# swiss-territorial-data-lab/proj-roadsurf

Hardware: AMD Instinct MI355X
Metric: tiles_per_sec_512x512x3 (higher is better)
Workload: dtype f16 hi + lo operand planes (22 significand bits, 3 MFMA products per product) / f32 accumulate; 1 GPU; Mask R-CNN R50-FPN inference, batch 16 of 512x512 3-band tiles per GPU (BASELINE configs[1]), 800x800 network input; seeded synthetic weights, saturated: 1000 proposals and 100 detections per tile; batch_per_gpu=16, lanes=2, lane_streams=independent, num_classes=2, weights=random

## Files before the change

proj_roadsurf_amd/csrc/common.h:

```cpp
#pragma once
#include <hip/hip_runtime.h>
#include <stdint.h>
#include <stdio.h>

typedef _Float16 half_t;
typedef _Float16 half4 __attribute__((ext_vector_type(4)));
typedef _Float16 half8 __attribute__((ext_vector_type(8)));
typedef float f32x4 __attribute__((ext_vector_type(4)));

#define RS_OK 0
#define RS_ERR_ARG -1
#define RS_ERR_HIP -2
#define RS_ERR_BLOB -3
#define RS_ERR_UNSUPPORTED -4

void rs_set_error(const char* fmt, ...);

#define RS_HIP(expr)                                                                       \
  do {                                                                                     \
    hipError_t _e = (expr);                                                                \
    if (_e != hipSuccess) {                                                                \
      rs_set_error("%s:%d: %s -> %s", __FILE__, __LINE__, #expr, hipGetErrorString(_e));   \
      return RS_ERR_HIP;                                                                   \
    }                                                                                      \
  } while (0)

#define RS_CHECK(cond, code, ...)  \
  do {                             \
    if (!(cond)) {                 \
      rs_set_error(__VA_ARGS__);   \
      return (code);               \
    }                              \
  } while (0)

static inline int cdiv(long long a, long long b) { return (int)((a + b - 1) / b); }

#if defined(__HIPCC__)
__device__ __forceinline__ float rs_fdiv(float a, float b) {
  const float y0 = __builtin_amdgcn_rcpf(b);
  const float e = __builtin_fmaf(-b, y0, 1.0f);
  const float y = __builtin_fmaf(e, y0, y0);
  const float q0 = a * y;
  const float r0 = __builtin_fmaf(-b, q0, a);
  const float q1 = __builtin_fmaf(r0, y, q0);
  const float r1 = __builtin_fmaf(-b, q1, a);
  const float q = __builtin_fmaf(r1, y, q1);
  const bool special = !(__builtin_fabsf(b) > 0.f && __builtin_fabsf(b) < __builtin_inff() && __builtin_fabsf(a) > 0.f && __builtin_fabsf(a) < __builtin_inff());
  return special ? a * y0 : q;
}

__device__ __forceinline__ unsigned rs_sat_bad(float f) { return !(__builtin_fabsf(f) <= 65504.f); }
__device__ __forceinline__ void rs_sat_flush(unsigned long long* sat, unsigned cnt) {
  if (sat != nullptr && cnt != 0u) atomicAdd(sat, (unsigned long long)cnt);
}
#endif

struct RsDebug {
  int conv_single_stage_nk = 4;
  int conv_persist = 0;
  int conv_tuned = 1;
  int conv_deep = 1;
  int conv_wide_px = 128;
  int wreg_dbg = 0;
  int wreg_waves = 2;
  int conv_wreg = 1;
  int stem_small_tile = 1;
  int deep_dbg = 0;
  int deconv_variant = 22;
  int fuse_mask_predictor = 1;
  int side_stream = 1;
  int narrow_roialign = 0;
  int use_glds = 1;
  int fuse_shortcut = 1;
  int fuse_stem = 1;
  int fuse_bneck = 1;
  int deep_tile_px = 1;
  int deep_tail = 1;
  int fuse_rpn_heads = 1;
  int merge_levels = 1;
  int graph_small = 1;
  int use_graph = 0;
  int train_roi_side = -1;
  int train_side = -1;
  int wgrad_target = 512;
  int wgrad_cb = 0;
  int select_debug = 0;
  int nms_debug = 0;
  int roi_window = 1;
  int roi_bwd_atomic = 0;
  int roi_order = 1;
};
const RsDebug& rs_debug();
void rs_debug_reload();

struct ConvSeg {
  const half_t* in;
  const half_t* w;
  const float* bias;
  void* out;
  float* head_out;
  int Ho, Wo, in_Hp, in_Wp, out_Hp, out_Wp;
  int M;
  int tile0;
  long long in_lo, out_lo;
  const float* wscale;
};
#define RS_MAX_SEGS 5

struct ConvParams {
  const half_t* in;
  const half_t* w;
  const float* bias;
  void* out;
  const half_t* res;
  const half_t* up;
  const int* m_count;
  const int* koff;
  int m_mul;
  int M;
  int Ho, Wo;
  int in_Hp, in_Wp, in_Cs, in_off;
  int stride;
  int KH, KW, Cin;
  int Kpad;
  int Cout;
  int out_Hp, out_Wp, out_Cs, out_pad;
  int up_Hp, up_Wp, up_Cs, up_pad;
  int relu;
  int mode;
  int out_f32;
  const float* dot_w;
  const int* dot_cls;
  const int* dot_slot;
  float* dot_out;
  int dot_k;
  const half_t* in2;
  int in2_Hp, in2_Wp, in2_Cs, in2_off, stride2, Cin2;
  const half_t* down;
  int down_Hp, down_Wp, down_Cs, down_pad;
  const float* res32;
  const half_t* mask;
  int out_stride;
  long long* probe;
  int persist;
  int stages;
  const half_t* head_w;
  const float* head_b;
  float* head_out;
  int nseg;
  int seg_tiles;
  int tail_tiles;
  int split;
  long long in_lo, w_lo, out_lo, res_lo, up_lo, in2_lo;
  const float* wscale;
  long long head_w_lo;
  const float* head_scale;
  ConvSeg seg[RS_MAX_SEGS];
  unsigned long long* sat;
};

int launch_conv(const ConvParams& p, hipStream_t stream, int force_variant , int use_glds);
int conv_choose_variant(ConvParams& p, int force_variant, int use_glds);
extern thread_local int g_last_conv_variant;

struct StemPoolParams {
  const half_t* in;
  const half_t* wf;
  const float* bias;
  half_t* out;
  int N, in_Hp, in_Wp;
  int Hc, Wc;
  int Hq, Wq;
  unsigned long long* sat;
};
int launch_stem_pool(const StemPoolParams& p, hipStream_t stream);
struct StemPoolSplitParams {
  const half_t* in; long long in_lo;
  const half_t* wf;
  const float* wscale;
  const float* bias;
  half_t* out; long long out_lo;
  int N, in_Hp, in_Wp;
  int Hc, Wc;
  int Hq, Wq;
  unsigned long long* sat;
};
int launch_stem_pool_split(const StemPoolSplitParams& p, hipStream_t stream);

struct BneckParams {
  const half_t* t1;
  const half_t* w2;
  const float* b2;
  const half_t* w3p;
  const float* b3;
  const half_t* x;
  const half_t* x0;
  const half_t* wsc;
  half_t* out;
  const half_t* w1p;
  const float* b1;
  half_t* t1n;
  int M, H, W, Hp, Wp;
  int CB;
  unsigned long long* sat;
};
int launch_bneck_tail(const BneckParams& p, hipStream_t stream);

struct BneckSplitParams {
  const half_t* t1; long long t1_lo;
  const half_t* w2; long long w2_lo;
  const float* b2; const float* s2;
  const half_t* w3p; long long w3_lo;
  const float* b3; const float* s3;
  const half_t* x; long long x_lo;
  half_t* out; long long out_lo;
  const half_t* w1p; long long w1_lo;
  const float* b1; const float* s1;
  half_t* t1n; long long t1n_lo;
  const half_t* x0; long long x0_lo;
  int M, H, W, Hp, Wp;
  int CB;
  unsigned long long* sat;
};
int launch_bneck_tail_split(const BneckSplitParams& p, hipStream_t stream);

int launch_mask_overlap(const uint8_t* det, int n_det, const uint8_t* lab, int n_lab, int h, int w, int* inter, int* lab_area, hipStream_t s);

struct WgradParams {
  const half_t* dy;
  const half_t* x;
  float* partial;
  float* grad;
  const half_t* zeros;
  const float* scale;
  int M, Ho, Wo;
  int dy_Hp, dy_Wp, dy_Cs, dy_pad;
  int in_Hp, in_Wp, in_Cs, in_off;
  int stride, KH, KW, Cin, Cout, Kpad;
  const int* m_count;
  int m_mul;
  int splits;
  int accumulate;
  int f32;
};
int wgrad_splits(const WgradParams& p);
int launch_conv_wgrad(const WgradParams& p, hipStream_t stream);

struct PreprocParams {
  const uint8_t* tiles;
  half_t* out;
  const int* hb;
  const int* hk;
  const int* vb;
  const int* vk;
  int N, H, W, C;
  int new_h, new_w;
  int out_Hp, out_Wp;
  int ksh, ksv;
  int need_h, need_v;
  int flip;
  int out_f32;
  long long out_lo;
  float mean[4], stdv[4];
  unsigned long long* sat;
};
int launch_preprocess(const PreprocParams& p, hipStream_t s);
int launch_maxpool(const half_t* in, half_t* out, int N, int Hi, int Wi, int Ho, int Wo, int C, hipStream_t s);
int launch_subsample2(const half_t* in, half_t* out, int N, int Hi, int Wi, int Ho, int Wo, int C, hipStream_t s);
int launch_maxpool_f32(const float* in, float* out, int N, int Hi, int Wi, int Ho, int Wo, int C, hipStream_t s);
int launch_maxpool_split(const half_t* in, long long in_lo, half_t* out, long long out_lo, int N, int Hi, int Wi, int Ho, int Wo, int C, hipStream_t s);
int launch_subsample2_split(const half_t* in, long long in_lo, half_t* out, long long out_lo, int N, int Hi, int Wi, int Ho, int Wo, int C, hipStream_t s);
int launch_subsample2_f32(const float* in, float* out, int N, int Hi, int Wi, int Ho, int Wo, int C, hipStream_t s);
int launch_conv_f32(const ConvParams& p, hipStream_t stream, int force_valu = 0, int tile = 0);
int launch_conv_deep(const ConvParams& p, hipStream_t stream, int tile_px = 256);
int rs_device_cu_count();
bool conv_wreg_ok(const ConvParams& p);
int launch_conv_wreg(const ConvParams& p, hipStream_t stream, int waves = 0);
int launch_conv_deep_multi(const ConvParams& common, const ConvSeg* segs, const int* m_per_image, int nseg, int images, hipStream_t stream);
```

proj_roadsurf_amd/csrc/conv_deep.hip:

```cpp
#include "common.h"

namespace {

constexpr int BN = 256, NT = 512, MI = 4, WCH = 4;
constexpr int ASTAGE = 256 * 128, WSTAGE = BN * 128;
constexpr int W_BASE = 3 * ASTAGE;
constexpr int LDS_BYTES = 3 * ASTAGE + 2 * WSTAGE;

__device__ __forceinline__ void glds16(const half_t* g, char* lds_wave_base) {
  __builtin_amdgcn_global_load_lds((const __attribute__((address_space(1))) void*)g,
                                   (__attribute__((address_space(3))) void*)lds_wave_base, 16, 0, 0);
}

template <int DBG, bool TRAIN, int NJ, bool SPLIT>
__device__ __forceinline__ void conv_deep_tile(const ConvParams& p, char* smem, const half_t* g_in, const half_t* g_w, const float* g_bias, void* g_out,
                                               float* g_head_out, const int Ho, const int Wo, const int in_Hp, const int in_Wp, const int out_Hp, const int out_Wp,
                                               const int M, const int m0, const int n0, const int q, const long long in_lo, const long long out_lo,
                                               const float* g_wscale) {
  constexpr int APS = (NJ + 1) / 2;
  constexpr int WPX = NJ * 16;
  const int tid = threadIdx.x;
  const int lane = tid & 63;
  const int wave = __builtin_amdgcn_readfirstlane(tid >> 6);
  const int wpx = wave / WCH, wch = wave % WCH;
  (void)q;

  const int lrow = lane >> 3, lchk = lane & 7;
  const half_t* aptr[APS];
  const half_t* wptr[4];
  unsigned aoffb[APS], woffb[4];
#pragma unroll
  for (int ps = 0; ps < APS; ++ps) {
    int m = m0 + ps * 64 + wave * 8 + lrow;
    if (m >= M) m = M - 1;
    const int x = m % Wo;
    const int t = m / Wo;
    const int y = t % Ho;
    const int n = t / Ho;
    const long long base =
        ((long long)(n * in_Hp + y * p.stride + p.in_off) * in_Wp + x * p.stride + p.in_off) * p.in_Cs;
    if constexpr (SPLIT) aoffb[ps] = (unsigned)((base + ((lchk ^ lrow) & 3) * 8 + ((lchk ^ lrow) >> 2) * in_lo) * 2);
    else aptr[ps] = g_in + base + (lchk ^ lrow) * 8;
  }
#pragma unroll
  for (int ps = 0; ps < 4; ++ps) {
    const int row = ps * 64 + wave * 8 + lrow;
    const int key = (row & 3) | (((row >> 4) & 1) << 2);
    if constexpr (SPLIT) woffb[ps] = (unsigned)(((long long)(n0 + row) * p.Kpad + ((lchk ^ key) & 3) * 8 + ((lchk ^ key) >> 2) * p.w_lo) * 2);
    else wptr[ps] = g_w + (long long)(n0 + row) * p.Kpad + (lchk ^ key) * 8;
  }
  constexpr int KST = SPLIT ? 32 : 64;
  const int nk = p.KH * p.KW * (p.Cin / KST);

  int akh = 0, akw = 0, ac0 = 0, an = 0;
  auto stage_a = [&]() {
    const int off = (akh * in_Wp + akw) * p.in_Cs + ac0;
    if (++akw == p.KW) { akw = 0; if (++akh == p.KH) { akh = 0; ac0 += KST; } }
    char* abase = smem + (an % 3) * ASTAGE;
    ++an;
    if (DBG & 1) return;
    if (DBG & 8) return;
    if constexpr (SPLIT) {
#pragma unroll
      for (int ps = 0; ps < APS; ++ps) glds16((const half_t*)((const char*)g_in + (aoffb[ps] + (unsigned)(off * 2))), abase + (ps * 64 + wave * 8) * 128);
    } else {
#pragma unroll
      for (int ps = 0; ps < APS; ++ps) glds16(aptr[ps] + off, abase + (ps * 64 + wave * 8) * 128);
    }
  };
  int wkh = 0, wkw = 0, wc0 = 0, wn = 0;
  auto stage_w = [&]() {
    const int koff = (wkh * p.KW + wkw) * p.Cin + wc0;
    if (++wkw == p.KW) { wkw = 0; if (++wkh == p.KH) { wkh = 0; wc0 += KST; } }
    char* wbase = smem + W_BASE + (wn & 1) * WSTAGE;
    ++wn;
    if (DBG & 1) return;
    if (DBG & 4) return;
    if constexpr (SPLIT) {
#pragma unroll
      for (int ps = 0; ps < 4; ++ps) glds16((const half_t*)((const char*)g_w + (woffb[ps] + (unsigned)(koff * 2))), wbase + (ps * 64 + wave * 8) * 128);
    } else {
#pragma unroll
      for (int ps = 0; ps < 4; ++ps) glds16(wptr[ps] + koff, wbase + (ps * 64 + wave * 8) * 128);
    }
  };

  const int fi = lane & 15, fq = lane >> 4, fkey = lane & 7;
  int w_off[MI], x_off[NJ];
#pragma unroll
  for (int i = 0; i < MI; ++i) w_off[i] = W_BASE + (wch * 64 + (fi >> 2) * 16 + i * 4 + (fi & 3)) * 128;
#pragma unroll
  for (int j = 0; j < NJ; ++j) x_off[j] = (wpx * WPX + j * 16 + fi) * 128;
  const int c0_off = (fq ^ fkey) * 16, c1_off = ((4 + fq) ^ fkey) * 16;

  f32x4 acc[MI][NJ];
#pragma unroll
  for (int i = 0; i < MI; ++i)
#pragma unroll
    for (int j = 0; j < NJ; ++j) acc[i][j] = f32x4{0.f, 0.f, 0.f, 0.f};

  half8 wf0[MI], xf0[NJ], wf1[MI], xf1[NJ];
  const unsigned lds0 = (unsigned)(uintptr_t)(__attribute__((address_space(3))) char*)smem;
  const unsigned wrow = (unsigned)(W_BASE + (wch * 64 + (fi >> 2) * 16 + (fi & 3)) * 128);
  const unsigned xrow = (unsigned)((wpx * WPX + fi) * 128);
  const unsigned wa0 = lds0 + wrow + c0_off, wa1 = lds0 + wrow + c1_off;
  const unsigned xa0 = lds0 + xrow + c0_off, xa1 = lds0 + xrow + c1_off;
#define RS_DSR(dst, addr, off) asm volatile("ds_read_b128 %0, %1 offset:%2" : "=v"(dst) : "v"(addr), "n"(off))
#define RS_READS(wf, xf, wa, xa)                                                        \
  RS_DSR(wf[0], wa, 0); RS_DSR(wf[1], wa, 512); RS_DSR(wf[2], wa, 1024); RS_DSR(wf[3], wa, 1536);   \
  RS_DSR(xf[0], xa, 0); RS_DSR(xf[1], xa, 2048);                                                    \
  if constexpr (NJ > 2) { RS_DSR(xf[2], xa, 4096); }                                                \
  if constexpr (NJ > 3) { RS_DSR(xf[3], xa, 6144); }                                                \
  if constexpr (NJ > 4) { RS_DSR(xf[4], xa, 8192); }                                                \
  if constexpr (NJ > 5) { RS_DSR(xf[5], xa, 10240); }                                               \
  if constexpr (NJ > 6) { RS_DSR(xf[6], xa, 12288); }                                               \
  if constexpr (NJ > 7) { RS_DSR(xf[7], xa, 14336); }
  auto reads0 = [&](int ab, int wb) {
    if (DBG & 16) return;
    const unsigned wa = wa0 + ((DBG & 2) ? 0 : wb) * WSTAGE, xa = xa0 + ((DBG & 2) ? 0 : ab) * ASTAGE;
    RS_READS(wf0, xf0, wa, xa)
  };
  auto reads1 = [&](int ab, int wb) {
    if (DBG & 16) return;
    const unsigned wa = wa1 + ((DBG & 2) ? 0 : wb) * WSTAGE, xa = xa1 + ((DBG & 2) ? 0 : ab) * ASTAGE;
    RS_READS(wf1, xf1, wa, xa)
  };
#ifdef RS_CLOCK_PROBE
  const unsigned long long pr_t0 = __builtin_amdgcn_s_memtime(), pr_r0 = __builtin_amdgcn_s_memrealtime();
#endif
#ifdef RS_SPLIT_PHASES
  const unsigned long long ph_entry = __builtin_amdgcn_s_memtime();
  unsigned long long ph_loop0 = 0, ph_loop1 = 0;
#endif
  stage_w();
  stage_a();
  if (nk > 1) stage_a();
  if (nk > 1) asm volatile("s_waitcnt vmcnt(%0)" ::"n"(APS) : "memory");
  else asm volatile("s_waitcnt vmcnt(0)" ::: "memory");
  asm volatile("s_barrier" ::: "memory");
  __builtin_amdgcn_sched_barrier(0);
  if (nk > 1) stage_w();
#ifndef RS_SPLIT_SCHED_V1
  if constexpr (!SPLIT) { if (nk > 2) stage_a(); }
#else
  if (nk > 2) stage_a();
#endif
  if constexpr (SPLIT) {
#define RS_RD_W(wf, wa) RS_DSR(wf[0], wa, 0); RS_DSR(wf[1], wa, 512); RS_DSR(wf[2], wa, 1024); RS_DSR(wf[3], wa, 1536);
#define RS_RD_X(xf, xa)                                                                             \
  RS_DSR(xf[0], xa, 0); RS_DSR(xf[1], xa, 2048);                                                    \
  if constexpr (NJ > 2) { RS_DSR(xf[2], xa, 4096); }                                                \
  if constexpr (NJ > 3) { RS_DSR(xf[3], xa, 6144); }                                                \
  if constexpr (NJ > 4) { RS_DSR(xf[4], xa, 8192); }                                                \
  if constexpr (NJ > 5) { RS_DSR(xf[5], xa, 10240); }                                               \
  if constexpr (NJ > 6) { RS_DSR(xf[6], xa, 12288); }                                               \
  if constexpr (NJ > 7) { RS_DSR(xf[7], xa, 14336); }
    {
      const unsigned wa = wa0, xa = xa1;
      RS_RD_W(wf0, wa)
      RS_RD_X(xf1, xa)
    }
    int sab = 0;
#ifdef RS_SPLIT_PHASES
    unsigned long long ph_work = 0, ph_vm = 0, ph_bar = 0, ph_last = __builtin_amdgcn_s_memtime();
    ph_loop0 = ph_last;
#endif
    for (int t = 0; t < nk; ++t) {
      const unsigned wst = (t & 1) * WSTAGE, ast = sab * ASTAGE;
      __builtin_amdgcn_sched_barrier(0);
      { const unsigned xa = xa0 + ast; RS_RD_X(xf0, xa) }
      __builtin_amdgcn_sched_barrier(0);
      asm volatile("s_waitcnt lgkmcnt(%0)" ::"n"(NJ) : "memory");
      __builtin_amdgcn_sched_barrier(0);
#pragma unroll
      for (int i = 0; i < MI; ++i)
#pragma unroll
        for (int j = 0; j < NJ; ++j)
          acc[i][j] = __builtin_amdgcn_mfma_f32_16x16x32_f16(wf0[i], xf1[j], acc[i][j], 0, 0, 0);
      __builtin_amdgcn_sched_barrier(0);
#ifndef RS_SPLIT_SCHED_V1
      if (t + 2 < nk) stage_a();
#endif
      { const unsigned wa = wa1 + wst; RS_RD_W(wf1, wa) }
      __builtin_amdgcn_sched_barrier(0);
      asm volatile("s_waitcnt lgkmcnt(4)" ::: "memory");
      __builtin_amdgcn_sched_barrier(0);
#pragma unroll
      for (int i = 0; i < MI; ++i)
#pragma unroll
        for (int j = 0; j < NJ; ++j)
          acc[i][j] = __builtin_amdgcn_mfma_f32_16x16x32_f16(wf0[i], xf0[j], acc[i][j], 0, 0, 0);
      __builtin_amdgcn_sched_barrier(0);
      const int snext = sab == 2 ? 0 : sab + 1;
      if (t + 1 < nk) {
        asm volatile("s_waitcnt lgkmcnt(0)" ::: "memory");
#ifdef RS_SPLIT_PHASES
        __builtin_amdgcn_sched_barrier(0);
        const unsigned long long ph1 = __builtin_amdgcn_s_memtime();
        ph_work += ph1 - ph_last;
        __builtin_amdgcn_sched_barrier(0);
#endif
        if (t + 2 < nk) asm volatile("s_waitcnt vmcnt(%0)" ::"n"(APS) : "memory");
        else asm volatile("s_waitcnt vmcnt(0)" ::: "memory");
#ifdef RS_SPLIT_PHASES
        __builtin_amdgcn_sched_barrier(0);
        const unsigned long long ph2 = __builtin_amdgcn_s_memtime();
        ph_vm += ph2 - ph1;
        __builtin_amdgcn_sched_barrier(0);
#endif
        asm volatile("s_barrier" ::: "memory");
        __builtin_amdgcn_sched_barrier(0);
#ifdef RS_SPLIT_PHASES
        ph_last = __builtin_amdgcn_s_memtime();
        ph_bar += ph_last - ph2;
        __builtin_amdgcn_sched_barrier(0);
#endif
        if (wpx) {
#pragma unroll
          for (int i = 0; i < MI; ++i)
#pragma unroll
            for (int j = 0; j < NJ; ++j)
              acc[i][j] = __builtin_amdgcn_mfma_f32_16x16x32_f16(wf1[i], xf0[j], acc[i][j], 0, 0, 0);
          __builtin_amdgcn_sched_barrier(0);
        }
        if (t + 2 < nk) stage_w();
#ifdef RS_SPLIT_SCHED_V1
        if (t + 3 < nk) stage_a();
#endif
        {
          const unsigned wa = wa0 + ((t + 1) & 1) * WSTAGE, xa = xa1 + snext * ASTAGE;
          RS_RD_W(wf0, wa)
          RS_RD_X(xf1, xa)
        }
        if (wpx) { sab = snext; continue; }
      } else {
        __builtin_amdgcn_sched_barrier(0);
        asm volatile("s_waitcnt lgkmcnt(0)" ::: "memory");
      }
      sab = snext;
      __builtin_amdgcn_sched_barrier(0);
#pragma unroll
      for (int i = 0; i < MI; ++i)
#pragma unroll
        for (int j = 0; j < NJ; ++j)
          acc[i][j] = __builtin_amdgcn_mfma_f32_16x16x32_f16(wf1[i], xf0[j], acc[i][j], 0, 0, 0);
    }
#undef RS_RD_W
#undef RS_RD_X
#ifdef RS_SPLIT_PHASES
    ph_loop1 = __builtin_amdgcn_s_memtime();
    if (p.probe && lane == 0) {
      long long* o = p.probe + ((long long)q * 8 + wave) * 8;
      o[0] = (long long)ph_work; o[1] = (long long)ph_vm; o[2] = (long long)ph_bar; o[3] = nk;
      o[4] = (long long)(ph_loop0 - ph_entry); o[5] = (long long)(ph_loop1 - ph_loop0);
    }
#endif
  } else {
  reads0(0, 0);
  int abuf = 0;
  for (int t = 0; t < nk; ++t) {
    __builtin_amdgcn_sched_barrier(0);
    reads1(abuf, t & 1);
    __builtin_amdgcn_sched_barrier(0);
    asm volatile("s_waitcnt lgkmcnt(%0)" ::"n"(4 + NJ) : "memory");
    __builtin_amdgcn_sched_barrier(0);
#pragma unroll
    for (int i = 0; i < MI; ++i)
#pragma unroll
      for (int j = 0; j < NJ; ++j)
        acc[i][j] = __builtin_amdgcn_mfma_f32_16x16x32_f16(wf0[i], xf0[j], acc[i][j], 0, 0, 0);
    __builtin_amdgcn_sched_barrier(0);
    const int anext = abuf == 2 ? 0 : abuf + 1;
    if (t + 1 < nk) {
      asm volatile("s_waitcnt lgkmcnt(0)" ::: "memory");
      if (t + 2 < nk) asm volatile("s_waitcnt vmcnt(%0)" ::"n"(APS) : "memory");
      else asm volatile("s_waitcnt vmcnt(0)" ::: "memory");
      asm volatile("s_barrier" ::: "memory");
      __builtin_amdgcn_sched_barrier(0);
#ifndef RS_DEEP_LOCKSTEP
      if (wpx) {
#pragma unroll
        for (int i = 0; i < MI; ++i)
#pragma unroll
          for (int j = 0; j < NJ; ++j)
            acc[i][j] = __builtin_amdgcn_mfma_f32_16x16x32_f16(wf1[i], xf1[j], acc[i][j], 0, 0, 0);
        __builtin_amdgcn_sched_barrier(0);
      }
#endif
      if (t + 2 < nk) stage_w();
      if (t + 3 < nk) stage_a();
      reads0(anext, (t + 1) & 1);
#ifndef RS_DEEP_LOCKSTEP
      if (wpx) { abuf = anext; continue; }
#endif
    }
    else {
      __builtin_amdgcn_sched_barrier(0);
      asm volatile("s_waitcnt lgkmcnt(0)" ::: "memory");
    }
    abuf = anext;
    __builtin_amdgcn_sched_barrier(0);
#pragma unroll
    for (int i = 0; i < MI; ++i)
#pragma unroll
      for (int j = 0; j < NJ; ++j)
        acc[i][j] = __builtin_amdgcn_mfma_f32_16x16x32_f16(wf1[i], xf1[j], acc[i][j], 0, 0, 0);
  }
  }

#ifdef RS_CLOCK_PROBE
  if (p.probe && tid == 0) {
    p.probe[2 * q] = (long long)(__builtin_amdgcn_s_memtime() - pr_t0);
    p.probe[2 * q + 1] = (long long)(__builtin_amdgcn_s_memrealtime() - pr_r0);
  }
#endif
  const int crow = n0 + wch * 64 + fq * 16;
  float bias[16];
#pragma unroll
  for (int i = 0; i < MI; ++i) {
    const f32x4 b4 = *(const f32x4*)(g_bias + crow + i * 4);
    bias[i * 4 + 0] = b4[0]; bias[i * 4 + 1] = b4[1]; bias[i * 4 + 2] = b4[2]; bias[i * 4 + 3] = b4[3];
  }
  float wsc[SPLIT ? 16 : 1];
  if constexpr (SPLIT) {
#pragma unroll
    for (int i = 0; i < MI; ++i) {
      const f32x4 s4 = *(const f32x4*)(g_wscale + crow + i * 4);
      wsc[i * 4 + 0] = s4[0]; wsc[i * 4 + 1] = s4[1]; wsc[i * 4 + 2] = s4[2]; wsc[i * 4 + 3] = s4[3];
    }
  }
  unsigned satc = 0;
  if (!TRAIN && SPLIT && p.head_w) {
    const half_t* hw = p.head_w + (long long)fi * 256 + wch * 64 + fq * 8;
    const half8 ha0 = *(const half8*)hw, ha1 = *(const half8*)(hw + 32);
    const half8 hl0 = *(const half8*)(hw + p.head_w_lo), hl1 = *(const half8*)(hw + p.head_w_lo + 32);
    f32x4 hacc[NJ];
#pragma unroll
    for (int j = 0; j < NJ; ++j) {
      half8 b0, b1, l0, l1;
      const bool mv = m0 + wpx * WPX + j * 16 + fi < M;
      unsigned sath = 0;
#pragma unroll
      for (int i = 0; i < MI; ++i)
#pragma unroll
        for (int r = 0; r < 4; ++r) {
          float f = acc[i][j][r] * wsc[i * 4 + r] + bias[i * 4 + r];
          if (p.relu) f = f > 0.f ? f : 0.f;
          sath += mv ? rs_sat_bad(f) : 0u;
          f = f > 65504.f ? 65504.f : (f < -65504.f ? -65504.f : f);
          const half_t h = (half_t)f;
          const half_t l = (half_t)(f - (float)h);
          if (i < 2) { b0[i * 4 + r] = h; l0[i * 4 + r] = l; } else { b1[(i - 2) * 4 + r] = h; l1[(i - 2) * 4 + r] = l; }
        }
      rs_sat_flush(p.sat, sath);
      f32x4 a = f32x4{0.f, 0.f, 0.f, 0.f};
      a = __builtin_amdgcn_mfma_f32_16x16x32_f16(ha0, b0, a, 0, 0, 0);
      a = __builtin_amdgcn_mfma_f32_16x16x32_f16(ha1, b1, a, 0, 0, 0);
      a = __builtin_amdgcn_mfma_f32_16x16x32_f16(ha0, l0, a, 0, 0, 0);
      a = __builtin_amdgcn_mfma_f32_16x16x32_f16(ha1, l1, a, 0, 0, 0);
      a = __builtin_amdgcn_mfma_f32_16x16x32_f16(hl0, b0, a, 0, 0, 0);
      a = __builtin_amdgcn_mfma_f32_16x16x32_f16(hl1, b1, a, 0, 0, 0);
      hacc[j] = a;
    }
    asm volatile("s_barrier" ::: "memory");
    float* part = (float*)smem;
#pragma unroll
    for (int j = 0; j < NJ; ++j) *(f32x4*)(part + ((wch * 2 * WPX + wpx * WPX + j * 16 + fi) * 16 + fq * 4)) = hacc[j];
    __syncthreads();
    const int px = tid >> 1, oh = (tid & 1) * 8;
    const int m = m0 + px;
    if (px < 2 * WPX && m < M) {
      f32x4 s0 = f32x4{0.f, 0.f, 0.f, 0.f}, s1 = f32x4{0.f, 0.f, 0.f, 0.f};
#pragma unroll
      for (int w = 0; w < 4; ++w) {
        s0 += *(const f32x4*)(part + ((w * 2 * WPX + px) * 16 + oh));
        s1 += *(const f32x4*)(part + ((w * 2 * WPX + px) * 16 + oh + 4));
      }
      s0 = s0 * *(const f32x4*)(p.head_scale + oh) + *(const f32x4*)(p.head_b + oh);
      s1 = s1 * *(const f32x4*)(p.head_scale + oh + 4) + *(const f32x4*)(p.head_b + oh + 4);
      const int x = m % Wo, t = m / Wo, y = t % Ho, n = t / Ho;
      float* op = g_head_out + ((long long)(n * Ho + y) * Wo + x) * 16 + oh;
      *(f32x4*)op = s0;
      *(f32x4*)(op + 4) = s1;
    }
    return;
  }
  if (!TRAIN && !SPLIT && p.head_w) {
    const half_t* hw = p.head_w + (long long)fi * 256 + wch * 64 + fq * 8;
    const half8 ha0 = *(const half8*)hw, ha1 = *(const half8*)(hw + 32);
    f32x4 hacc[NJ];
#pragma unroll
    for (int j = 0; j < NJ; ++j) {
      half8 b0, b1;
      const bool mv = m0 + wpx * WPX + j * 16 + fi < M;
      unsigned sath = 0;
#pragma unroll
      for (int i = 0; i < MI; ++i)
#pragma unroll
        for (int r = 0; r < 4; ++r) {
          float f = acc[i][j][r] + bias[i * 4 + r];
          if (p.relu) f = f > 0.f ? f : 0.f;
          sath += mv ? rs_sat_bad(f) : 0u;
          f = f > 65504.f ? 65504.f : (f < -65504.f ? -65504.f : f);
          if (i < 2) b0[i * 4 + r] = (half_t)f; else b1[(i - 2) * 4 + r] = (half_t)f;
        }
      rs_sat_flush(p.sat, sath);
      f32x4 a = f32x4{0.f, 0.f, 0.f, 0.f};
      a = __builtin_amdgcn_mfma_f32_16x16x32_f16(ha0, b0, a, 0, 0, 0);
      a = __builtin_amdgcn_mfma_f32_16x16x32_f16(ha1, b1, a, 0, 0, 0);
      hacc[j] = a;
    }
    asm volatile("s_barrier" ::: "memory");
    float* part = (float*)smem;
#pragma unroll
    for (int j = 0; j < NJ; ++j) *(f32x4*)(part + ((wch * 2 * WPX + wpx * WPX + j * 16 + fi) * 16 + fq * 4)) = hacc[j];
    __syncthreads();
    const int px = tid >> 1, oh = (tid & 1) * 8;
    const int m = m0 + px;
    if (px < 2 * WPX && m < M) {
      f32x4 s0 = *(const f32x4*)(p.head_b + oh), s1 = *(const f32x4*)(p.head_b + oh + 4);
#pragma unroll
      for (int w = 0; w < 4; ++w) {
        s0 += *(const f32x4*)(part + ((w * 2 * WPX + px) * 16 + oh));
        s1 += *(const f32x4*)(part + ((w * 2 * WPX + px) * 16 + oh + 4));
      }
      const int x = m % Wo, t = m / Wo, y = t % Ho, n = t / Ho;
      float* op = g_head_out + ((long long)(n * Ho + y) * Wo + x) * 16 + oh;
      *(f32x4*)op = s0;
      *(f32x4*)(op + 4) = s1;
    }
    return;
  }
#pragma unroll
  for (int j = 0; j < NJ; ++j) {
    const int m = m0 + wpx * WPX + j * 16 + fi;
    if (m >= M) continue;
    const int x = m % Wo;
    const int t = m / Wo;
    const int y = t % Ho;
    const int n = t / Ho;
    const long long opix = (long long)(n * out_Hp + y + p.out_pad) * out_Wp + x + p.out_pad;
    float v[16];
#pragma unroll
    for (int i = 0; i < MI; ++i)
#pragma unroll
      for (int r = 0; r < 4; ++r) {
        if constexpr (SPLIT) v[i * 4 + r] = acc[i][j][r] * wsc[i * 4 + r] + bias[i * 4 + r];
        else v[i * 4 + r] = acc[i][j][r] + bias[i * 4 + r];
      }
    if (p.res) {
      const half_t* rp = p.res + opix * p.out_Cs + crow;
#pragma unroll
      for (int i = 0; i < MI; ++i) {
        const half4 h = *(const half4*)(rp + i * 4);
        if constexpr (SPLIT) {
          const half4 l = *(const half4*)(rp + p.res_lo + i * 4);
#pragma unroll
          for (int r = 0; r < 4; ++r) v[i * 4 + r] += (float)h[r] + (float)l[r];
        } else {
#pragma unroll
          for (int r = 0; r < 4; ++r) v[i * 4 + r] += (float)h[r];
        }
      }
    }
    if (p.up) {
      const long long upix = (long long)(n * p.up_Hp + (y >> 1) + p.up_pad) * p.up_Wp + (x >> 1) + p.up_pad;
      const half_t* up = p.up + upix * p.up_Cs + crow;
#pragma unroll
      for (int i = 0; i < MI; ++i) {
        const half4 h = *(const half4*)(up + i * 4);
        if constexpr (SPLIT) {
          const half4 l = *(const half4*)(up + p.up_lo + i * 4);
#pragma unroll
          for (int r = 0; r < 4; ++r) v[i * 4 + r] += (float)h[r] + (float)l[r];
        } else {
#pragma unroll
          for (int r = 0; r < 4; ++r) v[i * 4 + r] += (float)h[r];
        }
      }
    }
    if (TRAIN && p.down) {
#pragma unroll
      for (int dd = 0; dd < 4; ++dd) {
        const long long dpix = (long long)(n * p.down_Hp + 2 * y + (dd >> 1) + p.down_pad) * p.down_Wp + 2 * x + (dd & 1) + p.down_pad;
        const half_t* dp = p.down + dpix * p.down_Cs + crow;
#pragma unroll
        for (int i = 0; i < MI; ++i) {
          const half4 h = *(const half4*)(dp + i * 4);
#pragma unroll
          for (int r = 0; r < 4; ++r) v[i * 4 + r] += (float)h[r];
        }
      }
    }
    if (TRAIN && p.res32) {
      const float* rp = p.res32 + opix * p.out_Cs + crow;
#pragma unroll
      for (int i = 0; i < MI; ++i) {
        const f32x4 h = *(const f32x4*)(rp + i * 4);
#pragma unroll
        for (int r = 0; r < 4; ++r) v[i * 4 + r] += h[r];
      }
    }
    if (TRAIN && p.mask) {
      const half_t* mp = p.mask + opix * p.out_Cs + crow;
#pragma unroll
      for (int i = 0; i < MI; ++i) {
        const half4 h = *(const half4*)(mp + i * 4);
#pragma unroll
        for (int r = 0; r < 4; ++r) v[i * 4 + r] = (float)h[r] > 0.f ? v[i * 4 + r] : 0.f;
      }
    }
    if (p.relu) {
#pragma unroll
      for (int e = 0; e < 16; ++e) v[e] = v[e] > 0.f ? v[e] : 0.f;
    }
    if (p.out_f32) {
      float* op = (float*)g_out + opix * p.out_Cs + crow;
#pragma unroll
      for (int i = 0; i < MI; ++i) *(f32x4*)(op + i * 4) = f32x4{v[i * 4], v[i * 4 + 1], v[i * 4 + 2], v[i * 4 + 3]};
    } else {
      half_t* op = (half_t*)g_out + opix * p.out_Cs + crow;
#pragma unroll
      for (int i = 0; i < MI; i += 2) {
        half8 h, l;
#pragma unroll
        for (int r = 0; r < 8; ++r) {
          float f = v[i * 4 + r];
          satc += rs_sat_bad(f);
          f = f > 65504.f ? 65504.f : (f < -65504.f ? -65504.f : f);
          h[r] = (half_t)f;
          if constexpr (SPLIT) l[r] = (half_t)(f - (float)h[r]);
        }
        *(half8*)(op + i * 4) = h;
        if constexpr (SPLIT) *(half8*)(op + out_lo + i * 4) = l;
      }
    }
  }
  rs_sat_flush(p.sat, satc);
#ifdef RS_SPLIT_PHASES
  if constexpr (SPLIT) {
    const unsigned long long ph_issued = __builtin_amdgcn_s_memtime();
    asm volatile("s_waitcnt vmcnt(0)" ::: "memory");
    const unsigned long long ph_drained = __builtin_amdgcn_s_memtime();
    if (p.probe && lane == 0) {
      long long* o = p.probe + ((long long)q * 8 + wave) * 8;
      o[6] = (long long)(ph_issued - ph_loop1); o[7] = (long long)(ph_drained - ph_issued);
    }
  }
#endif
}


template <int DBG, bool TRAIN = false, int NJF = 8, bool SPLIT = false>
__global__ __launch_bounds__(NT) void conv_deep_kernel(const ConvParams p) {
  constexpr int BM = 32 * NJF;
  extern __shared__ __attribute__((aligned(16))) char smem[];
  int M = p.M;
  if (p.m_count) {
    long long mc = (long long)(*p.m_count) * p.m_mul;
    if (mc < M) M = (int)mc;
  }
  const int tiles_n = p.Cout / BN;
  const int ntiles = p.nseg ? p.seg_tiles : tiles_n * ((M + BM - 1) / BM);
  const int nfull = ntiles - p.tail_tiles;
  const int q = blockIdx.x;
  if (q >= nfull + 2 * p.tail_tiles) return;
  const half_t* g_in = p.in;
  const half_t* g_w = p.w;
  const float* g_bias = p.bias;
  void* g_out = p.out;
  float* g_head_out = p.head_out;
  long long in_lo = p.in_lo, out_lo = p.out_lo;
  const float* g_wscale = p.wscale;
  int Ho = p.Ho, Wo = p.Wo, in_Hp = p.in_Hp, in_Wp = p.in_Wp, out_Hp = p.out_Hp, out_Wp = p.out_Wp;
  int L, half = -1;
  if (q < nfull) {
    const int qn = nfull >> 3, r = nfull & 7, x = q & 7;
    L = (x < r ? x * (qn + 1) : r * (qn + 1) + (x - r) * qn) + (q >> 3);
  } else {
    L = nfull + ((q - nfull) >> 1);
    half = (q - nfull) & 1;
  }
  if (p.nseg) {
    int t0 = 0;
#pragma unroll
    for (int i = 0; i < RS_MAX_SEGS; ++i)
      if (i < p.nseg && L >= p.seg[i].tile0) {
        g_in = p.seg[i].in; g_w = p.seg[i].w; g_bias = p.seg[i].bias; g_out = p.seg[i].out; g_head_out = p.seg[i].head_out;
        Ho = p.seg[i].Ho; Wo = p.seg[i].Wo; in_Hp = p.seg[i].in_Hp; in_Wp = p.seg[i].in_Wp;
        out_Hp = p.seg[i].out_Hp; out_Wp = p.seg[i].out_Wp; M = p.seg[i].M; t0 = p.seg[i].tile0;
        if constexpr (SPLIT) { in_lo = p.seg[i].in_lo; out_lo = p.seg[i].out_lo; g_wscale = p.seg[i].wscale; }
      }
    L -= t0;
  }
  const int n0 = (L % tiles_n) * BN;
  const int m0 = (L / tiles_n) * BM;
  if (half < 0 || NJF != 8) {
    conv_deep_tile<DBG, TRAIN, NJF, SPLIT>(p, smem, g_in, g_w, g_bias, g_out, g_head_out, Ho, Wo, in_Hp, in_Wp, out_Hp, out_Wp, M, m0, n0, q, in_lo, out_lo, g_wscale);
  } else {
    if (m0 + half * (BM / 2) >= M) return;
    conv_deep_tile<DBG, TRAIN, NJF == 8 ? 4 : NJF, SPLIT>(p, smem, g_in, g_w, g_bias, g_out, g_head_out, Ho, Wo, in_Hp, in_Wp, out_Hp, out_Wp, M, m0 + half * (BM / 2), n0, q, in_lo, out_lo, g_wscale);
  }
}

}

int rs_device_cu_count() {
  static int ncu[64] = {0};
  int dev = 0;
  if (hipGetDevice(&dev) != hipSuccess || dev < 0 || dev >= 64) return 256;
  if (!ncu[dev]) {
    int n = 0;
    if (hipDeviceGetAttribute(&n, hipDeviceAttributeMultiprocessorCount, dev) != hipSuccess || n <= 0) n = 256;
    ncu[dev] = n;
  }
  return ncu[dev];
}

static int deep_tail_tiles(long long tiles) {
  const int ncu = rs_device_cu_count();
  if (!rs_debug().deep_tail) return 0;
  const int r = (int)(tiles % ncu);
  return (r > 0 && 2 * r <= ncu) ? r : 0;
}

static int no_scratch(const void* kernel, const char* what) {
  hipFuncAttributes a;
  RS_HIP(hipFuncGetAttributes(&a, kernel));
  RS_CHECK(a.localSizeBytes == 0, RS_ERR_UNSUPPORTED, "%s was built with %zu bytes of scratch per thread: its asm fragment reads must not be spilled (rebuild with the documented toolchain)",
           what, (size_t)a.localSizeBytes);
  return RS_OK;
}

template <int NJF>
static int launch_deep_nj(ConvParams& p, hipStream_t stream) {
  static bool done = false;
  if (!done) {
    RS_HIP(hipFuncSetAttribute((const void*)conv_deep_kernel<0, false, NJF>, hipFuncAttributeMaxDynamicSharedMemorySize, LDS_BYTES));
    if constexpr (NJF >= 5) RS_HIP(hipFuncSetAttribute((const void*)conv_deep_kernel<0, false, NJF, true>, hipFuncAttributeMaxDynamicSharedMemorySize, LDS_BYTES));
    { int rc = no_scratch((const void*)conv_deep_kernel<0, false, NJF>, "conv_deep_kernel"); if (rc) return rc; }
    if constexpr (NJF >= 5) { int rc = no_scratch((const void*)conv_deep_kernel<0, false, NJF, true>, "conv_deep_kernel (split operands)"); if (rc) return rc; }
    done = true;
  }
  const long long nblk = (long long)(p.Cout / BN) * cdiv(p.M, 32 * NJF);
  RS_CHECK(nblk < (1ll << 30), RS_ERR_ARG, "conv_deep: grid too large");
  p.tail_tiles = 0;
  if (p.split) {
    if constexpr (NJF >= 5) hipLaunchKernelGGL((conv_deep_kernel<0, false, NJF, true>), dim3((unsigned)nblk), dim3(NT), LDS_BYTES, stream, p);
    else RS_CHECK(false, RS_ERR_UNSUPPORTED, "conv_deep: the split-operand mode has the 160 .. 256-pixel tiles only");
    RS_HIP(hipGetLastError());
    return RS_OK;
  }
  hipLaunchKernelGGL((conv_deep_kernel<0, false, NJF>), dim3((unsigned)nblk), dim3(NT), LDS_BYTES, stream, p);
  RS_HIP(hipGetLastError());
  return RS_OK;
}

int launch_conv_deep(const ConvParams& p0, hipStream_t stream, int tile_px) {
  ConvParams p = p0;
  p.nseg = 0;
  RS_CHECK(p.mode == 0 && !p.in2 && p.Cin % 64 == 0 && p.Cout % BN == 0 && p.M > 0, RS_ERR_ARG,
           "conv_deep: unsupported shape (mode %d, Cin %d, Cout %d)", p.mode, p.Cin, p.Cout);
  RS_CHECK(!p.head_w || (p.Cout == BN && p.head_b && p.head_out && !p.res && !p.up && !p.down && !p.res32 && !p.mask), RS_ERR_ARG,
           "conv_deep: the fused head needs Cout == 256, its bias and output, and no other epilogue option");
  RS_CHECK(p.out_stride <= 1, RS_ERR_UNSUPPORTED, "conv_deep: no strided scatter");
  RS_CHECK(!p.split || (p.wscale && (!p.head_w || p.head_scale) && !p.down && !p.res32 && !p.mask), RS_ERR_UNSUPPORTED, "conv_deep: the split-operand mode needs the row scales (the fused head's too) and has no training epilogue");
  if (p.split) {
    const long long in_px = (long long)cdiv(p.M, p.Ho * p.Wo) * p.in_Hp * p.in_Wp;
    RS_CHECK((p.in_lo + in_px * p.in_Cs) * 2 < (1ll << 32) && (p.w_lo + (long long)p.Cout * p.Kpad) * 2 < (1ll << 32), RS_ERR_UNSUPPORTED,
             "conv_deep: split-operand tensor of more than 4 GB (input %lld elements per plane)", in_px * p.in_Cs);
  }
  if (tile_px != 256) {
    RS_CHECK(tile_px >= 64 && tile_px <= 224 && tile_px % 32 == 0 && !p.down && !p.res32 && !p.mask, RS_ERR_ARG,
             "conv_deep: tile height %d (256, or 64 .. 224 in steps of 32 without training epilogue options)", tile_px);
    switch (tile_px / 32) {
      case 2: return launch_deep_nj<2>(p, stream);
      case 3: return launch_deep_nj<3>(p, stream);
      case 4: return launch_deep_nj<4>(p, stream);
      case 5: return launch_deep_nj<5>(p, stream);
      case 6: return launch_deep_nj<6>(p, stream);
      default: return launch_deep_nj<7>(p, stream);
    }
  }
  constexpr int BM = 256;
  static bool done = false;
  if (!done) {
    RS_HIP(hipFuncSetAttribute((const void*)conv_deep_kernel<0>, hipFuncAttributeMaxDynamicSharedMemorySize, LDS_BYTES));
    RS_HIP(hipFuncSetAttribute((const void*)conv_deep_kernel<0, true>, hipFuncAttributeMaxDynamicSharedMemorySize, LDS_BYTES));
    RS_HIP(hipFuncSetAttribute((const void*)conv_deep_kernel<0, false, 8, true>, hipFuncAttributeMaxDynamicSharedMemorySize, LDS_BYTES));
    { int rc = no_scratch((const void*)conv_deep_kernel<0>, "conv_deep_kernel"); if (rc) return rc; }
    { int rc = no_scratch((const void*)conv_deep_kernel<0, true>, "conv_deep_kernel (training epilogue)"); if (rc) return rc; }
    { int rc = no_scratch((const void*)conv_deep_kernel<0, false, 8, true>, "conv_deep_kernel (split operands)"); if (rc) return rc; }
#ifdef RS_DEEP_CEILING
    RS_HIP(hipFuncSetAttribute((const void*)conv_deep_kernel<1>, hipFuncAttributeMaxDynamicSharedMemorySize, LDS_BYTES));
    RS_HIP(hipFuncSetAttribute((const void*)conv_deep_kernel<3>, hipFuncAttributeMaxDynamicSharedMemorySize, LDS_BYTES));
    RS_HIP(hipFuncSetAttribute((const void*)conv_deep_kernel<4>, hipFuncAttributeMaxDynamicSharedMemorySize, LDS_BYTES));
    RS_HIP(hipFuncSetAttribute((const void*)conv_deep_kernel<8>, hipFuncAttributeMaxDynamicSharedMemorySize, LDS_BYTES));
    RS_HIP(hipFuncSetAttribute((const void*)conv_deep_kernel<17>, hipFuncAttributeMaxDynamicSharedMemorySize, LDS_BYTES));
#endif
    done = true;
  }
#ifdef RS_DEEP_CEILING
  const int dbg = rs_debug().deep_dbg;
#else
  constexpr int dbg = 0;
#endif
  long long nblk = (long long)(p.Cout / BN) * cdiv(p.M, BM);
  RS_CHECK(nblk < (1ll << 30), RS_ERR_ARG, "conv_deep: grid too large");
  p.tail_tiles = (p.m_count || dbg) ? 0 : deep_tail_tiles(nblk);
  nblk += p.tail_tiles;
#ifdef RS_DEEP_CEILING
  if (dbg == 1) { hipLaunchKernelGGL(conv_deep_kernel<1>, dim3((unsigned)nblk), dim3(NT), LDS_BYTES, stream, p); return RS_OK; }
  if (dbg == 3) { hipLaunchKernelGGL(conv_deep_kernel<3>, dim3((unsigned)nblk), dim3(NT), LDS_BYTES, stream, p); return RS_OK; }
  if (dbg == 4) { hipLaunchKernelGGL(conv_deep_kernel<4>, dim3((unsigned)nblk), dim3(NT), LDS_BYTES, stream, p); return RS_OK; }
  if (dbg == 8) { hipLaunchKernelGGL(conv_deep_kernel<8>, dim3((unsigned)nblk), dim3(NT), LDS_BYTES, stream, p); return RS_OK; }
  if (dbg == 17) { hipLaunchKernelGGL(conv_deep_kernel<17>, dim3((unsigned)nblk), dim3(NT), LDS_BYTES, stream, p); return RS_OK; }
#endif
  (void)dbg;
  if (p.split) hipLaunchKernelGGL((conv_deep_kernel<0, false, 8, true>), dim3((unsigned)nblk), dim3(NT), LDS_BYTES, stream, p);
  else if (p.down || p.res32 || p.mask) hipLaunchKernelGGL((conv_deep_kernel<0, true>), dim3((unsigned)nblk), dim3(NT), LDS_BYTES, stream, p);
  else hipLaunchKernelGGL(conv_deep_kernel<0>, dim3((unsigned)nblk), dim3(NT), LDS_BYTES, stream, p);
  RS_HIP(hipGetLastError());
  return RS_OK;
}

int launch_conv_deep_multi(const ConvParams& common, const ConvSeg* segs, const int* m_per_image, int nseg, int images, hipStream_t stream) {
  RS_CHECK(nseg >= 1 && nseg <= RS_MAX_SEGS && images >= 1, RS_ERR_ARG, "conv_deep_multi: %d maps", nseg);
  RS_CHECK(common.mode == 0 && !common.in2 && common.Cin % 64 == 0 && common.Cout % BN == 0 && !common.res && !common.up && !common.m_count &&
               !common.down && !common.res32 && !common.mask && common.out_stride <= 1,
           RS_ERR_ARG, "conv_deep_multi: unsupported shape (mode %d, Cin %d, Cout %d) or epilogue option", common.mode, common.Cin, common.Cout);
  ConvParams p = common;
  p.nseg = nseg;
  long long tiles = 0;
  for (int i = 0; i < nseg; ++i) {
    RS_CHECK(segs[i].in && segs[i].w && segs[i].bias && segs[i].out && m_per_image[i] > 0, RS_ERR_ARG, "conv_deep_multi: map %d incomplete", i);
    RS_CHECK(!common.split || segs[i].wscale, RS_ERR_ARG, "conv_deep_multi: map %d has no row scales (split-operand mode)", i);
    RS_CHECK(!common.split || ((segs[i].in_lo + (long long)images * segs[i].in_Hp * segs[i].in_Wp * common.in_Cs) * 2 < (1ll << 32) &&
                               (common.w_lo + (long long)common.Cout * common.Kpad) * 2 < (1ll << 32)),
             RS_ERR_UNSUPPORTED, "conv_deep_multi: map %d: split-operand tensor of more than 4 GB", i);
    p.seg[i] = segs[i];
    p.seg[i].M = images * m_per_image[i];
    p.seg[i].tile0 = (int)tiles;
    tiles += (long long)(p.Cout / BN) * cdiv(p.seg[i].M, 256);
  }
  RS_CHECK(tiles < (1ll << 30), RS_ERR_ARG, "conv_deep_multi: grid too large");
  if (p.head_w) {
    RS_CHECK(p.Cout == BN && p.head_b && !p.out_f32, RS_ERR_ARG, "conv_deep_multi: the fused head needs Cout == 256 and its bias");
    for (int i = 0; i < nseg; ++i) RS_CHECK(segs[i].head_out, RS_ERR_ARG, "conv_deep_multi: map %d has no head output", i);
  }
  p.seg_tiles = (int)tiles;
  p.tail_tiles = deep_tail_tiles(tiles);
  tiles += p.tail_tiles;
  p.in = segs[0].in; p.w = segs[0].w; p.bias = segs[0].bias; p.out = segs[0].out; p.M = p.seg[0].M;
  static bool done = false;
  if (!done) {
    RS_HIP(hipFuncSetAttribute((const void*)conv_deep_kernel<0>, hipFuncAttributeMaxDynamicSharedMemorySize, LDS_BYTES));
    RS_HIP(hipFuncSetAttribute((const void*)conv_deep_kernel<0, false, 8, true>, hipFuncAttributeMaxDynamicSharedMemorySize, LDS_BYTES));
    { int rc = no_scratch((const void*)conv_deep_kernel<0>, "conv_deep_kernel"); if (rc) return rc; }
    { int rc = no_scratch((const void*)conv_deep_kernel<0, false, 8, true>, "conv_deep_kernel (split operands)"); if (rc) return rc; }
    done = true;
  }
  if (p.split) {
    RS_CHECK(!p.head_w || p.head_scale, RS_ERR_ARG, "conv_deep_multi: the fused head of the split-operand mode needs its row scales");
    hipLaunchKernelGGL((conv_deep_kernel<0, false, 8, true>), dim3((unsigned)tiles), dim3(NT), LDS_BYTES, stream, p);
    RS_HIP(hipGetLastError());
    return RS_OK;
  }
  hipLaunchKernelGGL(conv_deep_kernel<0>, dim3((unsigned)tiles), dim3(NT), LDS_BYTES, stream, p);
  RS_HIP(hipGetLastError());
  return RS_OK;
}
```

proj_roadsurf_amd/csrc/engine.hip:

```cpp
#include <stdarg.h>
#include <string.h>

#include <cmath>
#include <functional>
#include <map>
#include <set>
#include <string>
#include <vector>

#include "../../include/rs_engine.h"
#include "detect.h"
#include "train.h"

static thread_local char g_err[1024] = "";
static bool g_trainer_unfused_shortcut = false;

static RsDebug g_debug;
static bool g_debug_loaded = false;
void rs_debug_reload() {
  RsDebug d;
  auto rd = [](const char* name, int* v) { const char* e = getenv(name); if (e && *e) *v = atoi(e); };
  rd("RS_CONV_SINGLE_STAGE_NK", &d.conv_single_stage_nk); rd("RS_CONV_PERSIST", &d.conv_persist); rd("RS_CONV_TUNED", &d.conv_tuned);
  rd("RS_CONV_DEEP", &d.conv_deep); rd("RS_CONV_WIDE_PX", &d.conv_wide_px); rd("RS_CONV_WREG", &d.conv_wreg); rd("RS_WREG_DBG", &d.wreg_dbg); rd("RS_ROI_BWD_ATOMIC", &d.roi_bwd_atomic); rd("RS_WREG_WAVES", &d.wreg_waves); rd("RS_STEM_SMALL_TILE", &d.stem_small_tile); rd("RS_DEEP_DBG", &d.deep_dbg);
  rd("RS_DECONV_VARIANT", &d.deconv_variant); rd("RS_FUSE_MASK_PREDICTOR", &d.fuse_mask_predictor); rd("RS_SIDE_STREAM", &d.side_stream);
  rd("RS_NARROW_ROIALIGN", &d.narrow_roialign); rd("RS_USE_GLDS", &d.use_glds); rd("RS_FUSE_SHORTCUT", &d.fuse_shortcut); rd("RS_MERGE_LEVELS", &d.merge_levels); rd("RS_FUSE_RPN_HEADS", &d.fuse_rpn_heads); rd("RS_DEEP_TAIL", &d.deep_tail); rd("RS_DEEP_TILE_PX", &d.deep_tile_px); rd("RS_FUSE_BNECK", &d.fuse_bneck); rd("RS_FUSE_STEM", &d.fuse_stem);
  rd("RS_USE_GRAPH", &d.use_graph); rd("RS_GRAPH_SMALL", &d.graph_small); rd("RS_TRAIN_ROI_SIDE", &d.train_roi_side);
  rd("RS_TRAIN_SIDE", &d.train_side); rd("RS_WGRAD_TARGET", &d.wgrad_target); rd("RS_WGRAD_CB", &d.wgrad_cb);
  rd("RS_SELECT_DEBUG", &d.select_debug); rd("RS_NMS_DEBUG", &d.nms_debug); rd("RS_ROI_WINDOW", &d.roi_window); rd("RS_ROI_ORDER", &d.roi_order);
  g_debug = d;
  g_debug_loaded = true;
}
const RsDebug& rs_debug() {
  if (!g_debug_loaded) rs_debug_reload();
  return g_debug;
}
void rs_set_error(const char* fmt, ...) {
  va_list a;
  va_start(a, fmt);
  vsnprintf(g_err, sizeof g_err, fmt, a);
  va_end(a);
}

namespace {

enum { DT_F16 = 1, DT_F32 = 2, DT_I32 = 3, DT_U8 = 4, DT_SPLIT16 = 5 };
static size_t dt_size(int dt) { return (dt == DT_F16 || dt == DT_SPLIT16) ? 2 : (dt == DT_U8 ? 1 : 4); }

struct TensorInfo {
  std::string name;
  void* p = nullptr;
  int dtype = 0, ndim = 0, halo = 0;
  int64_t dims[5] = {1, 1, 1, 1, 1};
  size_t bytes = 0;
};

struct Act {
  half_t* p = nullptr;
  long long lo = 0;
  int N = 0, H = 0, W = 0, C = 0, pad = 0;
  int Hp() const { return H + 2 * pad; }
  int Wp() const { return W + 2 * pad; }
};

struct Stage {
  std::string name;
  std::function<int(int, hipStream_t)> fn;
  double flops_per_image = 0, bytes_per_image = 0;
  double ms_total = 0;
  int calls = 0;
  double last_flops = 0, last_bytes = 0;
  int variant = -2;
  bool narrow = false;
  bool grad_side = false;
  int bucket = -1;
  int phase = 0;
  hipEvent_t handoff = nullptr;
};

struct BlobEntry { const void* host; void* dev; int dtype; int ndim; int64_t dims[4]; size_t nbytes; };

}

extern "C" void rs_resize_shape(int h, int w, int short_edge, int max_size, int* new_h, int* new_w) {
  double scale = (double)short_edge * 1.0 / (double)(h < w ? h : w);
  double newh, neww;
  if (h < w) { newh = short_edge; neww = scale * w; } else { newh = scale * h; neww = short_edge; }
  const double mx = newh > neww ? newh : neww;
  if (mx > max_size) {
    scale = (double)max_size * 1.0 / mx;
    newh = newh * scale;
    neww = neww * scale;
  }
  *new_w = (int)(neww + 0.5);
  *new_h = (int)(newh + 0.5);
}

extern "C" int rs_resize_coeffs(int in_size, int out_size, int32_t* bounds, int32_t* coeffs) {
  const double scale = (double)in_size / (double)out_size;
  const double filterscale = scale < 1.0 ? 1.0 : scale;
  const double support = 1.0 * filterscale;
  const int ksize = (int)ceil(support) * 2 + 1;
  if (!bounds || !coeffs) return ksize;
  const double ss = 1.0 / filterscale;
  std::vector<double> w(ksize);
  for (int xx = 0; xx < out_size; ++xx) {
    const double center = (xx + 0.5) * scale;
    int xmin = (int)(center - support + 0.5);
    if (xmin < 0) xmin = 0;
    int xmax = (int)(center + support + 0.5);
    if (xmax > in_size) xmax = in_size;
    xmax -= xmin;
    double ww = 0.0;
    for (int x = 0; x < ksize; ++x) w[x] = 0.0;
    for (int x = 0; x < xmax; ++x) {
      double a = (x + xmin - center + 0.5) * ss;
      if (a < 0) a = -a;
      const double v = a < 1.0 ? 1.0 - a : 0.0;
      w[x] = v;
      ww += v;
    }
    for (int x = 0; x < xmax; ++x)
      if (ww != 0.0) w[x] /= ww;
    for (int x = 0; x < ksize; ++x) {
      const double v = w[x] * (double)(1 << 22);
      coeffs[xx * ksize + x] = v < 0 ? (int)(v - 0.5) : (int)(v + 0.5);
    }
    bounds[xx * 2] = xmin;
    bounds[xx * 2 + 1] = xmax;
  }
  return ksize;
}

struct rs_engine {
  rs_spec spec;
  int device = 0;
  hipStream_t stream = nullptr;
  bool own_stream = false;
  hipStream_t copy_stream = nullptr;
  hipEvent_t ev_results = nullptr;
  hipEvent_t ev_copied = nullptr;
  bool copy_pending = false;
  hipStream_t narrow = nullptr;
  bool on_narrow = false;
  hipEvent_t ev_join = nullptr;
  bool cur_record = false;
  int max_batch = 0, tile_h = 0, tile_w = 0, tile_c = 0;
  int net_h = 0, net_w = 0, pad_h = 0, pad_w = 0;
  int use_glds = 1;
  bool f32 = false;
  bool split = false;
  int profiling = 0;
  hipEvent_t ev0 = nullptr, ev1 = nullptr;
  std::vector<std::pair<hipEvent_t, hipEvent_t>> ev_pool;
  std::vector<int> ev_stage;
  std::vector<int> ev_batch;
  size_t ev_used = 0;
  int resolve_profile();

  void* blob_dev = nullptr;
  std::map<std::string, BlobEntry> blob;
  std::vector<void*> allocs;
  std::vector<TensorInfo> tensors;
  std::vector<Stage> stages;

  uint8_t* tiles_dev = nullptr;
  struct ResizeTab { int* b = nullptr; int* k = nullptr; int ks = 0; };
  std::map<int, ResizeTab> tab_h, tab_v;
  std::vector<int> img_new_h, img_new_w;
  float* img_hw_dev = nullptr;
  int resize_tab(int in_size, int out_size, std::map<int, ResizeTab>& cache, ResizeTab* out);
  int set_image_sizes(const int32_t* new_h, const int32_t* new_w, int n);
  int* det_count = nullptr;
  float* det_boxes = nullptr;
  float* det_boxes_net = nullptr;
  float* det_scores = nullptr;
  int* det_classes = nullptr;
  uint8_t* masks = nullptr;
  float* mask_probs = nullptr;
  int D = 0;
  int* crop_rects = nullptr;
  unsigned int* crop_offsets = nullptr;
  unsigned long long* crop_total = nullptr;
  uint8_t* crop_data = nullptr;
  unsigned long long* h_crop_total = nullptr;
  hipEvent_t ev_crop_hdr = nullptr;

  int alloc(void** p, size_t bytes) {
    if (bytes == 0) bytes = 16;
    bytes = (bytes + 255) & ~(size_t)255;
    RS_HIP(hipMalloc(p, bytes));
    allocs.push_back(*p);
    RS_HIP(hipMemsetAsync(*p, 0, bytes, stream));
    return RS_OK;
  }
  void reg(const std::string& name, void* p, int dtype, std::vector<int64_t> dims, int halo) {
    TensorInfo t;
    t.name = name; t.p = p; t.dtype = dtype; t.ndim = (int)dims.size(); t.halo = halo;
    size_t nb = dt_size(dtype);
    for (size_t i = 0; i < dims.size(); ++i) { t.dims[i] = dims[i]; nb *= (size_t)dims[i]; }
    t.bytes = dtype == DT_SPLIT16 ? 2 * nb : nb;
    tensors.push_back(t);
  }
  int new_act(Act* a, const std::string& name, int N, int H, int W, int C, int pad) {
    a->N = N; a->H = H; a->W = W; a->C = C; a->pad = pad;
    const size_t bytes = (size_t)N * a->Hp() * a->Wp() * C * (f32 ? 4 : 2) * (split ? 2 : 1);
    int rc = alloc((void**)&a->p, bytes);
    if (rc) return rc;
    a->lo = split ? (long long)N * a->Hp() * a->Wp() * C : 0;
    reg(name, a->p, f32 ? DT_F32 : (split ? DT_SPLIT16 : DT_F16), {N, a->Hp(), a->Wp(), C}, pad);
    return RS_OK;
  }
  const BlobEntry* find(const std::string& n) {
    auto it = blob.find(n);
    return it == blob.end() ? nullptr : &it->second;
  }
  const BlobEntry* findw(const std::string& layer) { return find(layer + (f32 ? ".w32" : (split ? ".ws" : ".w"))); }
  int wrows(const BlobEntry* w) const { return (int)(split ? w->dims[0] / 2 : w->dims[0]); }
  int set_split(ConvParams* p, const std::string& wname, const BlobEntry* w, const Act* in, const Act* out, const Act* res, const Act* up, const Act* in2) {
    if (!split) return RS_OK;
    const BlobEntry* si = find(wname + ".wsi");
    RS_CHECK(si && si->dtype == DT_F32 && si->dims[0] >= w->dims[0] / 2 && (w->dims[0] & 1) == 0, RS_ERR_BLOB, "row scales of %s missing from blob (split-operand mode)", wname.c_str());
    p->split = 1;
    p->wscale = (const float*)si->dev;
    p->w_lo = (long long)(w->dims[0] / 2) * w->dims[1];
    if (in) p->in_lo = in->lo;
    if (out) p->out_lo = out->lo;
    if (res) p->res_lo = res->lo;
    if (up) p->up_lo = up->lo;
    if (in2) p->in2_lo = in2->lo;
    return RS_OK;
  }
  int parse_blob(const void* data, size_t nbytes);
  int build();
  struct DeferredConv { ConvParams p; int m_per_image = 0; double flops = 0, bytes = 0; };
  int add_conv(const std::string& name, const std::string& wname, const Act& in, const Act& out, int k, int stride,
               int pad, bool relu, const Act* res, const Act* up, int cin_real, int units_per_tile = 1,
               const int* m_count = nullptr, const Act* in2 = nullptr, int stride2 = 1, DeferredConv* defer = nullptr);
  int add_merged_convs(const std::string& name, const std::vector<DeferredConv>& d);
  int run(const uint8_t* tiles, int n, int phase = -1);
  int run_stages(int n, bool record, int phase = -1, bool all_wide = false);
  int assign_phases();
  int use_graph = 0;
  int fuse_shortcut = 1;
  int fuse_bneck = 1;
  int fuse_stem = 1;
  bool frozen_fusions_only = false;
  int merge_levels = 1;
  long long forward_index = 0;
  static constexpr int kSatCap = 512;
  unsigned long long* sat_dev = nullptr;
  unsigned long long* sat_snap = nullptr;
  unsigned long long* h_sat_copy = nullptr;
  bool sat_copy_pending = false;
  std::vector<int64_t> h_sat;
  unsigned long long* sat_slot() const { return sat_dev ? sat_dev + stages.size() : nullptr; }
  int sat_copy(hipStream_t s) {
    if (!sat_dev) return RS_OK;
    RS_HIP(hipMemcpyAsync(h_sat_copy, sat_snap, stages.size() * 8, hipMemcpyDeviceToHost, s));
    sat_copy_pending = true;
    return RS_OK;
  }
  void sat_publish() {
    if (!sat_copy_pending) return;
    h_sat.assign(h_sat_copy, h_sat_copy + stages.size());
    sat_copy_pending = false;
  }
  std::set<int> warmed;
  std::map<int, hipGraphExec_t> graphs;
};

int rs_engine::parse_blob(const void* data, size_t nbytes) {
  const uint8_t* b = (const uint8_t*)data;
  RS_CHECK(nbytes >= 16, RS_ERR_BLOB, "weight blob too small");
  uint32_t hdr[4];
  memcpy(hdr, b, 16);
  RS_CHECK(hdr[0] == 0x52534557u && hdr[1] == 1u, RS_ERR_BLOB, "bad weight blob magic/version %08x/%u", hdr[0], hdr[1]);
  const size_t ent = 96 + 4 + 4 + 32 + 8 + 8;
  RS_CHECK(16 + ent * hdr[2] <= nbytes, RS_ERR_BLOB, "weight blob truncated");
  RS_HIP(hipMalloc(&blob_dev, nbytes));
  RS_HIP(hipMemcpy(blob_dev, data, nbytes, hipMemcpyHostToDevice));
  for (uint32_t i = 0; i < hdr[2]; ++i) {
    const uint8_t* e = b + 16 + ent * i;
    char name[97];
    memcpy(name, e, 96);
    name[96] = 0;
    BlobEntry be;
    uint32_t dt, nd;
    uint64_t dims[4], off, nb;
    memcpy(&dt, e + 96, 4);
    memcpy(&nd, e + 100, 4);
    memcpy(dims, e + 104, 32);
    memcpy(&off, e + 136, 8);
    memcpy(&nb, e + 144, 8);
    RS_CHECK(off + nb <= nbytes, RS_ERR_BLOB, "weight blob entry %s out of range", name);
    be.host = b + off;
    be.dev = (char*)blob_dev + off;
    be.dtype = (int)dt;
    be.ndim = (int)nd;
    for (int d = 0; d < 4; ++d) be.dims[d] = (int64_t)dims[d];
    be.nbytes = nb;
    blob[name] = be;
  }
  return RS_OK;
}

int rs_engine::add_conv(const std::string& name, const std::string& wname, const Act& in, const Act& out, int k,
                        int stride, int pad, bool relu, const Act* res, const Act* up, int cin_real, int units_per_tile,
                        const int* m_count, const Act* in2, int stride2, DeferredConv* defer) {
  const BlobEntry* w = findw(wname);
  const BlobEntry* b = find(wname + ".b");
  RS_CHECK(w && b, RS_ERR_BLOB, "weights for %s missing from blob", wname.c_str());
  RS_CHECK(w->dtype == (f32 ? DT_F32 : DT_F16) && b->dtype == DT_F32, RS_ERR_BLOB, "weights for %s have wrong dtype", wname.c_str());
  ConvParams p;
  memset(&p, 0, sizeof p);
  { int rc = set_split(&p, wname, w, &in, &out, res, up, in2); if (rc) return rc; }
  p.in = in.p; p.w = (const half_t*)w->dev; p.bias = (const float*)b->dev; p.out = out.p;
  p.res = res ? res->p : nullptr;
  p.up = up ? up->p : nullptr;
  p.Ho = out.H; p.Wo = out.W;
  p.in_Hp = in.Hp(); p.in_Wp = in.Wp(); p.in_Cs = in.C; p.in_off = in.pad - pad;
  p.stride = stride; p.KH = k; p.KW = k; p.Cin = in.C;
  p.Kpad = (int)w->dims[1];
  p.Cout = out.C;
  p.out_Hp = out.Hp(); p.out_Wp = out.Wp(); p.out_Cs = out.C; p.out_pad = out.pad;
  if (up) { p.up_Hp = up->Hp(); p.up_Wp = up->Wp(); p.up_Cs = up->C; p.up_pad = up->pad; }
  p.relu = relu ? 1 : 0;
  if (in2) {
    RS_CHECK((out.H - 1) * stride2 < in2->H && (out.W - 1) * stride2 < in2->W && in2->C % 64 == 0, RS_ERR_ARG, "%s: second source geometry", name.c_str());
// ... 440 lines not shown
    if ((rc = add_conv("rpn.conv" + ln, "proposal_generator.rpn_head.conv", P[l], t, 3, 1, 1, true, nullptr, nullptr, 256))) return rc;
    rpn_t[l] = t;
  }
  for (int l = 0; l < L; ++l) {
    const std::string ln = std::to_string(l + 2);
    const Act t = rpn_t[l];
    float* ho = rpn_ho[l];
    if (!fuse_heads) {
      const BlobEntry* w = findw("proposal_generator.rpn_head.heads");
      const BlobEntry* b = find("proposal_generator.rpn_head.heads.b");
      RS_CHECK(w && b, RS_ERR_BLOB, "rpn head weights missing");
      RS_CHECK(wrows(w) == head_cs, RS_ERR_BLOB, "rpn head rows %d != %d", wrows(w), head_cs);
      ConvParams p;
      memset(&p, 0, sizeof p);
      if ((rc = set_split(&p, "proposal_generator.rpn_head.heads", w, &t, nullptr, nullptr, nullptr, nullptr))) return rc;
      p.in = t.p; p.w = (const half_t*)w->dev; p.bias = (const float*)b->dev; p.out = ho;
      p.Ho = t.H; p.Wo = t.W; p.in_Hp = t.Hp(); p.in_Wp = t.Wp(); p.in_Cs = 256; p.in_off = t.pad; p.stride = 1;
      p.KH = p.KW = 1; p.Cin = 256; p.Kpad = (int)w->dims[1]; p.Cout = head_cs;
      p.out_Hp = t.H; p.out_Wp = t.W; p.out_Cs = head_cs; p.out_pad = 0; p.out_f32 = 1;
      const int mpi = t.H * t.W;
      const int glds = use_glds;
      Stage st;
      st.name = "rpn.heads" + ln;
      st.flops_per_image = 2.0 * mpi * 256 * 5 * A;
      st.bytes_per_image = (double)mpi * (256 * 2 + head_cs * 4);
      st.fn = [p, mpi, glds](int n, hipStream_t s) mutable { p.M = n * mpi; return launch_conv(p, s, 2, glds); };
      stages.push_back(st);
    }
    rp.head[l] = ho;
    rp.H[l] = P[l].H; rp.W[l] = P[l].W; rp.stride[l] = 4 << l;
    uint32_t* keys = nullptr;
    if ((rc = alloc((void**)&keys, (size_t)NB * P[l].H * P[l].W * A * 4 * 2))) return rc;
    rp.keys[l] = keys;
    for (int a = 0; a < A; ++a)
      for (int d = 0; d < 4; ++d) rp.base[l][a][d] = S.cell_anchors[l][a][d];
    RS_CHECK((long long)P[l].H * P[l].W * A < (1 << 24), RS_ERR_UNSUPPORTED, "feature map too large for the RPN index select");
  }
  rp.offset = S.anchor_offset; rp.L = L; rp.A = A; rp.cs = head_cs; rp.topk = S.rpn_pre_nms_topk;
  rp.img_h = (float)net_h; rp.img_w = (float)net_w;
  rp.wx = S.rpn_bbox_reg_weights[0]; rp.wy = S.rpn_bbox_reg_weights[1]; rp.ww = S.rpn_bbox_reg_weights[2]; rp.wh = S.rpn_bbox_reg_weights[3];
  rp.scale_clamp = S.scale_clamp; rp.min_size = S.rpn_min_size;
  auto add_nms_rule = [&](const char* head, NmsParams* np, int group) -> int {
    int rc2;
    if ((rc2 = alloc((void**)&np->rule, (size_t)NB * 2 * 4))) return rc2;
    if ((rc2 = alloc((void**)&np->unit, (size_t)NB * 4))) return rc2;
    reg(std::string(head) + "_nms_rule", np->rule, DT_I32, {NB, 2}, 0);
    reg(std::string(head) + "_nms_unit", np->unit, DT_F32, {NB}, 0);
    np->group = group;
    return RS_OK;
  };
  uint8_t* cand_keep = nullptr;
  if ((rc = alloc((void**)&rp.cand_boxes, (size_t)NB * L * 1024 * 16))) return rc;
  if ((rc = alloc((void**)&rp.cand_scores, (size_t)NB * L * 1024 * 4))) return rc;
  if ((rc = alloc((void**)&rp.cand_valid, (size_t)NB * L * 1024))) return rc;
  if ((rc = alloc((void**)&rp.cand_count, (size_t)NB * L * 4))) return rc;
  if ((rc = alloc((void**)&rp.cand_index, (size_t)NB * L * 1024 * 4))) return rc;
  if ((rc = alloc((void**)&cand_keep, (size_t)NB * L * 1024))) return rc;
  reg("rpn_cand_boxes", rp.cand_boxes, DT_F32, {NB, L, 1024, 4}, 0);
  reg("rpn_cand_scores", rp.cand_scores, DT_F32, {NB, L, 1024}, 0);
  reg("rpn_cand_valid", rp.cand_valid, DT_U8, {NB, L, 1024}, 0);
  reg("rpn_cand_count", rp.cand_count, DT_I32, {NB, L}, 0);
  reg("rpn_cand_index", rp.cand_index, DT_I32, {NB, L, 1024}, 0);
  reg("rpn_cand_keep", cand_keep, DT_U8, {NB, L, 1024}, 0);
  {
    Stage st;
    st.name = "rpn.select_decode";
    st.fn = [rp](int n, hipStream_t s) mutable { rp.N = n; return launch_rpn_select(rp, s); };
    stages.push_back(st);
  }
  {
    NmsParams np = {};
    np.boxes = rp.cand_boxes; np.count = rp.cand_count; np.valid = rp.cand_valid; np.keep = cand_keep; np.cap = 1024;
    np.thresh = S.rpn_nms_thresh;
    if ((rc = alloc((void**)&np.scratch, (size_t)(NB * L < 32 ? NB * L : 32) * 1024 * 16 * 8))) return rc;
    if (S.batched_nms) { if ((rc = add_nms_rule("rpn", &np, L))) return rc; }
    Stage st;
    st.name = "rpn.nms";
    st.fn = [np, L](int n, hipStream_t s) { return launch_nms(np, n * L, s); };
    stages.push_back(st);
  }
  const int PC = 1024;
  float *prop_boxes, *prop_scores;
  int *prop_count, *prop_level;
  if ((rc = alloc((void**)&prop_boxes, (size_t)NB * PC * 16))) return rc;
  if ((rc = alloc((void**)&prop_scores, (size_t)NB * PC * 4))) return rc;
  if ((rc = alloc((void**)&prop_level, (size_t)NB * PC * 4))) return rc;
  if ((rc = alloc((void**)&prop_count, (size_t)NB * 4))) return rc;
  reg("proposal_boxes", prop_boxes, DT_F32, {NB, PC, 4}, 0);
  reg("proposal_logits", prop_scores, DT_F32, {NB, PC}, 0);
  reg("proposal_level", prop_level, DT_I32, {NB, PC}, 0);
  reg("proposal_count", prop_count, DT_I32, {NB}, 0);
  int* prop_order = nullptr;
  const bool roi_order = !f32 && !(split && rs_debug().roi_window != 1) && !g_trainer_unfused_shortcut && rs_debug().roi_order != 0;
  if (roi_order) {
    if ((rc = alloc((void**)&prop_order, (size_t)NB * PC * 4))) return rc;
    reg("proposal_order", prop_order, DT_I32, {NB, PC}, 0);
  }
  {
    RpnMergeParams mp = {};
    mp.cand_boxes = rp.cand_boxes; mp.cand_scores = rp.cand_scores; mp.keep = cand_keep; mp.cand_count = rp.cand_count;
    mp.L = L; mp.post_topk = S.rpn_post_nms_topk; mp.cap = PC;
    mp.prop_boxes = prop_boxes; mp.prop_scores = prop_scores; mp.prop_level = prop_level; mp.prop_count = prop_count;
    mp.prop_order = prop_order;
    Stage st;
    st.name = "rpn.merge";
    st.fn = [mp](int n, hipStream_t s) { return launch_rpn_merge(mp, n, s); };
    stages.push_back(st);
  }

  const int PR = S.box_pooler_resolution;
  RoiAlignParams ra;
  memset(&ra, 0, sizeof ra);
  for (int l = 0; l < 4; ++l) { ra.feat[l] = P[l].p; ra.H[l] = P[l].H; ra.W[l] = P[l].W; ra.scale[l] = 1.0f / (float)(4 << l); }
  ra.nlevels = 4; ra.C = 256; ra.f32 = f32 ? 1 : (split ? 2 : 0);
  for (int l = 0; l < 4; ++l) ra.feat_lo[l] = P[l].lo;
  Act boxfeat;
  if ((rc = new_act(&boxfeat, "box_pooled", NB * PC, PR, PR, 256, 0))) return rc;
  int* box_level = nullptr;
  if ((rc = alloc((void**)&box_level, (size_t)NB * PC * 4))) return rc;
  reg("box_roi_level", box_level, DT_I32, {NB, PC}, 0);
  {
    RoiAlignParams q = ra;
    q.rois = prop_boxes; q.per_image_count = prop_count; q.slots_per_image = PC; q.out = boxfeat.p; q.out_lo = boxfeat.lo; q.P = PR; q.out_pad = 0;
    q.out_level = box_level;
    q.order = prop_order;
    Stage st;
    st.name = "box.roi_align";
    st.bytes_per_image = (double)PC * PR * PR * 256 * 2 * 2 * (split ? 2 : 1);
    st.fn = [q](int n, hipStream_t s) mutable { q.S = n * PC; return launch_roi_align(q, s); };
    stages.push_back(st);
  }
  const int FC = S.box_fc_dim;
  Act fin, f1, f2;
  fin.p = boxfeat.p; fin.lo = boxfeat.lo; fin.N = 1; fin.H = NB * PC; fin.W = 1; fin.C = PR * PR * 256; fin.pad = 0;
  if ((rc = new_act(&f1, "box_fc1", 1, NB * PC, 1, FC, 0))) return rc;
  if ((rc = new_act(&f2, "box_fc2", 1, NB * PC, 1, FC, 0))) return rc;
  auto add_fc = [&](const std::string& name, const std::string& wn, const Act& in, const Act& out, bool relu, float* out32, int rows32) -> int {
    const BlobEntry* w = findw(wn);
    const BlobEntry* b = find(wn + ".b");
    RS_CHECK(w && b, RS_ERR_BLOB, "weights for %s missing", wn.c_str());
    ConvParams p;
    memset(&p, 0, sizeof p);
    { int rc2 = set_split(&p, wn, w, &in, out32 ? nullptr : &out, nullptr, nullptr, nullptr); if (rc2) return rc2; }
    p.in = in.p; p.w = (const half_t*)w->dev; p.bias = (const float*)b->dev;
    p.Ho = NB * PC; p.Wo = 1; p.in_Hp = NB * PC; p.in_Wp = 1; p.in_Cs = in.C; p.stride = 1; p.KH = p.KW = 1; p.Cin = in.C;
    p.Kpad = (int)w->dims[1];
    p.out_Hp = NB * PC; p.out_Wp = 1; p.relu = relu;
    if (out32) { p.out = out32; p.Cout = rows32; p.out_Cs = rows32; p.out_f32 = 1; }
    else { p.out = out.p; p.Cout = out.C; p.out_Cs = out.C; }
    RS_CHECK(wrows(w) >= p.Cout && p.Kpad >= in.C, RS_ERR_BLOB, "%s: weight shape", wn.c_str());
    const int glds = use_glds;
    const int variant = out32 ? 2 : -1;
    Stage st;
    st.name = name;
    st.flops_per_image = 2.0 * PC * (double)in.C * p.Cout;
    st.bytes_per_image = (double)PC * (in.C * 2 * (split ? 2 : 1) + p.Cout * (out32 ? 4 : (split ? 4 : 2)));
    p.sat = out32 ? nullptr : sat_slot();
    st.fn = [p, glds, variant](int n, hipStream_t s) mutable { p.M = n * PC; return launch_conv(p, s, variant, glds); };
    stages.push_back(st);
    return RS_OK;
  };
  if ((rc = add_fc("box.fc1", "roi_heads.box_head.fc1", fin, f1, true, nullptr, 0))) return rc;
  if ((rc = add_fc("box.fc2", "roi_heads.box_head.fc2", f1, f2, true, nullptr, 0))) return rc;
  const int K = S.num_classes;
  const int pred_cs = (5 * K + 1 + 15) / 16 * 16;
  float* pred = nullptr;
  if ((rc = alloc((void**)&pred, (size_t)NB * PC * pred_cs * 4))) return rc;
  reg("box_pred", pred, DT_F32, {NB, PC, pred_cs}, 0);
  if ((rc = add_fc("box.predictor", "roi_heads.box_predictor", f2, f2, false, pred, pred_cs))) return rc;

  D = S.detections_per_image;
  BoxCandParams bc;
  memset(&bc, 0, sizeof bc);
  bc.pred = pred; bc.prop_boxes = prop_boxes; bc.prop_count = prop_count; bc.K = K; bc.cap = PC; bc.cs = pred_cs;
  bc.wx = S.box_reg_weights[0]; bc.wy = S.box_reg_weights[1]; bc.ww = S.box_reg_weights[2]; bc.wh = S.box_reg_weights[3];
  bc.scale_clamp = S.scale_clamp; bc.img_h = (float)net_h; bc.img_w = (float)net_w; bc.score_thresh = S.score_thresh_test;
  uint8_t* seg_keep = nullptr;
  if ((rc = alloc((void**)&bc.dec_boxes, (size_t)NB * PC * K * 16))) return rc;
  if ((rc = alloc((void**)&bc.dec_scores, (size_t)NB * PC * K * 4))) return rc;
  if ((rc = alloc((void**)&bc.seg_boxes, (size_t)NB * K * 1024 * 16))) return rc;
  if ((rc = alloc((void**)&bc.seg_roi, (size_t)NB * K * 1024 * 4))) return rc;
  if ((rc = alloc((void**)&bc.seg_count, (size_t)NB * K * 4))) return rc;
  if ((rc = alloc((void**)&seg_keep, (size_t)NB * K * 1024))) return rc;
  reg("box_dec_boxes", bc.dec_boxes, DT_F32, {NB, PC, K, 4}, 0);
  reg("box_dec_scores", bc.dec_scores, DT_F32, {NB, PC, K}, 0);
  reg("box_seg_boxes", bc.seg_boxes, DT_F32, {NB, K, 1024, 4}, 0);
  reg("box_seg_roi", bc.seg_roi, DT_I32, {NB, K, 1024}, 0);
  reg("box_seg_count", bc.seg_count, DT_I32, {NB, K}, 0);
  reg("box_seg_keep", seg_keep, DT_U8, {NB, K, 1024}, 0);
  {
    Stage st;
    st.name = "box.candidates";
    st.fn = [bc](int n, hipStream_t s) { return launch_box_candidates(bc, n, s); };
    stages.push_back(st);
  }
  {
    NmsParams np = {};
    np.boxes = bc.seg_boxes; np.count = bc.seg_count; np.valid = nullptr; np.keep = seg_keep; np.cap = 1024; np.thresh = S.nms_thresh_test;
    if ((rc = alloc((void**)&np.scratch, (size_t)(NB * K < 32 ? NB * K : 32) * 1024 * 16 * 8))) return rc;
    if (S.batched_nms) { if ((rc = add_nms_rule("box", &np, K))) return rc; }
    Stage st;
    st.name = "box.nms";
    st.fn = [np, K](int n, hipStream_t s) { return launch_nms(np, n * K, s); };
    stages.push_back(st);
  }
  int* det_roi = nullptr;
  if ((rc = alloc((void**)&det_boxes_net, (size_t)NB * D * 16))) return rc;
  if ((rc = alloc((void**)&det_boxes, (size_t)NB * D * 16))) return rc;
  if ((rc = alloc((void**)&det_scores, (size_t)NB * D * 4))) return rc;
  if ((rc = alloc((void**)&det_classes, (size_t)NB * D * 4))) return rc;
  if ((rc = alloc((void**)&det_roi, (size_t)NB * D * 4))) return rc;
  if ((rc = alloc((void**)&det_count, (size_t)NB * 4))) return rc;
  reg("det_boxes_net", det_boxes_net, DT_F32, {NB, D, 4}, 0);
  reg("det_boxes", det_boxes, DT_F32, {NB, D, 4}, 0);
  reg("det_scores", det_scores, DT_F32, {NB, D}, 0);
  reg("det_classes", det_classes, DT_I32, {NB, D}, 0);
  reg("det_roi", det_roi, DT_I32, {NB, D}, 0);
  reg("det_count", det_count, DT_I32, {NB}, 0);
  {
    DetMergeParams dm;
    memset(&dm, 0, sizeof dm);
    dm.dec_boxes = bc.dec_boxes; dm.dec_scores = bc.dec_scores; dm.seg_roi = bc.seg_roi; dm.seg_count = bc.seg_count; dm.keep = seg_keep;
    dm.K = K; dm.cap = PC; dm.dets_per_image = D;
    dm.scale_x = (float)((double)tile_w / (double)net_w);
    dm.scale_y = (float)((double)tile_h / (double)net_h);
    dm.out_w = (float)tile_w; dm.out_h = (float)tile_h;
    dm.det_boxes_net = det_boxes_net; dm.det_boxes = det_boxes; dm.det_scores = det_scores; dm.det_classes = det_classes;
    dm.det_roi = det_roi; dm.det_count = det_count;
    Stage st;
    st.name = "box.merge_postprocess";
    st.fn = [dm](int n, hipStream_t s) { return launch_det_merge(dm, n, s); };
    stages.push_back(st);
  }

  if (S.mask_on) {
    const int MR = S.mask_pooler_resolution, R = NB * D;
    int *slot_list, *det_total;
    if ((rc = alloc((void**)&slot_list, (size_t)R * 4))) return rc;
    if ((rc = alloc((void**)&det_total, 16))) return rc;
    reg("det_slot_list", slot_list, DT_I32, {R}, 0);
    reg("det_total", det_total, DT_I32, {1}, 0);
    {
      Stage st;
      st.name = "mask.compact";
      int* dc = det_count;
      const int Dc = D;
      st.fn = [dc, Dc, slot_list, det_total](int n, hipStream_t s) { return launch_det_compact(dc, n, Dc, slot_list, det_total, s); };
      stages.push_back(st);
    }
    Act mx;
    if ((rc = new_act(&mx, "mask_pooled", R, MR, MR, 256, 1))) return rc;
    {
      RoiAlignParams q = ra;
      q.rois = det_boxes_net; q.slot_list = slot_list; q.n_entries = det_total; q.slots_per_image = D;
      q.out = mx.p; q.out_lo = mx.lo; q.P = MR; q.out_pad = 1;
      Stage st;
      st.name = "mask.roi_align";
      st.bytes_per_image = (double)D * MR * MR * 256 * 2 * 2 * (split ? 2 : 1);
      const int Dc = D;
      st.fn = [q, Dc](int n, hipStream_t s) mutable { q.S = n * Dc; return launch_roi_align(q, s); };
      stages.push_back(st);
    }
    Act curm = mx;
    for (int i = 0; i < S.mask_num_conv; ++i) {
      Act o;
      const std::string nm = "mask_fcn" + std::to_string(i + 1);
      if ((rc = new_act(&o, nm, R, MR, MR, 256, 1))) return rc;
      if ((rc = add_conv("mask.fcn" + std::to_string(i + 1), "roi_heads.mask_head." + nm, curm, o, 3, 1, 1, true, nullptr, nullptr, 256, D, det_total))) return rc;
      curm = o;
    }
    if ((rc = alloc((void**)&mask_probs, (size_t)R * RS_MASK_SIDE * RS_MASK_SIDE * 4))) return rc;
    reg("mask_probs", mask_probs, DT_F32, {NB, D, RS_MASK_SIDE, RS_MASK_SIDE}, 0);
    const BlobEntry* dw = findw("roi_heads.mask_head.deconv");
    const BlobEntry* db = find("roi_heads.mask_head.deconv.b");
    const BlobEntry* pw = find("roi_heads.mask_head.predictor.w");
    const BlobEntry* pb = find("roi_heads.mask_head.predictor.b");
    RS_CHECK(dw && db && wrows(dw) == 1024, RS_ERR_BLOB, "deconv weights missing / wrong rows");
    RS_CHECK(pw && pb && pw->dtype == DT_F32, RS_ERR_BLOB, "mask predictor weights missing");
    const bool fuse = f32 ? false : rs_debug().fuse_mask_predictor != 0;
    ConvParams dp;
    memset(&dp, 0, sizeof dp);
    if ((rc = set_split(&dp, "roi_heads.mask_head.deconv", dw, &curm, nullptr, nullptr, nullptr, nullptr))) return rc;
    dp.in = curm.p; dp.w = (const half_t*)dw->dev; dp.bias = (const float*)db->dev;
    dp.Ho = MR; dp.Wo = MR; dp.in_Hp = curm.Hp(); dp.in_Wp = curm.Wp(); dp.in_Cs = 256; dp.in_off = 1; dp.stride = 1; dp.KH = dp.KW = 1;
    dp.Cin = 256; dp.Kpad = (int)dw->dims[1]; dp.Cout = 256; dp.out_Hp = 2 * MR; dp.out_Wp = 2 * MR; dp.out_Cs = 256; dp.out_pad = 0; dp.relu = 1;
    dp.m_count = det_total; dp.m_mul = MR * MR;
    const int per_roi = MR * MR;
    if (fuse) {
      dp.mode = 2; dp.out = nullptr;
      dp.dot_w = (const float*)pw->dev; dp.dot_cls = det_classes; dp.dot_slot = slot_list; dp.dot_out = mask_probs;
      dp.dot_k = (int)pw->dims[0];
      const int glds = use_glds, Dc = D;
      const bool sp = split;
      float* probs = mask_probs;
      const size_t zero_per_tile = (size_t)D * RS_MASK_SIDE * RS_MASK_SIDE * 4;
      Stage st;
      st.name = "mask.deconv_predict";
      st.flops_per_image = 2.0 * D * per_roi * 256 * 1024 + 2.0 * D * RS_MASK_SIDE * RS_MASK_SIDE * 256;
      st.bytes_per_image = (double)D * per_roi * 256 * 2 * (split ? 2 : 1) + (double)D * RS_MASK_SIDE * RS_MASK_SIDE * 4;
      st.fn = [dp, per_roi, Dc, glds, probs, zero_per_tile, sp](int n, hipStream_t s) mutable {
        RS_HIP(hipMemsetAsync(probs, 0, zero_per_tile * n, s));
        dp.M = n * Dc * per_roi;
        const int dv = rs_debug().deconv_variant;
        return launch_conv(dp, s, (dv == 22 && (sp || !(rs_debug().conv_wreg && glds > 0))) ? 14 : dv, glds);
      };
      stages.push_back(st);
      MaskPredictParams mp;
      mp.f32 = 0;
      mp.in = nullptr; mp.w = nullptr; mp.b = (const float*)pb->dev; mp.slot_list = slot_list; mp.det_classes = det_classes;
      mp.n_entries = det_total; mp.out = mask_probs; mp.S = RS_MASK_SIDE;
      Stage st2;
      st2.name = "mask.bias_sigmoid";
      st2.fn = [mp, Dc](int n, hipStream_t s) { return launch_mask_sigmoid(mp, n * Dc, s); };
      stages.push_back(st2);
    } else {
      Act dec;
      if ((rc = new_act(&dec, "mask_deconv", R, 2 * MR, 2 * MR, 256, 0))) return rc;
      dp.mode = 1; dp.out = dec.p; dp.out_lo = dec.lo;
      {
        const int glds = use_glds, Dc = D;
        Stage st;
        st.name = "mask.deconv";
        st.flops_per_image = 2.0 * D * per_roi * 256 * 1024;
        st.bytes_per_image = (double)D * per_roi * 256 * 2 * 5;
        dp.sat = sat_slot();
        st.fn = [dp, per_roi, Dc, glds](int n, hipStream_t s) mutable { dp.M = n * Dc * per_roi; return launch_conv(dp, s, -1, glds); };
        stages.push_back(st);
      }
      MaskPredictParams mp;
      mp.in = dec.p; mp.w = (const float*)pw->dev; mp.b = (const float*)pb->dev; mp.slot_list = slot_list; mp.det_classes = det_classes;
      mp.n_entries = det_total; mp.out = mask_probs; mp.S = RS_MASK_SIDE; mp.f32 = f32 ? 1 : (split ? 2 : 0); mp.in_lo = dec.lo;
      Stage st;
      st.name = "mask.predict_sigmoid";
      st.bytes_per_image = (double)D * RS_MASK_SIDE * RS_MASK_SIDE * (256 * 2 + 4);
      const int Dc = D;
      st.fn = [mp, Dc](int n, hipStream_t s) { return launch_mask_predict(mp, n * Dc, s); };
      stages.push_back(st);
    }
    const int Wb = (tile_w + 7) / 8;
    if ((rc = alloc((void**)&masks, (size_t)R * tile_h * Wb))) return rc;
    reg("masks", masks, DT_U8, {NB, D, tile_h, Wb}, 0);
    if ((rc = alloc((void**)&crop_data, (size_t)R * tile_h * Wb))) return rc;
    if ((rc = alloc((void**)&crop_rects, (size_t)R * 16))) return rc;
    if ((rc = alloc((void**)&crop_offsets, (size_t)R * 4))) return rc;
    if ((rc = alloc((void**)&crop_total, 16))) return rc;
    {
      PasteParams pm;
      pm.probs = mask_probs; pm.det_boxes = det_boxes; pm.slot_list = slot_list; pm.n_entries = det_total; pm.out = masks;
      pm.S = RS_MASK_SIDE; pm.out_h = tile_h; pm.out_w = tile_w; pm.threshold = S.mask_threshold;
      Stage st;
      st.name = "mask.paste";
      st.bytes_per_image = (double)D * tile_h * Wb;
      const int Dc = D;
      st.fn = [pm, Dc](int n, hipStream_t s) { return launch_paste_masks(pm, n * Dc, s); };
      stages.push_back(st);
    }
  }
  RS_CHECK(stages.size() <= (size_t)kSatCap, RS_ERR_UNSUPPORTED, "%d stages: more than the %d saturation counters", (int)stages.size(), kSatCap);
  h_sat.assign(stages.size(), 0);
  RS_HIP(hipStreamSynchronize(stream));
  return RS_OK;
}

int rs_engine::assign_phases() {
  const bool side = rs_debug().side_stream != 0 && !use_graph;
  static const char* kNarrow[] = {"rpn.select_decode", "rpn.nms", "rpn.merge", "box.candidates", "box.nms",
                                  "box.merge_postprocess", "mask.compact"};
  int phase = 0;
  const bool roi_narrow = rs_debug().narrow_roialign != 0;
  for (Stage& st : stages) {
    if (st.name.rfind("box.", 0) == 0 && phase < 1) phase = 1;
    if (st.name.rfind("mask.", 0) == 0 && st.name != "mask.compact" && phase < 2) phase = 2;
    st.phase = phase;
    for (const char* nm : kNarrow) if (side && st.name == nm) st.narrow = true;
    if (side && roi_narrow && (st.name == "box.roi_align" || st.name == "mask.roi_align")) st.narrow = true;
  }
  if (!side) return RS_OK;
  RS_HIP(hipStreamCreateWithFlags(&narrow, hipStreamNonBlocking));
  RS_HIP(hipEventCreateWithFlags(&ev_join, hipEventDisableTiming));
  bool prev = false;
  for (Stage& st : stages) {
    if (st.narrow != prev) RS_HIP(hipEventCreateWithFlags(&st.handoff, hipEventDisableTiming));
    prev = st.narrow;
  }
  return RS_OK;
}

int rs_engine::run_stages(int n, bool record, int phase, bool all_wide) {
  if (sat_dev && phase <= 0) RS_HIP(hipMemsetAsync(sat_dev, 0, stages.size() * 8, stream));
  for (size_t si = 0; si < stages.size(); ++si) {
    Stage& st = stages[si];
    if (phase >= 0 && st.phase != phase) continue;
    if (all_wide) {
      g_last_conv_variant = -2;
      int rc = st.fn(n, stream);
      if (rc) return rc;
      st.variant = g_last_conv_variant;
      continue;
    }
    if (st.narrow != on_narrow) {
      hipStream_t from = on_narrow ? narrow : stream, to = st.narrow ? narrow : stream;
      RS_HIP(hipEventRecord(st.handoff, from));
      RS_HIP(hipStreamWaitEvent(to, st.handoff, 0));
      on_narrow = st.narrow;
    }
    hipStream_t ss = st.narrow ? narrow : stream;
    const bool pooled = record && profiling >= 2 && ev_used < ev_pool.size();
    if (record && profiling == 1) RS_HIP(hipEventRecord(ev0, ss));
    if (pooled) RS_HIP(hipEventRecord(ev_pool[ev_used].first, ss));
    g_last_conv_variant = -2;
    int rc = st.fn(n, ss);
    if (rc) return rc;
    st.variant = g_last_conv_variant;
    if (pooled) {
      RS_HIP(hipEventRecord(ev_pool[ev_used].second, ss));
      ev_stage[ev_used] = (int)si;
      ev_batch[ev_used] = n;
      ++ev_used;
    }
    if (record && profiling == 1) {
      RS_HIP(hipEventRecord(ev1, ss));
      RS_HIP(hipEventSynchronize(ev1));
      float ms = 0.f;
      RS_HIP(hipEventElapsedTime(&ms, ev0, ev1));
      st.ms_total += ms;
      st.calls += 1;
      st.last_flops = st.flops_per_image * n;
      st.last_bytes = st.bytes_per_image * n;
    }
  }
  if ((phase < 0 || phase == RS_NUM_PHASES - 1) && on_narrow) {
    RS_HIP(hipEventRecord(ev_join, narrow));
    RS_HIP(hipStreamWaitEvent(stream, ev_join, 0));
    on_narrow = false;
  }
  if (sat_dev && (phase < 0 || phase == RS_NUM_PHASES - 1))
    RS_HIP(hipMemcpyAsync(sat_snap, sat_dev, stages.size() * 8, hipMemcpyDeviceToDevice, stream));
  return RS_OK;
}

int rs_engine::run(const uint8_t* tiles, int n, int phase) {
  RS_CHECK(n >= 1 && n <= max_batch, RS_ERR_ARG, "batch %d outside [1, %d]", n, max_batch);
  RS_CHECK(phase >= -1 && phase < RS_NUM_PHASES, RS_ERR_ARG, "phase %d outside [-1, %d)", phase, RS_NUM_PHASES);
  if (phase <= 0) {
    if (tiles != tiles_dev) {
      RS_HIP(hipMemcpyAsync(tiles_dev, tiles, (size_t)n * tile_h * tile_w * tile_c, hipMemcpyDeviceToDevice, stream));
    }
    const long long idx = forward_index++;
    cur_record = profiling == 1 || profiling == 2 || (profiling == 3 && (idx & 3) == 0);
  }
  if (copy_pending && (phase < 0 || phase == 1)) {
    RS_HIP(hipStreamWaitEvent(stream, ev_copied, 0));
    copy_pending = false;
  }
  const bool record = cur_record;
  const bool small = n == 1 && rs_debug().graph_small != 0 && !on_narrow && img_new_h.empty() && !frozen_fusions_only;
  if (phase >= 0 || record || !(use_graph || small) || !warmed.count(n)) {
    int rc = run_stages(n, record, phase);
    if (rc) return rc;
    if (phase < 0) warmed.insert(n);
    return RS_OK;
  }
  auto it = graphs.find(n);
  if (it == graphs.end()) {
    hipGraph_t g = nullptr;
    hipGraphExec_t ge = nullptr;
    RS_HIP(hipStreamBeginCapture(stream, hipStreamCaptureModeThreadLocal));
    int rc = run_stages(n, false, -1, !use_graph);
    hipError_t he = hipStreamEndCapture(stream, &g);
    if (rc) { if (g) (void)hipGraphDestroy(g); return rc; }
    RS_HIP(he);
    RS_HIP(hipGraphInstantiate(&ge, g, nullptr, nullptr, 0));
    (void)hipGraphDestroy(g);
    it = graphs.emplace(n, ge).first;
  }
  RS_HIP(hipGraphLaunch(it->second, stream));
  return RS_OK;
}

int rs_engine::resolve_profile() {
  if (ev_used == 0) return RS_OK;
  RS_HIP(hipStreamSynchronize(stream));
  if (narrow) RS_HIP(hipStreamSynchronize(narrow));
  for (size_t i = 0; i < ev_used; ++i) {
    float ms = 0.f;
    RS_HIP(hipEventElapsedTime(&ms, ev_pool[i].first, ev_pool[i].second));
    Stage& st = stages[ev_stage[i]];
    st.ms_total += ms;
    st.calls += 1;
    st.last_flops = st.flops_per_image * ev_batch[i];
    st.last_bytes = st.bytes_per_image * ev_batch[i];
  }
  ev_used = 0;
  return RS_OK;
}

extern "C" {

const char* rs_last_error(void) { return g_err; }
int rs_abi_version(void) { return RS_ABI_VERSION; }

__global__ void fdiv_kernel(const float* a, const float* b, float* out, long long n) {
  const long long i = (long long)blockIdx.x * 256 + threadIdx.x;
  if (i < n) out[i] = rs_fdiv(a[i], b[i]);
}
int rs_op_fdiv(const float* a, const float* b, float* out, int64_t n, void* stream) {
  RS_CHECK(a && b && out && n > 0, RS_ERR_ARG, "bad argument");
  hipLaunchKernelGGL(fdiv_kernel, dim3((unsigned)((n + 255) / 256)), dim3(256), 0, (hipStream_t)stream, a, b, out, (long long)n);
  RS_HIP(hipGetLastError());
  return RS_OK;
}

int rs_memcpy_d2h(void* dst, const void* src, size_t n) {
  RS_HIP(hipMemcpy(dst, src, n, hipMemcpyDeviceToHost));
  return RS_OK;
}
int rs_memcpy_h2d(void* dst, const void* src, size_t n) {
  RS_HIP(hipMemcpy(dst, src, n, hipMemcpyHostToDevice));
  return RS_OK;
}

int rs_spec_batched_nms(const rs_spec* spec) {
  RS_CHECK(spec, RS_ERR_ARG, "null argument");
  if (spec->struct_size == RS_SPEC_SIZE_V1) return 0;
  RS_CHECK(spec->struct_size == (int32_t)sizeof(rs_spec), RS_ERR_ARG, "rs_spec size mismatch: caller %d, library %d (or %d without batched_nms)",
           spec->struct_size, (int)sizeof(rs_spec), (int)RS_SPEC_SIZE_V1);
  RS_CHECK(spec->batched_nms == 0 || spec->batched_nms == 1, RS_ERR_ARG, "rs_spec.batched_nms %d (0 = per category, 1 = torchvision's size rule)", spec->batched_nms);
  return spec->batched_nms;
}

int rs_engine_create(const rs_spec* spec, const void* weights, size_t nbytes, int device_ordinal, int max_batch,
                     int tile_h, int tile_w, int tile_c, void* stream, rs_engine** out) {
  RS_CHECK(spec && weights && out, RS_ERR_ARG, "null argument");
  const int nms_mode = rs_spec_batched_nms(spec);
  if (nms_mode < 0) return nms_mode;
  RS_CHECK(max_batch >= 1 && tile_h >= 32 && tile_w >= 32, RS_ERR_ARG, "bad batch/tile shape");
  int ndev = 0;
  RS_HIP(hipGetDeviceCount(&ndev));
  RS_CHECK(ndev > 0, RS_ERR_HIP, "no HIP device visible: the engine has no CPU fallback");
  RS_CHECK(device_ordinal >= 0 && device_ordinal < ndev, RS_ERR_ARG, "device %d of %d", device_ordinal, ndev);
  RS_HIP(hipSetDevice(device_ordinal));
  rs_engine* e = new rs_engine();
  memcpy(&e->spec, spec, (size_t)spec->struct_size);
  e->spec.struct_size = (int32_t)sizeof(rs_spec);
  e->spec.batched_nms = nms_mode;
  e->device = device_ordinal;
  e->max_batch = max_batch; e->tile_h = tile_h; e->tile_w = tile_w; e->tile_c = tile_c;
  rs_debug_reload();
  e->use_glds = rs_debug().use_glds;
  e->f32 = spec->precision == 1;
  e->split = spec->precision == 2;
  if (e->f32) e->use_glds = -1;
  if (e->split && (e->use_glds <= 0 || g_trainer_unfused_shortcut)) {
    rs_set_error("precision 2 (split operands) needs LDS-DMA staging and is an inference mode");
    delete e;
    return RS_ERR_UNSUPPORTED;
  }
  e->fuse_shortcut = rs_debug().fuse_shortcut;
  e->fuse_bneck = rs_debug().fuse_bneck;
  e->fuse_stem = rs_debug().fuse_stem;
  e->merge_levels = rs_debug().merge_levels;
  if (g_trainer_unfused_shortcut) e->frozen_fusions_only = true;
  e->use_graph = rs_debug().use_graph;
  if (stream) { e->stream = (hipStream_t)stream; e->own_stream = false; }
  else {
    hipError_t he = hipStreamCreateWithFlags(&e->stream, hipStreamNonBlocking);
    if (he != hipSuccess) { rs_set_error("hipStreamCreate: %s", hipGetErrorString(he)); delete e; return RS_ERR_HIP; }
    e->own_stream = true;
  }
  int rc = RS_OK;
  if (hipEventCreate(&e->ev0) != hipSuccess || hipEventCreate(&e->ev1) != hipSuccess) { rs_set_error("hipEventCreate failed"); rc = RS_ERR_HIP; }
  if (!rc) rc = e->parse_blob(weights, nbytes);
  if (!rc) rc = e->build();
  if (!rc) rc = e->assign_phases();
  if (rc) { rs_engine_destroy(e); return rc; }
  *out = e;
  return RS_OK;
}

void rs_engine_destroy(rs_engine* e) {
  if (!e) return;
  (void)hipSetDevice(e->device);
  if (e->stream) (void)hipStreamSynchronize(e->stream);
  if (e->narrow) { (void)hipStreamSynchronize(e->narrow); (void)hipStreamDestroy(e->narrow); }
  if (e->copy_stream) { (void)hipStreamSynchronize(e->copy_stream); (void)hipStreamDestroy(e->copy_stream); }
  if (e->ev_crop_hdr) (void)hipEventDestroy(e->ev_crop_hdr);
  if (e->h_crop_total) (void)hipHostFree(e->h_crop_total);
  if (e->h_sat_copy) (void)hipHostFree(e->h_sat_copy);
  if (e->ev_results) (void)hipEventDestroy(e->ev_results);
  if (e->ev_copied) (void)hipEventDestroy(e->ev_copied);
  if (e->ev_join) (void)hipEventDestroy(e->ev_join);
  for (Stage& st : e->stages) if (st.handoff) (void)hipEventDestroy(st.handoff);
  for (void* p : e->allocs) (void)hipFree(p);
  if (e->blob_dev) (void)hipFree(e->blob_dev);
  for (auto& kv : e->graphs) (void)hipGraphExecDestroy(kv.second);
  for (auto& pr : e->ev_pool) { if (pr.first) (void)hipEventDestroy(pr.first); if (pr.second) (void)hipEventDestroy(pr.second); }
  if (e->ev0) (void)hipEventDestroy(e->ev0);
  if (e->ev1) (void)hipEventDestroy(e->ev1);
  if (e->own_stream && e->stream) (void)hipStreamDestroy(e->stream);
  delete e;
}

int rs_engine_infer_device(rs_engine* e, const uint8_t* tiles_dev, int n) {
  RS_CHECK(e && tiles_dev, RS_ERR_ARG, "null argument");
  RS_HIP(hipSetDevice(e->device));
  return e->run(tiles_dev, n);
}

int rs_engine_infer_phase(rs_engine* e, const uint8_t* tiles_dev, int n, int phase) {
  RS_CHECK(e && tiles_dev, RS_ERR_ARG, "null argument");
  RS_CHECK(phase >= 0 && phase < RS_NUM_PHASES, RS_ERR_ARG, "phase %d outside [0, %d)", phase, RS_NUM_PHASES);
  RS_HIP(hipSetDevice(e->device));
  return e->run(tiles_dev, n, phase);
}
int rs_engine_phase_count(void) { return RS_NUM_PHASES; }

int rs_debug_run_stages_matching(rs_engine* e, const char* substr, int n) {
  RS_CHECK(e && substr && n >= 1 && n <= e->max_batch, RS_ERR_ARG, "bad argument");
  RS_HIP(hipSetDevice(e->device));
  for (Stage& st : e->stages)
    if (st.name.find(substr) != std::string::npos) {
      int rc = st.fn(n, e->stream);
      if (rc) return rc;
    }
  return RS_OK;
}

int rs_engine_sync(rs_engine* e) {
  RS_CHECK(e, RS_ERR_ARG, "null engine");
  RS_HIP(hipStreamSynchronize(e->stream));
  if (e->narrow) RS_HIP(hipStreamSynchronize(e->narrow));
  return RS_OK;
}

int rs_engine_fetch(rs_engine* e, int n, rs_dets* o) {
  RS_CHECK(e && o && o->count, RS_ERR_ARG, "null argument");
  RS_CHECK(n >= 1 && n <= e->max_batch, RS_ERR_ARG, "batch %d", n);
  const int D = e->D;
  hipStream_t s = e->stream;
  RS_HIP(hipMemcpyAsync(o->count, e->det_count, (size_t)n * 4, hipMemcpyDeviceToHost, s));
  if (o->boxes) RS_HIP(hipMemcpyAsync(o->boxes, e->det_boxes, (size_t)n * D * 16, hipMemcpyDeviceToHost, s));
  if (o->scores) RS_HIP(hipMemcpyAsync(o->scores, e->det_scores, (size_t)n * D * 4, hipMemcpyDeviceToHost, s));
  if (o->classes) RS_HIP(hipMemcpyAsync(o->classes, e->det_classes, (size_t)n * D * 4, hipMemcpyDeviceToHost, s));
  if (o->masks) {
    RS_CHECK(e->masks, RS_ERR_ARG, "masks requested but MASK_ON is false");
    RS_HIP(hipMemcpyAsync(o->masks, e->masks, (size_t)n * D * e->tile_h * ((e->tile_w + 7) / 8), hipMemcpyDeviceToHost, s));
  }
  if (o->mask_probs) {
    RS_CHECK(e->mask_probs, RS_ERR_ARG, "mask_probs requested but MASK_ON is false");
    RS_HIP(hipMemcpyAsync(o->mask_probs, e->mask_probs, (size_t)n * D * RS_MASK_SIDE * RS_MASK_SIDE * 4, hipMemcpyDeviceToHost, s));
  }
  { int rc = e->sat_copy(s); if (rc) return rc; }
  RS_HIP(hipStreamSynchronize(s));
  e->sat_publish();
  return RS_OK;
}

void* rs_host_alloc(size_t nbytes) {
  void* p = nullptr;
  if (hipHostMalloc(&p, nbytes ? nbytes : 16, hipHostMallocDefault) != hipSuccess) { rs_set_error("hipHostMalloc(%zu) failed", nbytes); return nullptr; }
  return p;
}
void rs_host_free(void* p) { if (p) (void)hipHostFree(p); }

int rs_host_register(void* p, size_t bytes) {
  RS_CHECK(p && bytes > 0, RS_ERR_ARG, "bad argument");
  RS_HIP(hipHostRegister(p, bytes, hipHostRegisterDefault));
  return RS_OK;
}
int rs_host_unregister(void* p) {
  RS_CHECK(p, RS_ERR_ARG, "bad argument");
  RS_HIP(hipHostUnregister(p));
  return RS_OK;
}

int rs_engine_upload_async(rs_engine* e, const uint8_t* tiles_host, int n) {
  RS_CHECK(e && tiles_host && n >= 1 && n <= e->max_batch, RS_ERR_ARG, "bad argument");
  RS_HIP(hipMemcpyAsync(e->tiles_dev, tiles_host, (size_t)n * e->tile_h * e->tile_w * e->tile_c, hipMemcpyHostToDevice, e->stream));
  return RS_OK;
}

int rs_engine_fetch_async(rs_engine* e, int n, rs_dets* o) {
  RS_CHECK(e && o && o->count && n >= 1 && n <= e->max_batch, RS_ERR_ARG, "bad argument");
  if (!e->copy_stream) {
    RS_HIP(hipStreamCreateWithFlags(&e->copy_stream, hipStreamNonBlocking));
    RS_HIP(hipEventCreateWithFlags(&e->ev_results, hipEventDisableTiming));
    RS_HIP(hipEventCreateWithFlags(&e->ev_copied, hipEventDisableTiming));
  }
  const int D = e->D;
  hipStream_t s = e->copy_stream;
  RS_HIP(hipEventRecord(e->ev_results, e->stream));
  RS_HIP(hipStreamWaitEvent(s, e->ev_results, 0));
  RS_HIP(hipMemcpyAsync(o->count, e->det_count, (size_t)n * 4, hipMemcpyDeviceToHost, s));
  if (o->boxes) RS_HIP(hipMemcpyAsync(o->boxes, e->det_boxes, (size_t)n * D * 16, hipMemcpyDeviceToHost, s));
  if (o->scores) RS_HIP(hipMemcpyAsync(o->scores, e->det_scores, (size_t)n * D * 4, hipMemcpyDeviceToHost, s));
  if (o->classes) RS_HIP(hipMemcpyAsync(o->classes, e->det_classes, (size_t)n * D * 4, hipMemcpyDeviceToHost, s));
  if (o->masks && e->masks) RS_HIP(hipMemcpyAsync(o->masks, e->masks, (size_t)n * D * e->tile_h * ((e->tile_w + 7) / 8), hipMemcpyDeviceToHost, s));
  { int rc = e->sat_copy(s); if (rc) return rc; }
  RS_HIP(hipEventRecord(e->ev_copied, s));
  e->copy_pending = true;
  return RS_OK;
}

int rs_engine_fetch_crops_async(rs_engine* e, int n, rs_dets* o, rs_mask_crops* c) {
  RS_CHECK(e && o && o->count && c && c->rects && c->offsets && c->data && n >= 1 && n <= e->max_batch, RS_ERR_ARG, "bad argument");
  RS_CHECK(e->masks && e->crop_data, RS_ERR_ARG, "mask crops requested but MASK_ON is false");
  if (!e->copy_stream) {
    RS_HIP(hipStreamCreateWithFlags(&e->copy_stream, hipStreamNonBlocking));
    RS_HIP(hipEventCreateWithFlags(&e->ev_results, hipEventDisableTiming));
    RS_HIP(hipEventCreateWithFlags(&e->ev_copied, hipEventDisableTiming));
  }
  if (!e->ev_crop_hdr) {
    RS_HIP(hipEventCreateWithFlags(&e->ev_crop_hdr, hipEventDisableTiming));
    RS_HIP(hipHostMalloc((void**)&e->h_crop_total, 16, hipHostMallocDefault));
  }
  const int D = e->D;
  hipStream_t s = e->copy_stream;
  RS_HIP(hipEventRecord(e->ev_results, e->stream));
  RS_HIP(hipStreamWaitEvent(s, e->ev_results, 0));
  CropParams cp;
  memset(&cp, 0, sizeof cp);
  cp.det_boxes = e->det_boxes; cp.det_count = e->det_count; cp.masks = e->masks; cp.n = n; cp.D = D; cp.h = e->tile_h; cp.w = e->tile_w;
  cp.Wb = (e->tile_w + 7) / 8; cp.rects = e->crop_rects; cp.offsets = e->crop_offsets; cp.total = e->crop_total; cp.data = e->crop_data;
  { int rc = launch_mask_crops(cp, s); if (rc) return rc; }
  RS_HIP(hipMemcpyAsync(o->count, e->det_count, (size_t)n * 4, hipMemcpyDeviceToHost, s));
  if (o->boxes) RS_HIP(hipMemcpyAsync(o->boxes, e->det_boxes, (size_t)n * D * 16, hipMemcpyDeviceToHost, s));
  if (o->scores) RS_HIP(hipMemcpyAsync(o->scores, e->det_scores, (size_t)n * D * 4, hipMemcpyDeviceToHost, s));
  if (o->classes) RS_HIP(hipMemcpyAsync(o->classes, e->det_classes, (size_t)n * D * 4, hipMemcpyDeviceToHost, s));
  RS_HIP(hipMemcpyAsync(c->rects, e->crop_rects, (size_t)n * D * 16, hipMemcpyDeviceToHost, s));
  RS_HIP(hipMemcpyAsync(c->offsets, e->crop_offsets, (size_t)n * D * 4, hipMemcpyDeviceToHost, s));
  RS_HIP(hipMemcpyAsync(e->h_crop_total, e->crop_total, 8, hipMemcpyDeviceToHost, s));
  { int rc = e->sat_copy(s); if (rc) return rc; }
  RS_HIP(hipEventRecord(e->ev_copied, s));
  RS_HIP(hipEventRecord(e->ev_crop_hdr, s));
  e->copy_pending = true;
  return RS_OK;
}

int rs_engine_fetch_crops_wait(rs_engine* e, rs_mask_crops* c) {
  RS_CHECK(e && c && c->data && e->ev_crop_hdr, RS_ERR_ARG, "rs_engine_fetch_crops_wait without rs_engine_fetch_crops_async");
  RS_HIP(hipEventSynchronize(e->ev_crop_hdr));
  const unsigned long long used = *e->h_crop_total;
  RS_CHECK(used <= c->capacity, RS_ERR_ARG, "mask crops need %llu bytes, the caller's buffer holds %llu", used, (unsigned long long)c->capacity);
  c->used = used;
  if (used) RS_HIP(hipMemcpyAsync(c->data, e->crop_data, (size_t)used, hipMemcpyDeviceToHost, e->copy_stream));
  RS_HIP(hipStreamSynchronize(e->copy_stream));
  e->sat_publish();
  return RS_OK;
}

int rs_engine_fetch_wait(rs_engine* e) {
  RS_CHECK(e, RS_ERR_ARG, "null engine");
  if (e->copy_stream) RS_HIP(hipStreamSynchronize(e->copy_stream));
  e->sat_publish();
  return RS_OK;
}

int rs_engine_infer(rs_engine* e, const uint8_t* tiles_host, int n, rs_dets* out_host) {
  RS_CHECK(e && tiles_host && out_host, RS_ERR_ARG, "null argument");
  RS_CHECK(n >= 1 && n <= e->max_batch, RS_ERR_ARG, "batch %d outside [1, %d]", n, e->max_batch);
  RS_HIP(hipSetDevice(e->device));
  RS_HIP(hipMemcpyAsync(e->tiles_dev, tiles_host, (size_t)n * e->tile_h * e->tile_w * e->tile_c, hipMemcpyHostToDevice, e->stream));
  int rc = e->run(e->tiles_dev, n);
  if (rc) return rc;
  return rs_engine_fetch(e, n, out_host);
}

void* rs_engine_stream(rs_engine* e) { return e ? (void*)e->stream : nullptr; }

int rs_engine_set_profiling(rs_engine* e, int enabled) {
  RS_CHECK(e, RS_ERR_ARG, "null engine");
  RS_CHECK(enabled >= 0 && enabled <= 3, RS_ERR_ARG, "profiling mode %d", enabled);
  if (e->ev_used) { int rc = e->resolve_profile(); if (rc) return rc; }
  e->forward_index = 0;
  e->ev_used = 0;
  e->profiling = enabled;
  for (Stage& s : e->stages) { s.ms_total = 0; s.calls = 0; }
  if (enabled >= 2 && e->ev_pool.empty()) {
    const size_t want = e->stages.size() * 32;
    e->ev_pool.resize(want);
    e->ev_stage.resize(want);
    e->ev_batch.resize(want);
    for (auto& pr : e->ev_pool) {
      RS_HIP(hipEventCreate(&pr.first));
      RS_HIP(hipEventCreate(&pr.second));
    }
  }
  return RS_OK;
}
int rs_engine_stage_count(rs_engine* e) { return e ? (int)e->stages.size() : 0; }
int rs_engine_saturation(rs_engine* e, int64_t* counts, int cap) {
  RS_CHECK(e && (counts || cap <= 0), RS_ERR_ARG, "null argument");
  const int n = (int)e->stages.size();
  for (int i = 0; i < n && i < cap; ++i) counts[i] = i < (int)e->h_sat.size() ? e->h_sat[i] : 0;
  return n;
}
int rs_engine_stage_info(rs_engine* e, int i, char* name_out, double* ms_total, int* calls, double* flops, double* bytes) {
  RS_CHECK(e && i >= 0 && i < (int)e->stages.size(), RS_ERR_ARG, "stage index");
  if (e->ev_used) { int rc = e->resolve_profile(); if (rc) return rc; }
  const Stage& s = e->stages[i];
  if (name_out) { strncpy(name_out, s.name.c_str(), 95); name_out[95] = 0; }
  if (ms_total) *ms_total = s.ms_total;
  if (calls) *calls = s.calls;
  if (flops) *flops = s.last_flops;
  if (bytes) *bytes = s.last_bytes;
  return RS_OK;
}

int rs_engine_stage_kernel(rs_engine* e, int i, char* name_out) {
  RS_CHECK(e && i >= 0 && i < (int)e->stages.size() && name_out, RS_ERR_ARG, "stage index");
  static const char* names[] = {"conv_igemm_kernel<2,2,4,4> 128x128", "conv_igemm_kernel<4,1,4,4> 256x64", "conv_igemm_kernel<4,1,1,4> 256x16 f32-out",
                                "conv_igemm_kernel<4,2,4,4> 256x128", "conv_igemm_kernel<2,4,4,8> 256x256", "conv_igemm_kernel<4,1,4,4,smallC> 256x64 stem",
                                "(retired)",
                                "conv_igemm_kernel<2,2,4,2> 64x128", "conv_igemm_kernel<4,1,4,2> 128x64", "conv_igemm_kernel<2,2,4,1> 32x128",
                                "conv_igemm_kernel<2,4,4,2> 64x256", "(retired)",
                                "conv_deep_kernel 256x256 (3 activation + 2 weight LDS stages)",
                                "bneck_tail_kernel 128 px (conv2 + conv3 + next conv1 chained through registers)",
                                "conv_igemm_kernel<2,4,4,4> 128x256",
                                "conv_deep_kernel 160x256", "conv_deep_kernel 192x256", "conv_deep_kernel 224x256",
                                "conv_deep_kernel 64x256", "conv_deep_kernel 96x256", "conv_deep_kernel 128x256",
                                "stem_pool_kernel (conv 7x7 s2 + ReLU + max-pool 3x3 s2, 8x8 pooled pixels per workgroup)",
                                "conv1x1_wreg_kernel 32 px x 256 ch (persistent, weights in registers, operand tiles by LDS-DMA, two workgroups per CU)",
                                "bneck_tail_split_kernel 128 px (conv2 + conv3 + next conv1 chained through registers)"};
  const int v = e->stages[i].variant;
  const char* s = v == -1 ? "conv_f32_mfma_kernel" : (v >= 0 && v <= 23 ? names[v] : "");
  if (e->split && v >= 0 && v <= 23) {
    snprintf(name_out, 96, "%.62s [split: hi+lo planes, 3 MFMA blocks]", s);
    return RS_OK;
  }
  strncpy(name_out, s, 95);
  name_out[95] = 0;
  return RS_OK;
}

int rs_engine_stage_variant(rs_engine* e, int i) {
  if (!e || i < 0 || i >= (int)e->stages.size()) return -2;
  return e->stages[i].variant;
}

int rs_op_conv_variant(int m, int cin, int k, int cout, int cin2, int deconv2x, int out_f32, int* stages_out) {
  ConvParams p;
  memset(&p, 0, sizeof p);
  p.M = m; p.Cin = cin; p.KH = p.KW = k; p.Cout = cout; p.mode = deconv2x ? 1 : 0; p.out_f32 = out_f32;
  p.stride = 1; p.in_Cs = cin; p.out_Cs = cout;
  p.Kpad = (k * k * (cin < 64 ? 8 : cin) + cin2 + 63) / 64 * 64;
  if (cin < 64 && k == 7) p.Kpad = 256;
  static const half_t dummy = (half_t)0;
  if (cin2 > 0) { p.in2 = &dummy; p.Cin2 = cin2; }
  const int v = conv_choose_variant(p, -1, 1);
  if (stages_out) *stages_out = p.stages;
  return cin < 64 ? 5 : v;
}

int rs_engine_tensor(rs_engine* e, const char* name, void** dev_ptr, int* dtype, int* ndim, int64_t dims[5], int* halo) {
  RS_CHECK(e && name, RS_ERR_ARG, "null argument");
  for (const TensorInfo& t : e->tensors) {
    if (t.name == name) {
      if (dev_ptr) *dev_ptr = t.p;
      if (dtype) *dtype = t.dtype;
      if (ndim) *ndim = t.ndim;
      if (dims) for (int i = 0; i < 5; ++i) dims[i] = t.dims[i];
      if (halo) *halo = t.halo;
      return RS_OK;
    }
  }
  rs_set_error("no tensor named %s", name);
  return RS_ERR_ARG;
}
int rs_engine_tensor_count(rs_engine* e) { return e ? (int)e->tensors.size() : 0; }
int rs_engine_tensor_name(rs_engine* e, int i, char* name_out) {
  RS_CHECK(e && i >= 0 && i < (int)e->tensors.size() && name_out, RS_ERR_ARG, "tensor index");
  strncpy(name_out, e->tensors[i].name.c_str(), 95);
  name_out[95] = 0;
  return RS_OK;
}

int rs_engine_net_shape(rs_engine* e, int* rh, int* rw, int* ph, int* pw) {
  RS_CHECK(e, RS_ERR_ARG, "null engine");
  if (rh) *rh = e->net_h;
  if (rw) *rw = e->net_w;
  if (ph) *ph = e->pad_h;
  if (pw) *pw = e->pad_w;
  return RS_OK;
}

static long long* g_conv_probe = nullptr;
static thread_local unsigned long long* g_op_sat = nullptr;
struct SplitArgs { long long in_lo, w_lo, out_lo, res_lo, up_lo; const float* wscale; };
static int op_conv2d(const void* in, const void* w, const float* bias, void* out, const void* residual, const void* upsample_add,
                     int n, int hi, int wi, int cin, int in_halo, int kh, int kw, int stride, int pad, int cout, int kpad,
                     int out_halo, int relu, int out_f32, int deconv2x, int variant, int use_glds, void* stream,
                     const void* in2, int h2, int w2, int cin2, int in2_halo, int stride2, const SplitArgs* sa = nullptr) {
  RS_CHECK(in && w && bias && out, RS_ERR_ARG, "null argument");
  RS_CHECK(in_halo >= pad, RS_ERR_ARG, "input halo %d < pad %d", in_halo, pad);
  const int ho = (hi + 2 * pad - kh) / stride + 1, wo = (wi + 2 * pad - kw) / stride + 1;
  ConvParams p;
  memset(&p, 0, sizeof p);
  p.in = (const half_t*)in; p.w = (const half_t*)w; p.bias = bias; p.out = out;
  p.res = (const half_t*)residual; p.up = (const half_t*)upsample_add;
  p.M = n * ho * wo; p.Ho = ho; p.Wo = wo;
  p.in_Hp = hi + 2 * in_halo; p.in_Wp = wi + 2 * in_halo; p.in_Cs = cin; p.in_off = in_halo - pad;
  p.stride = stride; p.KH = kh; p.KW = kw; p.Cin = cin; p.Kpad = kpad; p.Cout = cout;
  const int oh = deconv2x ? 2 * ho : ho, ow = deconv2x ? 2 * wo : wo;
  p.out_Hp = oh + 2 * out_halo; p.out_Wp = ow + 2 * out_halo; p.out_Cs = cout; p.out_pad = out_halo;
  if (upsample_add) { p.up_Hp = ho / 2 + 2 * out_halo; p.up_Wp = wo / 2 + 2 * out_halo; p.up_Cs = cout; p.up_pad = out_halo; }
  p.relu = relu; p.mode = deconv2x ? 1 : 0; p.out_f32 = out_f32;
  p.probe = g_conv_probe;
  p.sat = g_op_sat;
  if (sa) {
    RS_CHECK(sa->wscale && !in2, RS_ERR_ARG, "split-operand conv: row scales missing (or a second K source, which the operator does not take)");
    p.split = 1; p.in_lo = sa->in_lo; p.w_lo = sa->w_lo; p.out_lo = sa->out_lo; p.res_lo = sa->res_lo; p.up_lo = sa->up_lo; p.wscale = sa->wscale;
  }
  if (in2) {
    RS_CHECK(stride2 >= 1 && (ho - 1) * stride2 < h2 && (wo - 1) * stride2 < w2, RS_ERR_ARG, "second source geometry");
    p.in2 = (const half_t*)in2; p.in2_Hp = h2 + 2 * in2_halo; p.in2_Wp = w2 + 2 * in2_halo; p.in2_Cs = cin2;
    p.in2_off = in2_halo; p.stride2 = stride2; p.Cin2 = cin2;
  }
  int* koff_dev = nullptr;
  if (cin < 64 && use_glds >= 0) {
    RS_CHECK(cin == 8, RS_ERR_UNSUPPORTED, "small-Cin path needs cin == 8");
    std::vector<int> koff(kpad / 8, 0);
    for (int t = 0; t < kh * kw && t < (int)koff.size(); ++t) koff[t] = ((t / kw) * p.in_Wp + (t % kw)) * cin;
    RS_HIP(hipMalloc((void**)&koff_dev, koff.size() * 4));
    RS_HIP(hipMemcpy(koff_dev, koff.data(), koff.size() * 4, hipMemcpyHostToDevice));
    p.koff = koff_dev;
  }
  int rc = launch_conv(p, (hipStream_t)stream, variant, use_glds);
  if (koff_dev) {
    (void)hipStreamSynchronize((hipStream_t)stream);
    (void)hipFree(koff_dev);
  }
  return rc;
}

int rs_debug_set_conv_probe(void* buffer) { g_conv_probe = (long long*)buffer; return RS_OK; }
int rs_op_set_saturation_counter(void* dev_u64) { g_op_sat = (unsigned long long*)dev_u64; return RS_OK; }

int rs_op_conv2d(const void* in, const void* w, const float* bias, void* out, const void* residual, const void* upsample_add,
                 int n, int hi, int wi, int cin, int in_halo, int kh, int kw, int stride, int pad, int cout, int kpad,
                 int out_halo, int relu, int out_f32, int deconv2x, int variant, int use_glds, void* stream) {
  return op_conv2d(in, w, bias, out, residual, upsample_add, n, hi, wi, cin, in_halo, kh, kw, stride, pad, cout, kpad, out_halo,
                   relu, out_f32, deconv2x, variant, use_glds, stream, nullptr, 0, 0, 0, 0, 1);
}

int rs_op_conv2d_split(const void* in, int64_t in_lo, const void* w, int64_t w_lo, const float* wscale, const float* bias, void* out, int64_t out_lo,
                       const void* residual, int64_t res_lo, const void* upsample_add, int64_t up_lo,
                       int n, int hi, int wi, int cin, int in_halo, int kh, int kw, int stride, int pad, int cout, int kpad,
                       int out_halo, int relu, int out_f32, int deconv2x, int variant, void* stream) {
  SplitArgs sa = {in_lo, w_lo, out_lo, res_lo, up_lo, wscale};
  return op_conv2d(in, w, bias, out, residual, upsample_add, n, hi, wi, cin, in_halo, kh, kw, stride, pad, cout, kpad, out_halo,
                   relu, out_f32, deconv2x, variant, 1, stream, nullptr, 0, 0, 0, 0, 1, &sa);
}

int rs_op_conv2d_dual(const void* in, const void* in2, const void* w, const float* bias, void* out,
                      int n, int hi, int wi, int cin, int in_halo, int kh, int kw, int stride, int pad,
                      int h2, int w2, int cin2, int in2_halo, int stride2,
                      int cout, int kpad, int out_halo, int relu, int variant, void* stream) {
  RS_CHECK(in2, RS_ERR_ARG, "null argument");
  return op_conv2d(in, w, bias, out, nullptr, nullptr, n, hi, wi, cin, in_halo, kh, kw, stride, pad, cout, kpad, out_halo,
                   relu, 0, 0, variant, 1, stream, in2, h2, w2, cin2, in2_halo, stride2);
}

int rs_op_bneck_tail(const void* t1, const void* w2, const float* b2, const void* w3p, const float* b3, const void* x, void* out,
                     const void* w1p, const float* b1, void* t1n, const void* x0, const void* wsc, int n, int h, int w, int width, void* stream) {
  RS_CHECK(t1 && w2 && b2 && w3p && b3 && out && n > 0 && h > 0 && w > 0, RS_ERR_ARG, "bad argument");
  RS_CHECK(width == 64 || width == 128, RS_ERR_UNSUPPORTED, "bneck_tail: bottleneck width %d (64 or 128)", width);
  BneckParams p;
  memset(&p, 0, sizeof p);
  p.t1 = (const half_t*)t1; p.w2 = (const half_t*)w2; p.b2 = b2; p.w3p = (const half_t*)w3p; p.b3 = b3; p.x = (const half_t*)x; p.out = (half_t*)out;
  p.w1p = (const half_t*)w1p; p.b1 = b1; p.t1n = (half_t*)t1n; p.x0 = (const half_t*)x0; p.wsc = (const half_t*)wsc;
  p.M = n * h * w; p.H = h; p.W = w; p.Hp = h + 2; p.Wp = w + 2; p.CB = width / 64;
  p.sat = g_op_sat;
  return launch_bneck_tail(p, (hipStream_t)stream);
}

int rs_op_bneck_tail_split(const void* t1, int64_t t1_lo, const void* w2, const float* s2, const float* b2, const void* w3p, const float* s3, const float* b3,
                           const void* x, int64_t x_lo, void* out, int64_t out_lo, const void* w1p, const float* s1, const float* b1, void* t1n, int64_t t1n_lo,
                           const void* x0, int64_t x0_lo, int n, int h, int w, int width, void* stream) {
  RS_CHECK(t1 && w2 && s2 && b2 && w3p && s3 && b3 && (x || x0) && out && n > 0 && h > 0 && w > 0, RS_ERR_ARG, "bad argument");
  RS_CHECK(width == 64 || width == 128, RS_ERR_UNSUPPORTED, "bneck_tail_split: bottleneck width %d (64 or 128)", width);
  BneckSplitParams p;
  memset(&p, 0, sizeof p);
  p.t1 = (const half_t*)t1; p.t1_lo = t1_lo;
  p.w2 = (const half_t*)w2; p.w2_lo = (long long)width * 9 * width; p.s2 = s2; p.b2 = b2;
  p.w3p = (const half_t*)w3p; p.w3_lo = 4ll * width * (width + (x0 ? 64 : 0)); p.s3 = s3; p.b3 = b3;
  p.x = (const half_t*)x; p.x_lo = x_lo; p.x0 = (const half_t*)x0; p.x0_lo = x0_lo; p.out = (half_t*)out; p.out_lo = out_lo;
  p.w1p = (const half_t*)w1p; p.w1_lo = 4ll * width * width; p.s1 = s1; p.b1 = b1; p.t1n = (half_t*)t1n; p.t1n_lo = t1n_lo;
  p.M = n * h * w; p.H = h; p.W = w; p.Hp = h + 2; p.Wp = w + 2; p.CB = width / 64;
  p.sat = g_op_sat;
  return launch_bneck_tail_split(p, (hipStream_t)stream);
}

int rs_op_mask_overlap(const uint8_t* det_masks, int n_det, const uint8_t* label_masks, int n_labels, int h, int w, int32_t* inter,
                       int32_t* label_area, void* stream) {
  return launch_mask_overlap(det_masks, n_det, label_masks, n_labels, h, w, inter, label_area, (hipStream_t)stream);
}

int rs_engine_label_overlap(rs_engine* e, int tile, const uint8_t* label_masks_dev, int n_labels, int32_t* inter_dev, int32_t* label_area_dev) {
  RS_CHECK(e && e->masks && tile >= 0 && tile < e->max_batch && label_masks_dev && inter_dev && label_area_dev, RS_ERR_ARG, "bad argument");
  const size_t per = (size_t)e->tile_h * ((e->tile_w + 7) / 8);
  return launch_mask_overlap(e->masks + (size_t)tile * e->D * per, e->D, label_masks_dev, n_labels, e->tile_h, e->tile_w, inter_dev, label_area_dev, e->stream);
}

int rs_op_conv2d_dgrad(const void* dy, const void* w_t, void* dx, const void* res, const float* res32, const void* mask,
                       const void* down, int n, int hi, int wi, int cin, int ho, int wo, int cout, int kh, int kw, int stride,
                       int pad, int kpad, int halo, int variant, void* stream) {
  RS_CHECK(dy && w_t && dx, RS_ERR_ARG, "null argument");
  RS_CHECK(stride == 1 || (kh == 1 && kw == 1), RS_ERR_UNSUPPORTED, "dgrad: stride %d needs a 1x1 kernel (STRIDE_IN_1X1)", stride);
  RS_CHECK(halo >= kh - 1 - pad && halo >= 0 && kh == kw, RS_ERR_ARG, "dgrad: halo %d too small", halo);
  ConvParams p;
  memset(&p, 0, sizeof p);
  const int pad_t = kh - 1 - pad;
  const int oh = stride == 1 ? ho + 2 * pad_t - kh + 1 : ho, ow = stride == 1 ? wo + 2 * pad_t - kw + 1 : wo;
  RS_CHECK(stride == 1 ? (oh == hi && ow == wi) : ((ho - 1) * stride < hi && (wo - 1) * stride < wi), RS_ERR_ARG, "dgrad: geometry");
  void* zero_bias = nullptr;
  RS_HIP(hipMalloc(&zero_bias, (size_t)cin * 4 + 256));
  RS_HIP(hipMemsetAsync(zero_bias, 0, (size_t)cin * 4 + 256, (hipStream_t)stream));
  p.in = (const half_t*)dy; p.w = (const half_t*)w_t; p.bias = (const float*)zero_bias; p.out = dx;
  p.res = (const half_t*)res; p.res32 = res32; p.mask = (const half_t*)mask; p.down = (const half_t*)down;
  p.M = n * oh * ow; p.Ho = oh; p.Wo = ow;
  p.in_Hp = ho + 2 * halo; p.in_Wp = wo + 2 * halo; p.in_Cs = cout; p.in_off = halo - pad_t;
  p.stride = 1; p.KH = kh; p.KW = kw; p.Cin = cout; p.Kpad = kpad; p.Cout = cin;
  p.out_Hp = hi + 2 * halo; p.out_Wp = wi + 2 * halo; p.out_Cs = cin; p.out_pad = halo;
  p.out_stride = stride;
  if (down) { p.down_Hp = 2 * hi + 2 * halo; p.down_Wp = 2 * wi + 2 * halo; p.down_Cs = cin; p.down_pad = halo; }
  int rc = launch_conv(p, (hipStream_t)stream, variant, 1);
  (void)hipStreamSynchronize((hipStream_t)stream);
  (void)hipFree(zero_bias);
  return rc;
}

static int op_conv2d_wgrad(const void* dy, const void* x, float* grad, const float* scale, int n, int hi, int wi, int cin, int in_halo,
                           int kh, int kw, int stride, int pad, int cout, int kpad, int dy_halo, int splits, void* stream, int f32);
int rs_op_conv2d_wgrad(const void* dy, const void* x, float* grad, const float* scale, int n, int hi, int wi, int cin, int in_halo,
                       int kh, int kw, int stride, int pad, int cout, int kpad, int dy_halo, int splits, void* stream) {
  return op_conv2d_wgrad(dy, x, grad, scale, n, hi, wi, cin, in_halo, kh, kw, stride, pad, cout, kpad, dy_halo, splits, stream, 0);
}
int rs_op_conv2d_wgrad_f32(const void* dy, const void* x, float* grad, const float* scale, int n, int hi, int wi, int cin, int in_halo,
                           int kh, int kw, int stride, int pad, int cout, int kpad, int dy_halo, int splits, void* stream) {
  return op_conv2d_wgrad(dy, x, grad, scale, n, hi, wi, cin, in_halo, kh, kw, stride, pad, cout, kpad, dy_halo, splits, stream, 1);
}
static int op_conv2d_wgrad(const void* dy, const void* x, float* grad, const float* scale, int n, int hi, int wi, int cin, int in_halo,
                           int kh, int kw, int stride, int pad, int cout, int kpad, int dy_halo, int splits, void* stream, int f32) {
  RS_CHECK(dy && x && grad, RS_ERR_ARG, "null argument");
  RS_CHECK(in_halo >= pad, RS_ERR_ARG, "input halo %d < pad %d", in_halo, pad);
  const int ho = (hi + 2 * pad - kh) / stride + 1, wo = (wi + 2 * pad - kw) / stride + 1;
  WgradParams p;
  memset(&p, 0, sizeof p);
  p.dy = (const half_t*)dy; p.x = (const half_t*)x; p.grad = grad; p.scale = scale;
  p.M = n * ho * wo; p.Ho = ho; p.Wo = wo;
  p.dy_Hp = ho + 2 * dy_halo; p.dy_Wp = wo + 2 * dy_halo; p.dy_Cs = cout; p.dy_pad = dy_halo;
  p.in_Hp = hi + 2 * in_halo; p.in_Wp = wi + 2 * in_halo; p.in_Cs = cin; p.in_off = in_halo - pad;
  p.stride = stride; p.KH = kh; p.KW = kw; p.Cin = cin; p.Cout = cout; p.Kpad = kpad;
  p.f32 = f32;
  p.splits = splits > 0 ? splits : wgrad_splits(p);
  hipStream_t s = (hipStream_t)stream;
  void *partial = nullptr, *zeros = nullptr;
  RS_HIP(hipMalloc(&partial, (size_t)p.splits * cout * kpad * 4));
  RS_HIP(hipMalloc(&zeros, (size_t)cout * 2 + 256));
  RS_HIP(hipMemsetAsync(zeros, 0, (size_t)cout * 2 + 256, s));
  RS_HIP(hipMemsetAsync(partial, 0, (size_t)p.splits * cout * kpad * 4, s));
  p.partial = (float*)partial; p.zeros = (const half_t*)zeros;
  int rc = launch_conv_wgrad(p, s);
  (void)hipStreamSynchronize(s);
  (void)hipFree(partial);
  (void)hipFree(zeros);
  return rc;
}

int rs_op_nms(const float* boxes, const int32_t* counts, const uint8_t* valid, uint8_t* keep, int segments, int cap,
              float thresh, void* stream) {
  RS_CHECK(boxes && counts && keep && segments > 0, RS_ERR_ARG, "bad argument");
  RS_CHECK(cap >= 1 && cap <= 2048, RS_ERR_ARG, "cap %d outside [1,2048]", cap);
  NmsParams p = {};
  p.boxes = boxes; p.count = counts; p.valid = valid; p.keep = keep; p.cap = cap; p.thresh = thresh;
  void* scratch = nullptr;
  if (cap > 1024) {
    RS_HIP(hipMalloc(&scratch, (size_t)segments * 2048 * 32 * 8));
    p.scratch = (unsigned long long*)scratch;
  } else if (segments <= 32) {
    RS_HIP(hipMalloc(&scratch, (size_t)segments * 1024 * 16 * 8));
    p.scratch = (unsigned long long*)scratch;
  }
  int rc = launch_nms(p, segments, (hipStream_t)stream);
  if (scratch) { (void)hipStreamSynchronize((hipStream_t)stream); (void)hipFree(scratch); }
  return rc;
}

int rs_op_batched_nms(const float* boxes, const int32_t* counts, const uint8_t* valid, uint8_t* keep, int images, int segments_per_image,
                      int cap, float thresh, int rule, void* stream) {
  return rs_op_batched_nms_decision(boxes, counts, valid, keep, images, segments_per_image, cap, thresh, rule, nullptr, nullptr, stream);
}

int rs_op_batched_nms_decision(const float* boxes, const int32_t* counts, const uint8_t* valid, uint8_t* keep, int images, int segments_per_image,
                               int cap, float thresh, int rule, int32_t* rule_out, float* unit_out, void* stream) {
  RS_CHECK(boxes && counts && keep && images > 0 && segments_per_image > 0, RS_ERR_ARG, "bad argument");
  RS_CHECK(cap >= 1 && cap <= 2048, RS_ERR_ARG, "cap %d outside [1,2048]", cap);
  RS_CHECK(rule == 0 || rule == 1, RS_ERR_ARG, "rule %d (0 = per category, 1 = torchvision's size rule)", rule);
  const int segments = images * segments_per_image;
  RS_CHECK(rule || (!rule_out && !unit_out), RS_ERR_ARG, "rule 0 takes no decision");
  if (!rule) return rs_op_nms(boxes, counts, valid, keep, segments, cap, thresh, stream);
  RS_CHECK(cap > 1000, RS_ERR_ARG, "cap %d: the size rule needs a capacity above 1000 boxes per segment", cap);
  hipStream_t s = (hipStream_t)stream;
  NmsParams p = {};
  p.boxes = boxes; p.count = counts; p.valid = valid; p.keep = keep; p.cap = cap; p.thresh = thresh;
  void *scratch = nullptr, *dec = nullptr;
  RS_HIP(hipMalloc(&dec, (size_t)images * 12));
  const size_t sbytes = cap > 1024 ? (size_t)segments * 2048 * 32 * 8 : (segments <= 32 ? (size_t)segments * 1024 * 16 * 8 : 0);
  if (sbytes && hipMalloc(&scratch, sbytes) != hipSuccess) { (void)hipFree(dec); rs_set_error("hipMalloc(%zu)", sbytes); return RS_ERR_HIP; }
  p.scratch = (unsigned long long*)scratch;
  p.rule = (int*)dec; p.unit = (float*)((char*)dec + (size_t)images * 8); p.group = segments_per_image;
  int rc = launch_nms(p, segments, s);
  if (!rc && rule_out && hipMemcpyAsync(rule_out, p.rule, (size_t)images * 8, hipMemcpyDeviceToDevice, s) != hipSuccess) rc = RS_ERR_HIP;
  if (!rc && unit_out && hipMemcpyAsync(unit_out, p.unit, (size_t)images * 4, hipMemcpyDeviceToDevice, s) != hipSuccess) rc = RS_ERR_HIP;
  (void)hipStreamSynchronize(s);
  (void)hipFree(dec);
  if (scratch) (void)hipFree(scratch);
  return rc;
}

int rs_op_roi_align(const void* const feats[4], const int32_t heights[4], const int32_t widths[4], const float scales[4],
                    int nlevels, const float* rois, int n_rois, int rois_per_image, int P, int out_halo, void* out,
                    int32_t* levels_out, void* stream) {
  RS_CHECK(feats && rois && out && nlevels >= 1 && nlevels <= 4 && n_rois > 0 && rois_per_image > 0, RS_ERR_ARG, "bad argument");
  RoiAlignParams p;
  memset(&p, 0, sizeof p);
  for (int l = 0; l < nlevels; ++l) { p.feat[l] = (const half_t*)feats[l]; p.H[l] = heights[l]; p.W[l] = widths[l]; p.scale[l] = scales[l]; }
  p.nlevels = nlevels; p.C = 256; p.rois = rois; p.S = n_rois; p.slots_per_image = rois_per_image;
  p.out = (half_t*)out; p.P = P; p.out_pad = out_halo; p.out_level = levels_out;
  rs_debug_reload();
  return launch_roi_align(p, (hipStream_t)stream);
}

int rs_op_roi_align_bwd(float* const dfeats[4], const int32_t heights[4], const int32_t widths[4], const float scales[4],
                        int nlevels, const float* rois, int n_rois, int rois_per_image, int P, int out_halo, const void* dout,
                        void* stream) {
  RS_CHECK(dfeats && rois && dout && nlevels >= 1 && nlevels <= 4 && n_rois > 0 && rois_per_image > 0, RS_ERR_ARG, "bad argument");
  RoiAlignParams p;
  memset(&p, 0, sizeof p);
  for (int l = 0; l < nlevels; ++l) { p.dfeat[l] = dfeats[l]; p.H[l] = heights[l]; p.W[l] = widths[l]; p.scale[l] = scales[l]; }
  p.nlevels = nlevels; p.C = 256; p.rois = rois; p.S = n_rois; p.slots_per_image = rois_per_image;
  p.out = (half_t*)dout; p.P = P; p.out_pad = out_halo;
  rs_debug_reload();
  p.n_images = (n_rois + rois_per_image - 1) / rois_per_image;
  void* ws = nullptr;
  RS_HIP(hipMalloc(&ws, (size_t)n_rois * RS_ROI_BWD_TABLE_BYTES + 64));
  p.bwd_overflow = (int*)ws;
  p.bwd_tables = (char*)ws + 64;
  const int rc = launch_roi_align_bwd(p, (hipStream_t)stream);
  hipError_t he = hipStreamSynchronize((hipStream_t)stream);
  hipFree(ws);
  RS_HIP(he);
  return rc;
}

int rs_op_rpn_loss(const float* head, void* dhead, const int32_t* labels, const float* anchors, const float* matched_gt,
                   float* loss_out, int n, int hw, int num_anchors, int cs, int level_off, int total_anchors, float normalizer,
                   float loss_scale, void* stream) {
  RpnLossParams p;
  memset(&p, 0, sizeof p);
  p.head = head; p.dhead = (half_t*)dhead; p.labels = labels; p.anchors = anchors; p.matched_gt = matched_gt; p.loss_out = loss_out;
  p.A = num_anchors; p.cs = cs; p.HW = hw; p.n_anchors = hw * num_anchors; p.level_off = level_off; p.total_anchors = total_anchors;
  p.normalizer = normalizer; p.loss_scale = loss_scale;
  return launch_rpn_loss(p, n, (hipStream_t)stream);
}

int rs_op_box_loss(const float* pred, void* dpred, const int32_t* gt_classes, const float* proposals, const float* gt_boxes,
                   float* loss_out, int n_rois, int num_classes, int cs, float n_valid, const float reg_weights[4], float loss_scale,
                   void* stream) {
  RS_CHECK(reg_weights, RS_ERR_ARG, "null argument");
  BoxLossParams p;
  memset(&p, 0, sizeof p);
  p.pred = pred; p.dpred = (half_t*)dpred; p.gt_classes = gt_classes; p.proposals = proposals; p.gt_boxes = gt_boxes; p.loss_out = loss_out;
  p.n_rois = n_rois; p.K = num_classes; p.cs = cs; p.n_valid = n_valid;
  p.wx = reg_weights[0]; p.wy = reg_weights[1]; p.ww = reg_weights[2]; p.wh = reg_weights[3]; p.loss_scale = loss_scale;
  return launch_box_loss(p, (hipStream_t)stream);
}

int rs_op_mask_loss(const float* logits, void* dlogits, const uint8_t* targets, const int32_t* gt_classes, float* loss_out, int n_masks,
                    int side, int cs, float loss_scale, void* stream) {
  MaskLossParams p;
  memset(&p, 0, sizeof p);
  p.logits = logits; p.dlogits = (half_t*)dlogits; p.targets = targets; p.gt_classes = gt_classes; p.loss_out = loss_out;
  p.n_masks = n_masks; p.S = side; p.cs = cs; p.loss_scale = loss_scale;
  return launch_mask_loss(p, (hipStream_t)stream);
}

int rs_op_match(const float* boxes, int per_image_boxes, const int32_t* box_count, const float* gt, const int32_t* gt_count,
                int32_t* matched, int32_t* labels, float* best_iou, int n_images, int n_boxes, int gt_cap, float t_lo, float t_hi,
                int lbl_lo, int lbl_mid, int lbl_hi, int allow_low_quality, void* stream) {
  MatchParams p;
  memset(&p, 0, sizeof p);
  p.boxes = boxes; p.per_image_boxes = per_image_boxes; p.box_count = box_count; p.gt = gt; p.gt_count = gt_count;
  p.matched = matched; p.labels = labels; p.best_iou = best_iou; p.n_boxes = n_boxes; p.gt_cap = gt_cap;
  p.t_lo = t_lo; p.t_hi = t_hi; p.lbl_lo = lbl_lo; p.lbl_mid = lbl_mid; p.lbl_hi = lbl_hi;
  void* scratch = nullptr;
  if (allow_low_quality) {
// ... 31 lines not shown
```

Baseline: 949.9 tiles/s.

## Make deep conv kernel persistent with cross-tile prefetch of next tile's operands

Restructures the deep conv kernel so each workgroup can walk several tiles and carry pipeline state across them. It prefetches the next tile's first K-stage into LDS while the current tile's main loop finishes, hiding the per-tile prologue. Tile parameters are recomputed from kernarg at the epilogue to save registers. It also adds a mode-2 path for the fused mask predictor on deep tiles and grid-size knobs. With the default tiles_per_wg=1 the grid stays one workgroup per tile, so the prefetch only applies where grid < tiles. It adds complexity and register pressure.

```diff
diff --git a/proj_roadsurf_amd/csrc/common.h b/proj_roadsurf_amd/csrc/common.h
--- a/proj_roadsurf_amd/csrc/common.h
+++ b/proj_roadsurf_amd/csrc/common.h
@@ -76,6 +76,8 @@
   int fuse_bneck = 1;
   int deep_tile_px = 1;
   int deep_tail = 1;
+  int deep_tiles_per_wg = 1;
+  int deep_grid = 0;
   int fuse_rpn_heads = 1;
   int merge_levels = 1;
   int graph_small = 1;
diff --git a/proj_roadsurf_amd/csrc/conv_deep.hip b/proj_roadsurf_amd/csrc/conv_deep.hip
--- a/proj_roadsurf_amd/csrc/conv_deep.hip
+++ b/proj_roadsurf_amd/csrc/conv_deep.hip
@@ -1,4 +1,5 @@
 #include "common.h"
+#include <algorithm>
 
 namespace {
 
@@ -12,77 +13,161 @@
                                    (__attribute__((address_space(3))) void*)lds_wave_base, 16, 0, 0);
 }
 
-template <int DBG, bool TRAIN, int NJ, bool SPLIT>
-__device__ __forceinline__ void conv_deep_tile(const ConvParams& p, char* smem, const half_t* g_in, const half_t* g_w, const float* g_bias, void* g_out,
-                                               float* g_head_out, const int Ho, const int Wo, const int in_Hp, const int in_Wp, const int out_Hp, const int out_Wp,
-                                               const int M, const int m0, const int n0, const int q, const long long in_lo, const long long out_lo,
-                                               const float* g_wscale) {
+struct DeepTile {
+  const half_t* g_in; const half_t* g_w; const float* g_bias; void* g_out; float* g_head_out; const float* g_wscale;
+  long long in_lo, out_lo;
+  int Ho, Wo, in_Hp, in_Wp, out_Hp, out_Wp, M, m0, n0;
+  int half;
+  int q;
+  bool valid;
+  bool empty;
+};
+
+typedef const __attribute__((address_space(4))) ConvParams* DeepArgs;
+__device__ __forceinline__ DeepArgs deep_args() {
+  DeepArgs a = (DeepArgs)__builtin_amdgcn_kernarg_segment_ptr();
+  asm volatile("" : "+s"(a));
+  return a;
+}
+
+template <int NJF, bool SPLIT>
+__device__ __forceinline__ DeepTile deep_tile_at(int q, const int nfull, const int Mlaunch) {
+  asm volatile("" : "+s"(q));
+  constexpr int BM = 32 * NJF;
+  const DeepArgs P = deep_args();
+  DeepTile T;
+  T.q = q;
+  T.valid = q < nfull + 2 * P->tail_tiles;
+  T.g_in = P->in; T.g_w = P->w; T.g_bias = P->bias; T.g_out = P->out; T.g_head_out = P->head_out;
+  T.in_lo = P->in_lo; T.out_lo = P->out_lo; T.g_wscale = P->wscale;
+  T.Ho = P->Ho; T.Wo = P->Wo; T.in_Hp = P->in_Hp; T.in_Wp = P->in_Wp; T.out_Hp = P->out_Hp; T.out_Wp = P->out_Wp; T.M = Mlaunch;
+  const int tiles_n = P->Cout * (P->mode != 0 ? 4 : 1) / BN;
+  int L;
+  T.half = -1;
+  T.empty = false;
+  if (q < nfull) {
+    const int qn = nfull >> 3, r = nfull & 7, x = q & 7;
+    L = (x < r ? x * (qn + 1) : r * (qn + 1) + (x - r) * qn) + (q >> 3);
+  } else {
+    L = nfull + ((q - nfull) >> 1);
+    T.half = (q - nfull) & 1;
+  }
+  if (P->nseg) {
+    int t0 = 0;
+#pragma unroll
+    for (int i = 0; i < RS_MAX_SEGS; ++i)
+      if (i < P->nseg && L >= P->seg[i].tile0) {
+        T.g_in = P->seg[i].in; T.g_w = P->seg[i].w; T.g_bias = P->seg[i].bias; T.g_out = P->seg[i].out; T.g_head_out = P->seg[i].head_out;
+        T.Ho = P->seg[i].Ho; T.Wo = P->seg[i].Wo; T.in_Hp = P->seg[i].in_Hp; T.in_Wp = P->seg[i].in_Wp;
+        T.out_Hp = P->seg[i].out_Hp; T.out_Wp = P->seg[i].out_Wp; T.M = P->seg[i].M; t0 = P->seg[i].tile0;
+        if constexpr (SPLIT) { T.in_lo = P->seg[i].in_lo; T.out_lo = P->seg[i].out_lo; T.g_wscale = P->seg[i].wscale; }
+      }
+    L -= t0;
+  }
+  T.n0 = (L % tiles_n) * BN;
+  T.m0 = (L / tiles_n) * BM;
+  if (T.half >= 0 && NJF == 8) {
+    T.m0 += T.half * (BM / 2);
+    if (T.m0 >= T.M) T.empty = true;
+  }
+  return T;
+}
+
+template <bool SPLIT>
+struct DeepCarry {
+  int a3 = 0, w1 = 0;
+  int akh = 0, akw = 0, ac0 = 0, wkh = 0, wkw = 0, wc0 = 0;
+  const half_t* s_in = nullptr; const half_t* s_w = nullptr;
+  int s_in_Wp = 0;
+  long long s_wn0 = 0;
+  unsigned aoff[4];
+  int ra = 0, rw = 0;
+  bool pre = false;
+};
+
+template <int DBG, bool TRAIN, int NJ, bool SPLIT, int NJF>
+__device__ __forceinline__ void conv_deep_tile(const ConvParams& p, char* smem, const int q, const int qn , const int nfull, const int Mlaunch,
+                                               DeepCarry<SPLIT>& c) {
   constexpr int APS = (NJ + 1) / 2;
   constexpr int WPX = NJ * 16;
-  const int tid = threadIdx.x;
+  int tid = threadIdx.x;
+  asm volatile("" : "+v"(tid));
   const int lane = tid & 63;
   const int wave = __builtin_amdgcn_readfirstlane(tid >> 6);
   const int wpx = wave / WCH, wch = wave % WCH;
-  (void)q;
-
+#ifdef RS_SPLIT_PHASES
+  const unsigned long long ph_entry = __builtin_amdgcn_s_memtime();
+#endif
   const int lrow = lane >> 3, lchk = lane & 7;
-  const half_t* aptr[APS];
-  const half_t* wptr[4];
-  unsigned aoffb[APS], woffb[4];
-#pragma unroll
-  for (int ps = 0; ps < APS; ++ps) {
-    int m = m0 + ps * 64 + wave * 8 + lrow;
-    if (m >= M) m = M - 1;
-    const int x = m % Wo;
-    const int t = m / Wo;
-    const int y = t % Ho;
-    const int n = t / Ho;
-    const long long base =
-        ((long long)(n * in_Hp + y * p.stride + p.in_off) * in_Wp + x * p.stride + p.in_off) * p.in_Cs;
-    if constexpr (SPLIT) aoffb[ps] = (unsigned)((base + ((lchk ^ lrow) & 3) * 8 + ((lchk ^ lrow) >> 2) * in_lo) * 2);
-    else aptr[ps] = g_in + base + (lchk ^ lrow) * 8;
-  }
+  typedef unsigned aoff_t;
+  auto tile_aoff = [&](const DeepTile& D, aoff_t* o) {
+#pragma unroll
+    for (int ps = 0; ps < APS; ++ps) {
+      int m = D.m0 + ps * 64 + wave * 8 + lrow;
+      if (m >= D.M) m = D.M - 1;
+      const int x = m % D.Wo;
+      const int t = m / D.Wo;
+      const int y = t % D.Ho;
+      const int n = t / D.Ho;
+      const long long base =
+          ((long long)(n * D.in_Hp + y * p.stride + p.in_off) * D.in_Wp + x * p.stride + p.in_off) * p.in_Cs;
+      if constexpr (SPLIT) o[ps] = (unsigned)((base + ((lchk ^ lrow) & 3) * 8 + ((lchk ^ lrow) >> 2) * D.in_lo) * 2);
+      else o[ps] = (unsigned)((base + (lchk ^ lrow) * 8) * 2);
+    }
+  };
+  auto stream_to = [&](const DeepTile& D) {
+    c.s_in = D.g_in; c.s_w = D.g_w; c.s_in_Wp = D.in_Wp; c.s_wn0 = (long long)D.n0 * p.Kpad;
+    c.akh = c.akw = c.ac0 = c.wkh = c.wkw = c.wc0 = 0;
+  };
+  if (!c.pre) { const DeepTile D = deep_tile_at<NJF, SPLIT>(q, nfull, Mlaunch); tile_aoff(D, c.aoff); stream_to(D); }
+  unsigned woffb[4];
 #pragma unroll
   for (int ps = 0; ps < 4; ++ps) {
     const int row = ps * 64 + wave * 8 + lrow;
     const int key = (row & 3) | (((row >> 4) & 1) << 2);
-    if constexpr (SPLIT) woffb[ps] = (unsigned)(((long long)(n0 + row) * p.Kpad + ((lchk ^ key) & 3) * 8 + ((lchk ^ key) >> 2) * p.w_lo) * 2);
-    else wptr[ps] = g_w + (long long)(n0 + row) * p.Kpad + (lchk ^ key) * 8;
+    if constexpr (SPLIT) woffb[ps] = (unsigned)(((long long)row * p.Kpad + ((lchk ^ key) & 3) * 8 + ((lchk ^ key) >> 2) * p.w_lo) * 2);
+    else woffb[ps] = (unsigned)(((long long)row * p.Kpad + (lchk ^ key) * 8) * 2);
   }
   constexpr int KST = SPLIT ? 32 : 64;
   const int nk = p.KH * p.KW * (p.Cin / KST);
-
-  int akh = 0, akw = 0, ac0 = 0, an = 0;
+  const bool pf = !TRAIN && qn >= 0 && !p.head_w && nk >= (SPLIT ? 2 : 3);
+  aoff_t naoff[APS];
+  if (pf) { const DeepTile D = deep_tile_at<NJF, SPLIT>(qn, nfull, Mlaunch); tile_aoff(D, naoff); }
+
   auto stage_a = [&]() {
-    const int off = (akh * in_Wp + akw) * p.in_Cs + ac0;
-    if (++akw == p.KW) { akw = 0; if (++akh == p.KH) { akh = 0; ac0 += KST; } }
-    char* abase = smem + (an % 3) * ASTAGE;
-    ++an;
+    const int off = (c.akh * c.s_in_Wp + c.akw) * p.in_Cs + c.ac0;
+    if (++c.akw == p.KW) { c.akw = 0; if (++c.akh == p.KH) { c.akh = 0; c.ac0 += KST; } }
+    char* abase = smem + c.a3 * ASTAGE;
+    c.a3 = c.a3 == 2 ? 0 : c.a3 + 1;
     if (DBG & 1) return;
     if (DBG & 8) return;
-    if constexpr (SPLIT) {
-#pragma unroll
-      for (int ps = 0; ps < APS; ++ps) glds16((const half_t*)((const char*)g_in + (aoffb[ps] + (unsigned)(off * 2))), abase + (ps * 64 + wave * 8) * 128);
-    } else {
-#pragma unroll
-      for (int ps = 0; ps < APS; ++ps) glds16(aptr[ps] + off, abase + (ps * 64 + wave * 8) * 128);
-    }
+#pragma unroll
+    for (int ps = 0; ps < APS; ++ps) glds16((const half_t*)((const char*)c.s_in + (c.aoff[ps] + (unsigned)(off * 2))), abase + (ps * 64 + wave * 8) * 128);
   };
-  int wkh = 0, wkw = 0, wc0 = 0, wn = 0;
   auto stage_w = [&]() {
-    const int koff = (wkh * p.KW + wkw) * p.Cin + wc0;
-    if (++wkw == p.KW) { wkw = 0; if (++wkh == p.KH) { wkh = 0; wc0 += KST; } }
-    char* wbase = smem + W_BASE + (wn & 1) * WSTAGE;
-    ++wn;
+    const int koff = (c.wkh * p.KW + c.wkw) * p.Cin + c.wc0;
+    if (++c.wkw == p.KW) { c.wkw = 0; if (++c.wkh == p.KH) { c.wkh = 0; c.wc0 += KST; } }
+    char* wbase = smem + W_BASE + c.w1 * WSTAGE;
+    c.w1 ^= 1;
     if (DBG & 1) return;
     if (DBG & 4) return;
-    if constexpr (SPLIT) {
-#pragma unroll
-      for (int ps = 0; ps < 4; ++ps) glds16((const half_t*)((const char*)g_w + (woffb[ps] + (unsigned)(koff * 2))), wbase + (ps * 64 + wave * 8) * 128);
-    } else {
-#pragma unroll
-      for (int ps = 0; ps < 4; ++ps) glds16(wptr[ps] + koff, wbase + (ps * 64 + wave * 8) * 128);
-    }
+    const half_t* wrow0 = c.s_w + (c.s_wn0 + koff);
+#pragma unroll
+    for (int ps = 0; ps < 4; ++ps) glds16((const half_t*)((const char*)wrow0 + woffb[ps]), wbase + (ps * 64 + wave * 8) * 128);
+  };
+  auto issue_a = [&](int i) {
+    if (i < nk) { stage_a(); return; }
+    if (!pf) return;
+    if (i == nk) {
+      const DeepTile D = deep_tile_at<NJF, SPLIT>(qn, nfull, Mlaunch);
+      stream_to(D);
+#pragma unroll
+      for (int ps = 0; ps < APS; ++ps) c.aoff[ps] = naoff[ps];
+    }
+    stage_a();
+  };
+  auto issue_w = [&](int i) {
+    if (i < nk || pf) stage_w();
   };
 
   const int fi = lane & 15, fq = lane >> 4, fkey = lane & 7;
@@ -129,21 +214,27 @@
   const unsigned long long pr_t0 = __builtin_amdgcn_s_memtime(), pr_r0 = __builtin_amdgcn_s_memrealtime();
 #endif
 #ifdef RS_SPLIT_PHASES
-  const unsigned long long ph_entry = __builtin_amdgcn_s_memtime();
   unsigned long long ph_loop0 = 0, ph_loop1 = 0;
 #endif
-  stage_w();
-  stage_a();
-  if (nk > 1) stage_a();
-  if (nk > 1) asm volatile("s_waitcnt vmcnt(%0)" ::"n"(APS) : "memory");
-  else asm volatile("s_waitcnt vmcnt(0)" ::: "memory");
-  asm volatile("s_barrier" ::: "memory");
+  if (c.pre) {
+    asm volatile("s_waitcnt vmcnt(0)" ::: "memory");
+    asm volatile("s_barrier" ::: "memory");
+  } else {
+    if (q != (int)blockIdx.x) __syncthreads();
+    stage_w();
+    stage_a();
+    if (nk > 1) stage_a();
+    if (nk > 1) asm volatile("s_waitcnt vmcnt(%0)" ::"n"(APS) : "memory");
+    else asm volatile("s_waitcnt vmcnt(0)" ::: "memory");
+    asm volatile("s_barrier" ::: "memory");
+  }
   __builtin_amdgcn_sched_barrier(0);
-  if (nk > 1) stage_w();
+  c.pre = pf;
+  issue_w(1);
 #ifndef RS_SPLIT_SCHED_V1
-  if constexpr (!SPLIT) { if (nk > 2) stage_a(); }
+  if constexpr (!SPLIT) issue_a(2);
 #else
-  if (nk > 2) stage_a();
+  issue_a(2);
 #endif
   if constexpr (SPLIT) {
 #define RS_RD_W(wf, wa) RS_DSR(wf[0], wa, 0); RS_DSR(wf[1], wa, 512); RS_DSR(wf[2], wa, 1024); RS_DSR(wf[3], wa, 1536);
@@ -156,17 +247,18 @@
   if constexpr (NJ > 6) { RS_DSR(xf[6], xa, 12288); }                                               \
   if constexpr (NJ > 7) { RS_DSR(xf[7], xa, 14336); }
     {
-      const unsigned wa = wa0, xa = xa1;
+      const unsigned wa = wa0 + c.rw * WSTAGE, xa = xa1 + c.ra * ASTAGE;
       RS_RD_W(wf0, wa)
       RS_RD_X(xf1, xa)
     }
-    int sab = 0;
+    int sab = c.ra;
+    const unsigned wst0 = c.rw * WSTAGE;
 #ifdef RS_SPLIT_PHASES
     unsigned long long ph_work = 0, ph_vm = 0, ph_bar = 0, ph_last = __builtin_amdgcn_s_memtime();
     ph_loop0 = ph_last;
 #endif
     for (int t = 0; t < nk; ++t) {
-      const unsigned wst = (t & 1) * WSTAGE, ast = sab * ASTAGE;
+      const unsigned wst = (t & 1) ? WSTAGE - wst0 : wst0, ast = sab * ASTAGE;
       __builtin_amdgcn_sched_barrier(0);
       { const unsigned xa = xa0 + ast; RS_RD_X(xf0, xa) }
       __builtin_amdgcn_sched_barrier(0);
@@ -179,7 +271,7 @@
           acc[i][j] = __builtin_amdgcn_mfma_f32_16x16x32_f16(wf0[i], xf1[j], acc[i][j], 0, 0, 0);
       __builtin_amdgcn_sched_barrier(0);
 #ifndef RS_SPLIT_SCHED_V1
-      if (t + 2 < nk) stage_a();
+      issue_a(t + 2);
 #endif
       { const unsigned wa = wa1 + wst; RS_RD_W(wf1, wa) }
       __builtin_amdgcn_sched_barrier(0);
@@ -200,7 +292,7 @@
         ph_work += ph1 - ph_last;
         __builtin_amdgcn_sched_barrier(0);
 #endif
-        if (t + 2 < nk) asm volatile("s_waitcnt vmcnt(%0)" ::"n"(APS) : "memory");
+        if (t + 2 < nk || pf) asm volatile("s_waitcnt vmcnt(%0)" ::"n"(APS) : "memory");
         else asm volatile("s_waitcnt vmcnt(0)" ::: "memory");
 #ifdef RS_SPLIT_PHASES
         __builtin_amdgcn_sched_barrier(0);
@@ -223,12 +315,12 @@
               acc[i][j] = __builtin_amdgcn_mfma_f32_16x16x32_f16(wf1[i], xf0[j], acc[i][j], 0, 0, 0);
           __builtin_amdgcn_sched_barrier(0);
         }
-        if (t + 2 < nk) stage_w();
+        issue_w(t + 2);
 #ifdef RS_SPLIT_SCHED_V1
-        if (t + 3 < nk) stage_a();
+        issue_a(t + 3);
 #endif
         {
-          const unsigned wa = wa0 + ((t + 1) & 1) * WSTAGE, xa = xa1 + snext * ASTAGE;
+          const unsigned wa = wa0 + (WSTAGE - wst), xa = xa1 + snext * ASTAGE;
           RS_RD_W(wf0, wa)
           RS_RD_X(xf1, xa)
         }
@@ -247,6 +339,8 @@
     }
 #undef RS_RD_W
 #undef RS_RD_X
+    c.ra = sab;
+    c.rw ^= nk & 1;
 #ifdef RS_SPLIT_PHASES
     ph_loop1 = __builtin_amdgcn_s_memtime();
     if (p.probe && lane == 0) {
@@ -256,11 +350,11 @@
     }
 #endif
   } else {
-  reads0(0, 0);
-  int abuf = 0;
+  reads0(c.ra, c.rw);
+  int abuf = c.ra;
   for (int t = 0; t < nk; ++t) {
     __builtin_amdgcn_sched_barrier(0);
-    reads1(abuf, t & 1);
+    reads1(abuf, (t & 1) ^ c.rw);
     __builtin_amdgcn_sched_barrier(0);
     asm volatile("s_waitcnt lgkmcnt(%0)" ::"n"(4 + NJ) : "memory");
     __builtin_amdgcn_sched_barrier(0);
@@ -273,7 +367,7 @@
     const int anext = abuf == 2 ? 0 : abuf + 1;
     if (t + 1 < nk) {
       asm volatile("s_waitcnt lgkmcnt(0)" ::: "memory");
-      if (t + 2 < nk) asm volatile("s_waitcnt vmcnt(%0)" ::"n"(APS) : "memory");
+      if (t + 2 < nk || pf) asm volatile("s_waitcnt vmcnt(%0)" ::"n"(APS) : "memory");
       else asm volatile("s_waitcnt vmcnt(0)" ::: "memory");
       asm volatile("s_barrier" ::: "memory");
       __builtin_amdgcn_sched_barrier(0);
@@ -287,9 +381,9 @@
         __builtin_amdgcn_sched_barrier(0);
       }
 #endif
-      if (t + 2 < nk) stage_w();
-      if (t + 3 < nk) stage_a();
-      reads0(anext, (t + 1) & 1);
+      issue_w(t + 2);
+      issue_a(t + 3);
+      reads0(anext, ((t + 1) & 1) ^ c.rw);
 #ifndef RS_DEEP_LOCKSTEP
       if (wpx) { abuf = anext; continue; }
 #endif
@@ -306,6 +400,8 @@
       for (int j = 0; j < NJ; ++j)
         acc[i][j] = __builtin_amdgcn_mfma_f32_16x16x32_f16(wf1[i], xf1[j], acc[i][j], 0, 0, 0);
   }
+  c.ra = abuf;
+  c.rw ^= nk & 1;
   }
 
 #ifdef RS_CLOCK_PROBE
@@ -314,6 +410,11 @@
     p.probe[2 * q + 1] = (long long)(__builtin_amdgcn_s_memrealtime() - pr_r0);
   }
 #endif
+  const DeepArgs pe = deep_args();
+  const DeepTile T = deep_tile_at<NJF, SPLIT>(q, nfull, Mlaunch);
+  const float* const g_bias = T.g_bias; void* const g_out = T.g_out; float* const g_head_out = T.g_head_out; const float* const g_wscale = T.g_wscale;
+  const long long out_lo = T.out_lo;
+  const int Ho = T.Ho, Wo = T.Wo, out_Hp = T.out_Hp, out_Wp = T.out_Wp, M = T.M, m0 = T.m0, n0 = T.n0;
   const int crow = n0 + wch * 64 + fq * 16;
   float bias[16];
 #pragma unroll
@@ -330,10 +431,10 @@
     }
   }
   unsigned satc = 0;
-  if (!TRAIN && SPLIT && p.head_w) {
-    const half_t* hw = p.head_w + (long long)fi * 256 + wch * 64 + fq * 8;
+  if (!TRAIN && SPLIT && pe->head_w) {
+    const half_t* hw = pe->head_w + (long long)fi * 256 + wch * 64 + fq * 8;
     const half8 ha0 = *(const half8*)hw, ha1 = *(const half8*)(hw + 32);
-    const half8 hl0 = *(const half8*)(hw + p.head_w_lo), hl1 = *(const half8*)(hw + p.head_w_lo + 32);
+    const half8 hl0 = *(const half8*)(hw + pe->head_w_lo), hl1 = *(const half8*)(hw + pe->head_w_lo + 32);
     f32x4 hacc[NJ];
 #pragma unroll
     for (int j = 0; j < NJ; ++j) {
@@ -345,14 +446,14 @@
 #pragma unroll
         for (int r = 0; r < 4; ++r) {
           float f = acc[i][j][r] * wsc[i * 4 + r] + bias[i * 4 + r];
-          if (p.relu) f = f > 0.f ? f : 0.f;
+          if (pe->relu) f = f > 0.f ? f : 0.f;
           sath += mv ? rs_sat_bad(f) : 0u;
           f = f > 65504.f ? 65504.f : (f < -65504.f ? -65504.f : f);
           const half_t h = (half_t)f;
           const half_t l = (half_t)(f - (float)h);
           if (i < 2) { b0[i * 4 + r] = h; l0[i * 4 + r] = l; } else { b1[(i - 2) * 4 + r] = h; l1[(i - 2) * 4 + r] = l; }
         }
-      rs_sat_flush(p.sat, sath);
+      rs_sat_flush(pe->sat, sath);
       f32x4 a = f32x4{0.f, 0.f, 0.f, 0.f};
       a = __builtin_amdgcn_mfma_f32_16x16x32_f16(ha0, b0, a, 0, 0, 0);
       a = __builtin_amdgcn_mfma_f32_16x16x32_f16(ha1, b1, a, 0, 0, 0);
@@ -376,8 +477,8 @@
         s0 += *(const f32x4*)(part + ((w * 2 * WPX + px) * 16 + oh));
         s1 += *(const f32x4*)(part + ((w * 2 * WPX + px) * 16 + oh + 4));
       }
-      s0 = s0 * *(const f32x4*)(p.head_scale + oh) + *(const f32x4*)(p.head_b + oh);
-      s1 = s1 * *(const f32x4*)(p.head_scale + oh + 4) + *(const f32x4*)(p.head_b + oh + 4);
+      s0 = s0 * *(const f32x4*)(pe->head_scale + oh) + *(const f32x4*)(pe->head_b + oh);
+      s1 = s1 * *(const f32x4*)(pe->head_scale + oh + 4) + *(const f32x4*)(pe->head_b + oh + 4);
       const int x = m % Wo, t = m / Wo, y = t % Ho, n = t / Ho;
       float* op = g_head_out + ((long long)(n * Ho + y) * Wo + x) * 16 + oh;
       *(f32x4*)op = s0;
@@ -385,8 +486,8 @@
     }
     return;
   }
-  if (!TRAIN && !SPLIT && p.head_w) {
-    const half_t* hw = p.head_w + (long long)fi * 256 + wch * 64 + fq * 8;
+  if (!TRAIN && !SPLIT && pe->head_w) {
+    const half_t* hw = pe->head_w + (long long)fi * 256 + wch * 64 + fq * 8;
     const half8 ha0 = *(const half8*)hw, ha1 = *(const half8*)(hw + 32);
     f32x4 hacc[NJ];
 #pragma unroll
@@ -399,12 +500,12 @@
 #pragma unroll
         for (int r = 0; r < 4; ++r) {
           float f = acc[i][j][r] + bias[i * 4 + r];
-          if (p.relu) f = f > 0.f ? f : 0.f;
+          if (pe->relu) f = f > 0.f ? f : 0.f;
           sath += mv ? rs_sat_bad(f) : 0u;
           f = f > 65504.f ? 65504.f : (f < -65504.f ? -65504.f : f);
           if (i < 2) b0[i * 4 + r] = (half_t)f; else b1[(i - 2) * 4 + r] = (half_t)f;
         }
-      rs_sat_flush(p.sat, sath);
+      rs_sat_flush(pe->sat, sath);
       f32x4 a = f32x4{0.f, 0.f, 0.f, 0.f};
       a = __builtin_amdgcn_mfma_f32_16x16x32_f16(ha0, b0, a, 0, 0, 0);
       a = __builtin_amdgcn_mfma_f32_16x16x32_f16(ha1, b1, a, 0, 0, 0);
@@ -418,7 +519,7 @@
     const int px = tid >> 1, oh = (tid & 1) * 8;
     const int m = m0 + px;
     if (px < 2 * WPX && m < M) {
-      f32x4 s0 = *(const f32x4*)(p.head_b + oh), s1 = *(const f32x4*)(p.head_b + oh + 4);
+      f32x4 s0 = *(const f32x4*)(pe->head_b + oh), s1 = *(const f32x4*)(pe->head_b + oh + 4);
 #pragma unroll
       for (int w = 0; w < 4; ++w) {
         s0 += *(const f32x4*)(part + ((w * 2 * WPX + px) * 16 + oh));
@@ -430,6 +531,57 @@
       *(f32x4*)(op + 4) = s1;
     }
     return;
+  }
+  if constexpr (!TRAIN && SPLIT) {
+    if (pe->mode == 2) {
+      const int g = n0 / pe->Cout, cb = crow - n0;
+      float dotp[NJ];
+      int dot_idx[NJ];
+#pragma unroll
+      for (int j = 0; j < NJ; ++j) {
+        dotp[j] = 0.f; dot_idx[j] = -1;
+        const int m = m0 + wpx * WPX + j * 16 + fi;
+        if (m >= M) continue;
+        const int x = m % Wo, t = m / Wo, y = t % Ho, n = t / Ho;
+        const int oy = 2 * y + (g >> 1), ox = 2 * x + (g & 1);
+        const int slot = pe->dot_slot[n];
+        const float* wv = pe->dot_w + (long long)pe->dot_cls[slot] * pe->Cout + cb;
+        float sdot = 0.f;
+#pragma unroll
+        for (int i = 0; i < MI; ++i) {
+          const f32x4 w4 = *(const f32x4*)(wv + i * 4);
+#pragma unroll
+          for (int r = 0; r < 4; ++r) {
+            float f = acc[i][j][r] * wsc[i * 4 + r] + bias[i * 4 + r];
+            if (pe->relu) f = f > 0.f ? f : 0.f;
+            sdot += f * w4[r];
+          }
+        }
+        dotp[j] = sdot;
+        dot_idx[j] = slot * (4 * Ho * Wo) + oy * (2 * Wo) + ox;
+      }
+      float* red = (float*)(smem + (c.ra == 0 ? 2 : c.ra - 1) * ASTAGE);
+      asm volatile("s_barrier" ::: "memory");
+#pragma unroll
+      for (int j = 0; j < NJ; ++j) {
+        float v0 = dotp[j];
+        v0 += __shfl_xor(v0, 16);
+        v0 += __shfl_xor(v0, 32);
+        dotp[j] = v0;
+        if (wch > 0 && fq == 0) red[(wch - 1) * 2 * WPX + wpx * WPX + j * 16 + fi] = v0;
+      }
+      __syncthreads();
+      if (wch == 0 && fq == 0) {
+#pragma unroll
+        for (int j = 0; j < NJ; ++j) {
+          float v0 = dotp[j];
+#pragma unroll
+          for (int cw = 1; cw < WCH; ++cw) v0 += red[(cw - 1) * 2 * WPX + wpx * WPX + j * 16 + fi];
+          if (dot_idx[j] >= 0) pe->dot_out[dot_idx[j]] = v0;
+        }
+      }
+      return;
+    }
   }
 #pragma unroll
   for (int j = 0; j < NJ; ++j) {
@@ -439,7 +591,7 @@
     const int t = m / Wo;
     const int y = t % Ho;
     const int n = t / Ho;
-    const long long opix = (long long)(n * out_Hp + y + p.out_pad) * out_Wp + x + p.out_pad;
+    const long long opix = (long long)(n * out_Hp + y + pe->out_pad) * out_Wp + x + pe->out_pad;
     float v[16];
 #pragma unroll
     for (int i = 0; i < MI; ++i)
@@ -448,13 +600,13 @@
         if constexpr (SPLIT) v[i * 4 + r] = acc[i][j][r] * wsc[i * 4 + r] + bias[i * 4 + r];
         else v[i * 4 + r] = acc[i][j][r] + bias[i * 4 + r];
       }
-    if (p.res) {
-      const half_t* rp = p.res + opix * p.out_Cs + crow;
+    if (pe->res) {
+      const half_t* rp = pe->res + opix * pe->out_Cs + crow;
 #pragma unroll
       for (int i = 0; i < MI; ++i) {
         const half4 h = *(const half4*)(rp + i * 4);
         if constexpr (SPLIT) {
-          const half4 l = *(const half4*)(rp + p.res_lo + i * 4);
+          const half4 l = *(const half4*)(rp + pe->res_lo + i * 4);
 #pragma unroll
           for (int r = 0; r < 4; ++r) v[i * 4 + r] += (float)h[r] + (float)l[r];
         } else {
@@ -463,14 +615,14 @@
         }
       }
     }
-    if (p.up) {
-      const long long upix = (long long)(n * p.up_Hp + (y >> 1) + p.up_pad) * p.up_Wp + (x >> 1) + p.up_pad;
-      const half_t* up = p.up + upix * p.up_Cs + crow;
+    if (pe->up) {
+      const long long upix = (long long)(n * pe->up_Hp + (y >> 1) + pe->up_pad) * pe->up_Wp + (x >> 1) + pe->up_pad;
+      const half_t* up = pe->up + upix * pe->up_Cs + crow;
 #pragma unroll
       for (int i = 0; i < MI; ++i) {
         const half4 h = *(const half4*)(up + i * 4);
         if constexpr (SPLIT) {
-          const half4 l = *(const half4*)(up + p.up_lo + i * 4);
+          const half4 l = *(const half4*)(up + pe->up_lo + i * 4);
 #pragma unroll
           for (int r = 0; r < 4; ++r) v[i * 4 + r] += (float)h[r] + (float)l[r];
         } else {
@@ -479,11 +631,11 @@
         }
       }
     }
-    if (TRAIN && p.down) {
+    if (TRAIN && pe->down) {
 #pragma unroll
       for (int dd = 0; dd < 4; ++dd) {
-        const long long dpix = (long long)(n * p.down_Hp + 2 * y + (dd >> 1) + p.down_pad) * p.down_Wp + 2 * x + (dd & 1) + p.down_pad;
-        const half_t* dp = p.down + dpix * p.down_Cs + crow;
+        const long long dpix = (long long)(n * pe->down_Hp + 2 * y + (dd >> 1) + pe->down_pad) * pe->down_Wp + 2 * x + (dd & 1) + pe->down_pad;
+        const half_t* dp = pe->down + dpix * pe->down_Cs + crow;
 #pragma unroll
         for (int i = 0; i < MI; ++i) {
           const half4 h = *(const half4*)(dp + i * 4);
@@ -492,8 +644,8 @@
         }
       }
     }
-    if (TRAIN && p.res32) {
-      const float* rp = p.res32 + opix * p.out_Cs + crow;
+    if (TRAIN && pe->res32) {
+      const float* rp = pe->res32 + opix * pe->out_Cs + crow;
 #pragma unroll
       for (int i = 0; i < MI; ++i) {
         const f32x4 h = *(const f32x4*)(rp + i * 4);
@@ -501,8 +653,8 @@
         for (int r = 0; r < 4; ++r) v[i * 4 + r] += h[r];
       }
     }
-    if (TRAIN && p.mask) {
-      const half_t* mp = p.mask + opix * p.out_Cs + crow;
+    if (TRAIN && pe->mask) {
+      const half_t* mp = pe->mask + opix * pe->out_Cs + crow;
 #pragma unroll
       for (int i = 0; i < MI; ++i) {
         const half4 h = *(const half4*)(mp + i * 4);
@@ -510,16 +662,16 @@
         for (int r = 0; r < 4; ++r) v[i * 4 + r] = (float)h[r] > 0.f ? v[i * 4 + r] : 0.f;
       }
     }
-    if (p.relu) {
+    if (pe->relu) {
 #pragma unroll
       for (int e = 0; e < 16; ++e) v[e] = v[e] > 0.f ? v[e] : 0.f;
     }
-    if (p.out_f32) {
-      float* op = (float*)g_out + opix * p.out_Cs + crow;
+    if (pe->out_f32) {
+      float* op = (float*)g_out + opix * pe->out_Cs + crow;
 #pragma unroll
       for (int i = 0; i < MI; ++i) *(f32x4*)(op + i * 4) = f32x4{v[i * 4], v[i * 4 + 1], v[i * 4 + 2], v[i * 4 + 3]};
     } else {
-      half_t* op = (half_t*)g_out + opix * p.out_Cs + crow;
+      half_t* op = (half_t*)g_out + opix * pe->out_Cs + crow;
 #pragma unroll
       for (int i = 0; i < MI; i += 2) {
         half8 h, l;
@@ -536,14 +688,14 @@
       }
     }
   }
-  rs_sat_flush(p.sat, satc);
+  rs_sat_flush(pe->sat, satc);
 #ifdef RS_SPLIT_PHASES
   if constexpr (SPLIT) {
     const unsigned long long ph_issued = __builtin_amdgcn_s_memtime();
-    asm volatile("s_waitcnt vmcnt(0)" ::: "memory");
+    if (qn < 0) asm volatile("s_waitcnt vmcnt(0)" ::: "memory");
     const unsigned long long ph_drained = __builtin_amdgcn_s_memtime();
-    if (p.probe && lane == 0) {
-      long long* o = p.probe + ((long long)q * 8 + wave) * 8;
+    if (pe->probe && lane == 0) {
+      long long* o = pe->probe + ((long long)q * 8 + wave) * 8;
       o[6] = (long long)(ph_issued - ph_loop1); o[7] = (long long)(ph_drained - ph_issued);
     }
   }
@@ -554,52 +706,35 @@
 template <int DBG, bool TRAIN = false, int NJF = 8, bool SPLIT = false>
 __global__ __launch_bounds__(NT) void conv_deep_kernel(const ConvParams p) {
   constexpr int BM = 32 * NJF;
+  constexpr bool LOOP = !TRAIN && NJF == 8;
   extern __shared__ __attribute__((aligned(16))) char smem[];
   int M = p.M;
   if (p.m_count) {
     long long mc = (long long)(*p.m_count) * p.m_mul;
     if (mc < M) M = (int)mc;
   }
-  const int tiles_n = p.Cout / BN;
+  const int tiles_n = p.Cout * (p.mode != 0 ? 4 : 1) / BN;
   const int ntiles = p.nseg ? p.seg_tiles : tiles_n * ((M + BM - 1) / BM);
   const int nfull = ntiles - p.tail_tiles;
-  const int q = blockIdx.x;
-  if (q >= nfull + 2 * p.tail_tiles) return;
-  const half_t* g_in = p.in;
-  const half_t* g_w = p.w;
-  const float* g_bias = p.bias;
-  void* g_out = p.out;
-  float* g_head_out = p.head_out;
-  long long in_lo = p.in_lo, out_lo = p.out_lo;
-  const float* g_wscale = p.wscale;
-  int Ho = p.Ho, Wo = p.Wo, in_Hp = p.in_Hp, in_Wp = p.in_Wp, out_Hp = p.out_Hp, out_Wp = p.out_Wp;
-  int L, half = -1;
-  if (q < nfull) {
-    const int qn = nfull >> 3, r = nfull & 7, x = q & 7;
-    L = (x < r ? x * (qn + 1) : r * (qn + 1) + (x - r) * qn) + (q >> 3);
+  const int G = gridDim.x;
+  DeepCarry<SPLIT> c;
+  const int entries = nfull + 2 * p.tail_tiles;
+  auto entry_from = [&](int q) {
+    for (; q < entries; q += G)
+      if (q < nfull || NJF != 8 || !deep_tile_at<NJF, SPLIT>(q, nfull, M).empty) return q;
+    return -1;
+  };
+  if constexpr (!LOOP) {
+    const int q = blockIdx.x;
+    if (q < entries) conv_deep_tile<DBG, TRAIN, NJF, SPLIT, NJF>(p, smem, q, -1, nfull, M, c);
   } else {
-    L = nfull + ((q - nfull) >> 1);
-    half = (q - nfull) & 1;
-  }
-  if (p.nseg) {
-    int t0 = 0;
-#pragma unroll
-    for (int i = 0; i < RS_MAX_SEGS; ++i)
-      if (i < p.nseg && L >= p.seg[i].tile0) {
-        g_in = p.seg[i].in; g_w = p.seg[i].w; g_bias = p.seg[i].bias; g_out = p.seg[i].out; g_head_out = p.seg[i].head_out;
-        Ho = p.seg[i].Ho; Wo = p.seg[i].Wo; in_Hp = p.seg[i].in_Hp; in_Wp = p.seg[i].in_Wp;
-        out_Hp = p.seg[i].out_Hp; out_Wp = p.seg[i].out_Wp; M = p.seg[i].M; t0 = p.seg[i].tile0;
-        if constexpr (SPLIT) { in_lo = p.seg[i].in_lo; out_lo = p.seg[i].out_lo; g_wscale = p.seg[i].wscale; }
-      }
-    L -= t0;
-  }
-  const int n0 = (L % tiles_n) * BN;
-  const int m0 = (L / tiles_n) * BM;
-  if (half < 0 || NJF != 8) {
-    conv_deep_tile<DBG, TRAIN, NJF, SPLIT>(p, smem, g_in, g_w, g_bias, g_out, g_head_out, Ho, Wo, in_Hp, in_Wp, out_Hp, out_Wp, M, m0, n0, q, in_lo, out_lo, g_wscale);
-  } else {
-    if (m0 + half * (BM / 2) >= M) return;
-    conv_deep_tile<DBG, TRAIN, NJF == 8 ? 4 : NJF, SPLIT>(p, smem, g_in, g_w, g_bias, g_out, g_head_out, Ho, Wo, in_Hp, in_Wp, out_Hp, out_Wp, M, m0 + half * (BM / 2), n0, q, in_lo, out_lo, g_wscale);
+    int q = entry_from(blockIdx.x);
+    while (q >= 0) {
+      const int qn = entry_from(q + G);
+      if (q < nfull) conv_deep_tile<DBG, TRAIN, 8, SPLIT, 8>(p, smem, q, qn, nfull, M, c);
+      else conv_deep_tile<DBG, TRAIN, 4, SPLIT, 8>(p, smem, q, qn, nfull, M, c);
+      q = qn;
+    }
   }
 }
 
@@ -622,6 +757,17 @@
   if (!rs_debug().deep_tail) return 0;
   const int r = (int)(tiles % ncu);
   return (r > 0 && 2 * r <= ncu) ? r : 0;
+}
+
+static unsigned deep_grid(long long entries) {
+  const RsDebug& D = rs_debug();
+  const long long ncu = rs_device_cu_count();
+  long long g = entries;
+  if (D.deep_tiles_per_wg == 0) g = ncu;
+  else if (D.deep_tiles_per_wg > 1) g = std::max(ncu, (entries + D.deep_tiles_per_wg - 1) / D.deep_tiles_per_wg);
+  if (g < entries) g = (g + 7) & ~7ll;
+  if (D.deep_grid > 0 && D.deep_grid < g) g = D.deep_grid;
+  return (unsigned)std::min(g, entries);
 }
 
 static int no_scratch(const void* kernel, const char* what) {
@@ -659,16 +805,20 @@
 int launch_conv_deep(const ConvParams& p0, hipStream_t stream, int tile_px) {
   ConvParams p = p0;
   p.nseg = 0;
-  RS_CHECK(p.mode == 0 && !p.in2 && p.Cin % 64 == 0 && p.Cout % BN == 0 && p.M > 0, RS_ERR_ARG,
+  RS_CHECK((p.mode == 0 || p.mode == 2) && !p.in2 && p.Cin % 64 == 0 && p.Cout % BN == 0 && p.M > 0, RS_ERR_ARG,
            "conv_deep: unsupported shape (mode %d, Cin %d, Cout %d)", p.mode, p.Cin, p.Cout);
+  RS_CHECK(p.mode != 2 || (p.split && tile_px == 256 && p.Cout == BN && p.dot_w && p.dot_cls && p.dot_slot && p.dot_out && !p.head_w && !p.res && !p.up &&
+                           !p.down && !p.res32 && !p.mask && p.KH == 1 && p.KW == 1 && p.stride == 1),
+           RS_ERR_UNSUPPORTED, "conv_deep: the fused mask predictor runs in the split-operand mode on 256-pixel tiles with Cout == 256 and its pointers");
   RS_CHECK(!p.head_w || (p.Cout == BN && p.head_b && p.head_out && !p.res && !p.up && !p.down && !p.res32 && !p.mask), RS_ERR_ARG,
            "conv_deep: the fused head needs Cout == 256, its bias and output, and no other epilogue option");
   RS_CHECK(p.out_stride <= 1, RS_ERR_UNSUPPORTED, "conv_deep: no strided scatter");
   RS_CHECK(!p.split || (p.wscale && (!p.head_w || p.head_scale) && !p.down && !p.res32 && !p.mask), RS_ERR_UNSUPPORTED, "conv_deep: the split-operand mode needs the row scales (the fused head's too) and has no training epilogue");
-  if (p.split) {
+  {
     const long long in_px = (long long)cdiv(p.M, p.Ho * p.Wo) * p.in_Hp * p.in_Wp;
-    RS_CHECK((p.in_lo + in_px * p.in_Cs) * 2 < (1ll << 32) && (p.w_lo + (long long)p.Cout * p.Kpad) * 2 < (1ll << 32), RS_ERR_UNSUPPORTED,
-             "conv_deep: split-operand tensor of more than 4 GB (input %lld elements per plane)", in_px * p.in_Cs);
+    const long long in_lo = p.split ? p.in_lo : 0, w_lo = p.split ? p.w_lo : 0;
+    RS_CHECK((in_lo + in_px * p.in_Cs) * 2 < (1ll << 32) && (w_lo + (long long)p.Cout * (p.mode != 0 ? 4 : 1) * p.Kpad) * 2 < (1ll << 32), RS_ERR_UNSUPPORTED,
+             "conv_deep: tensor of more than 4 GB (input %lld elements per plane)", in_px * p.in_Cs);
   }
   if (tile_px != 256) {
     RS_CHECK(tile_px >= 64 && tile_px <= 224 && tile_px % 32 == 0 && !p.down && !p.res32 && !p.mask, RS_ERR_ARG,
@@ -705,7 +855,7 @@
 #else
   constexpr int dbg = 0;
 #endif
-  long long nblk = (long long)(p.Cout / BN) * cdiv(p.M, BM);
+  long long nblk = (long long)(p.Cout * (p.mode != 0 ? 4 : 1) / BN) * cdiv(p.M, BM);
   RS_CHECK(nblk < (1ll << 30), RS_ERR_ARG, "conv_deep: grid too large");
   p.tail_tiles = (p.m_count || dbg) ? 0 : deep_tail_tiles(nblk);
   nblk += p.tail_tiles;
@@ -717,9 +867,9 @@
   if (dbg == 17) { hipLaunchKernelGGL(conv_deep_kernel<17>, dim3((unsigned)nblk), dim3(NT), LDS_BYTES, stream, p); return RS_OK; }
 #endif
   (void)dbg;
-  if (p.split) hipLaunchKernelGGL((conv_deep_kernel<0, false, 8, true>), dim3((unsigned)nblk), dim3(NT), LDS_BYTES, stream, p);
+  if (p.split) hipLaunchKernelGGL((conv_deep_kernel<0, false, 8, true>), dim3(deep_grid(nblk)), dim3(NT), LDS_BYTES, stream, p);
   else if (p.down || p.res32 || p.mask) hipLaunchKernelGGL((conv_deep_kernel<0, true>), dim3((unsigned)nblk), dim3(NT), LDS_BYTES, stream, p);
-  else hipLaunchKernelGGL(conv_deep_kernel<0>, dim3((unsigned)nblk), dim3(NT), LDS_BYTES, stream, p);
+  else hipLaunchKernelGGL(conv_deep_kernel<0>, dim3(deep_grid(nblk)), dim3(NT), LDS_BYTES, stream, p);
   RS_HIP(hipGetLastError());
   return RS_OK;
 }
@@ -735,9 +885,9 @@
   for (int i = 0; i < nseg; ++i) {
     RS_CHECK(segs[i].in && segs[i].w && segs[i].bias && segs[i].out && m_per_image[i] > 0, RS_ERR_ARG, "conv_deep_multi: map %d incomplete", i);
     RS_CHECK(!common.split || segs[i].wscale, RS_ERR_ARG, "conv_deep_multi: map %d has no row scales (split-operand mode)", i);
-    RS_CHECK(!common.split || ((segs[i].in_lo + (long long)images * segs[i].in_Hp * segs[i].in_Wp * common.in_Cs) * 2 < (1ll << 32) &&
-                               (common.w_lo + (long long)common.Cout * common.Kpad) * 2 < (1ll << 32)),
-             RS_ERR_UNSUPPORTED, "conv_deep_multi: map %d: split-operand tensor of more than 4 GB", i);
+    RS_CHECK(((common.split ? segs[i].in_lo : 0) + (long long)images * segs[i].in_Hp * segs[i].in_Wp * common.in_Cs) * 2 < (1ll << 32) &&
+                 ((common.split ? common.w_lo : 0) + (long long)common.Cout * common.Kpad) * 2 < (1ll << 32),
+             RS_ERR_UNSUPPORTED, "conv_deep_multi: map %d: tensor of more than 4 GB", i);
     p.seg[i] = segs[i];
     p.seg[i].M = images * m_per_image[i];
     p.seg[i].tile0 = (int)tiles;
@@ -762,11 +912,11 @@
   }
   if (p.split) {
     RS_CHECK(!p.head_w || p.head_scale, RS_ERR_ARG, "conv_deep_multi: the fused head of the split-operand mode needs its row scales");
-    hipLaunchKernelGGL((conv_deep_kernel<0, false, 8, true>), dim3((unsigned)tiles), dim3(NT), LDS_BYTES, stream, p);
+    hipLaunchKernelGGL((conv_deep_kernel<0, false, 8, true>), dim3(deep_grid(tiles)), dim3(NT), LDS_BYTES, stream, p);
     RS_HIP(hipGetLastError());
     return RS_OK;
   }
-  hipLaunchKernelGGL(conv_deep_kernel<0>, dim3((unsigned)tiles), dim3(NT), LDS_BYTES, stream, p);
+  hipLaunchKernelGGL(conv_deep_kernel<0>, dim3(deep_grid(tiles)), dim3(NT), LDS_BYTES, stream, p);
   RS_HIP(hipGetLastError());
   return RS_OK;
 }
diff --git a/proj_roadsurf_amd/csrc/engine.hip b/proj_roadsurf_amd/csrc/engine.hip
--- a/proj_roadsurf_amd/csrc/engine.hip
+++ b/proj_roadsurf_amd/csrc/engine.hip
@@ -23,7 +23,7 @@
   rd("RS_CONV_SINGLE_STAGE_NK", &d.conv_single_stage_nk); rd("RS_CONV_PERSIST", &d.conv_persist); rd("RS_CONV_TUNED", &d.conv_tuned);
   rd("RS_CONV_DEEP", &d.conv_deep); rd("RS_CONV_WIDE_PX", &d.conv_wide_px); rd("RS_CONV_WREG", &d.conv_wreg); rd("RS_WREG_DBG", &d.wreg_dbg); rd("RS_ROI_BWD_ATOMIC", &d.roi_bwd_atomic); rd("RS_WREG_WAVES", &d.wreg_waves); rd("RS_STEM_SMALL_TILE", &d.stem_small_tile); rd("RS_DEEP_DBG", &d.deep_dbg);
   rd("RS_DECONV_VARIANT", &d.deconv_variant); rd("RS_FUSE_MASK_PREDICTOR", &d.fuse_mask_predictor); rd("RS_SIDE_STREAM", &d.side_stream);
-  rd("RS_NARROW_ROIALIGN", &d.narrow_roialign); rd("RS_USE_GLDS", &d.use_glds); rd("RS_FUSE_SHORTCUT", &d.fuse_shortcut); rd("RS_MERGE_LEVELS", &d.merge_levels); rd("RS_FUSE_RPN_HEADS", &d.fuse_rpn_heads); rd("RS_DEEP_TAIL", &d.deep_tail); rd("RS_DEEP_TILE_PX", &d.deep_tile_px); rd("RS_FUSE_BNECK", &d.fuse_bneck); rd("RS_FUSE_STEM", &d.fuse_stem);
+  rd("RS_NARROW_ROIALIGN", &d.narrow_roialign); rd("RS_USE_GLDS", &d.use_glds); rd("RS_FUSE_SHORTCUT", &d.fuse_shortcut); rd("RS_MERGE_LEVELS", &d.merge_levels); rd("RS_FUSE_RPN_HEADS", &d.fuse_rpn_heads); rd("RS_DEEP_TAIL", &d.deep_tail); rd("RS_DEEP_TILES_PER_WG", &d.deep_tiles_per_wg); rd("RS_DEEP_GRID", &d.deep_grid); rd("RS_DEEP_TILE_PX", &d.deep_tile_px); rd("RS_FUSE_BNECK", &d.fuse_bneck); rd("RS_FUSE_STEM", &d.fuse_stem);
   rd("RS_USE_GRAPH", &d.use_graph); rd("RS_GRAPH_SMALL", &d.graph_small); rd("RS_TRAIN_ROI_SIDE", &d.train_roi_side);
   rd("RS_TRAIN_SIDE", &d.train_side); rd("RS_WGRAD_TARGET", &d.wgrad_target); rd("RS_WGRAD_CB", &d.wgrad_cb);
   rd("RS_SELECT_DEBUG", &d.select_debug); rd("RS_NMS_DEBUG", &d.nms_debug); rd("RS_ROI_WINDOW", &d.roi_window); rd("RS_ROI_ORDER", &d.roi_order);
@@ -1070,7 +1070,8 @@
         RS_HIP(hipMemsetAsync(probs, 0, zero_per_tile * n, s));
         dp.M = n * Dc * per_roi;
         const int dv = rs_debug().deconv_variant;
-        return launch_conv(dp, s, (dv == 22 && (sp || !(rs_debug().conv_wreg && glds > 0))) ? 14 : dv, glds);
+        if (sp) return launch_conv(dp, s, dv == 22 || (dv == 12 && !(rs_debug().conv_deep && glds > 0)) ? 14 : dv, glds);
+        return launch_conv(dp, s, (dv == 22 && !(rs_debug().conv_wreg && glds > 0)) ? 14 : dv, glds);
       };
       stages.push_back(st);
       MaskPredictParams mp;
@@ -1661,6 +1662,7 @@
                      const void* in2, int h2, int w2, int cin2, int in2_halo, int stride2, const SplitArgs* sa = nullptr) {
   RS_CHECK(in && w && bias && out, RS_ERR_ARG, "null argument");
   RS_CHECK(in_halo >= pad, RS_ERR_ARG, "input halo %d < pad %d", in_halo, pad);
+  rs_debug_reload();
   const int ho = (hi + 2 * pad - kh) / stride + 1, wo = (wi + 2 * pad - kw) / stride + 1;
   ConvParams p;
   memset(&p, 0, sizeof p);
```

After: 928.8 tiles/s. 0.978x the previous value.
